# wallisc/TracerBoy

Hardware: AMD Instinct MI355X
Metric: Msamples/s (WxHxspp/s) (higher is better)
Workload: dtype f32; 1 GPU; cornell-box 1920x1080 64spp depth8; triangles=36, bvh_builder=sah, pipeline=lockstep, parallelism=tiles1, scene_in_lds=True, kernel_variant=matte

## Files before the change

### include/tracerboy_hip.h

```cpp
#ifndef TRACERBOY_HIP_H
#define TRACERBOY_HIP_H

#include <stdint.h>
#include "tb_abi.h"

#ifdef __cplusplus
extern "C" {
#endif

#define TB_OK 0
#define TB_E_INVALID -1
#define TB_E_NO_DEVICE -2
#define TB_E_IO -3
#define TB_E_PARSE -4
#define TB_E_DEVICE -5
#define TB_E_UNSUPPORTED -6
#define TB_E_NO_SCENE -7

typedef struct tb_context tb_context;

typedef struct tb_camera {
    float Position[3], LookAt[3], Right[3], Up[3];
    float LensHeight, FocalDistance;
} tb_camera;
// ... 220 lines not shown
void tb_default_visualize_settings(tb_visualize_settings* out);
int tb_record_paths(tb_context* ctx, uint32_t x, uint32_t y, uint32_t first_frame, uint32_t n_frames, TbPathFrame* frames_or_null, uint32_t* rays_total_or_null);
int tb_clear_paths(tb_context* ctx);
int tb_read_paths(tb_context* ctx, TbVisualizerRay* rays_or_null, uint32_t capacity, uint32_t* count);
int tb_visualize_rays(tb_context* ctx, const tb_visualize_settings* settings_or_null, float* rgba_f32_or_null, uint8_t* rgba8_or_null);
int tb_visualize_constants(const tb_camera* camera, uint32_t width, uint32_t height, const tb_visualize_settings* settings_or_null, TbVisualizeConstants* out);
int tb_run_visualize_rays(tb_context* ctx, const TbVisualizeConstants* constants, const TbVisualizerRay* rays, uint32_t n_rays, const float* scene_rgba,
                          const float* world_pos_or_null, float* out_rgba);

#define TB_RAYS_CLOSEST  0u
#define TB_RAYS_OCCLUDED 1u
#define TB_RAYS_DEVICE   0x100u
int tb_trace_rays(tb_context* ctx, uint32_t mode_and_flags, uint64_t n, const TbQueryRay* rays, void* out);

#define TB_RADIANCE_RAY        0u
#define TB_RADIANCE_HEMISPHERE 1u
#define TB_RADIANCE_DEVICE     0x100u
#define TB_RADIANCE_ACCUMULATE 0x200u
int tb_trace_radiance(tb_context* ctx, const tb_output_settings* settings_or_null, float time, const TbRadianceCall* call, uint64_t n,
                      const TbRadianceRay* rays, TbFloat4* out);
int tb_radiance_refusal(const TbRadianceCall* call, uint64_t n, const void* rays, const void* out, char* why_or_null, uint32_t why_bytes);
int tb_make_camera_rays(tb_context* ctx, const tb_output_settings* settings_or_null, float time, uint32_t width, uint32_t height,
                        uint32_t x0, uint32_t y0, uint32_t x1, uint32_t y1, uint32_t frame, uint32_t flags, TbRadianceRay* out, float* seed_advance_out);

#define TB_BAKE_DEVICE     0x100u
#define TB_BAKE_ACCUMULATE 0x200u
typedef struct tb_bake_call { uint32_t width, height, first_sample, num_samples, dilate_passes, flags; } tb_bake_call;
int tb_bake_lightmap(tb_context* ctx, const tb_output_settings* settings_or_null, float time, const tb_bake_call* call, const float* uv_or_null,
                     float* rgba_out);
int tb_bake_refusal(const tb_bake_call* call, const void* uv_or_null, const void* rgba_out, char* why_or_null, uint32_t why_bytes);
int tb_read_bake(tb_context* ctx, TbRadianceRay* rays_or_null, TbBakeTexel* texels_or_null, float* sums_or_null);
int tb_run_bake_raster(tb_context* ctx, uint32_t width, uint32_t height, uint32_t n_vertices, const float* positions, const float* normals,
                       const float* uvs, uint32_t n_triangles, const uint32_t* tri_vertex_index, TbRadianceRay* rays_out, TbBakeTexel* texels_out);
int tb_run_bake_dilate(tb_context* ctx, uint32_t width, uint32_t height, uint32_t passes, const float* rgba_in, float* rgba_out);

#define TB_PROBES_DEVICE     0x100u
#define TB_PROBES_ACCUMULATE 0x200u
#define TB_PROBES_KEEP_MAPS  0x400u
typedef struct tb_probe_call { uint32_t n, first_probe_number, resolution, first_sample, num_samples, flags; } tb_probe_call;
int tb_bake_probes(tb_context* ctx, const tb_output_settings* settings_or_null, float time, const tb_probe_call* call, const float* positions_xyz,
                   TbProbe* probes_out);
int tb_probes_refusal(const tb_probe_call* call, const void* positions_xyz, const void* probes_out, char* why_or_null, uint32_t why_bytes);
int tb_read_probe_maps(tb_context* ctx, float* sums_or_null, TbQueryHit* hits_or_null);
int tb_sample_probes(tb_context* ctx, uint32_t flags, const tb_probe_grid* grid, uint32_t resolution, float backface_limit, const TbProbe* probes,
                     uint64_t n, const float* points_xyz, const float* normals_xyz, float* rgba_out);
int tb_sh9_irradiance(const TbProbe* probe, const float* normal_xyz, float* rgb_out);
int tb_probe_directions(uint32_t resolution, float* dirs_out_or_null, float* weights_out_or_null);
int tb_run_probe_rays(tb_context* ctx, uint32_t n, uint32_t resolution, uint32_t first_probe_number, const float* positions_xyz,
                      TbRadianceRay* radiance_rays_out, TbQueryRay* query_rays_out);
int tb_run_probe_project(tb_context* ctx, uint32_t n, uint32_t resolution, const float* positions_xyz, const float* sums, const TbQueryHit* hits,
                         TbProbe* probes_out);

#define TB_NEAREST_SIGNED     0x1u
#define TB_NEAREST_DEVICE     0x100u
#define TB_NEAREST_HOST_BRUTE 0x1000u
#define TB_NEAREST_HOST_WALK  0x2000u
int tb_nearest_points(tb_context* ctx, uint32_t flags, uint64_t n, const TbQueryPoint* points, TbNearest* out);
int tb_bake_distance_field(tb_context* ctx, uint32_t flags, const tb_probe_grid* grid, float max_distance, float* out);
int tb_nearest_refusal(uint32_t flags, uint64_t n, const void* points, const void* out, const tb_probe_grid* grid_or_null, char* why_or_null,
                       uint32_t why_bytes);

#define TB_WINDING_DEVICE     0x100u
#define TB_WINDING_HOST_BRUTE 0x1000u
#define TB_WINDING_HOST_WALK  0x2000u
int tb_winding_numbers(tb_context* ctx, uint32_t flags, uint64_t n, const TbQueryPoint* points, float beta, float* out);
int tb_bake_winding_field(tb_context* ctx, uint32_t flags, const tb_probe_grid* grid, float beta, float* out);
int tb_nearest_points_winding(tb_context* ctx, uint32_t flags, uint64_t n, const TbQueryPoint* points, float beta, TbNearest* out);
int tb_bake_distance_field_winding(tb_context* ctx, uint32_t flags, const tb_probe_grid* grid, float max_distance, float beta, float* out);
int tb_winding_refusal(uint32_t flags, uint64_t n, const void* points, const void* out, const tb_probe_grid* grid_or_null, float beta, char* why_or_null,
                       uint32_t why_bytes);

#define TB_UPDATE_DEVICE    0x100u
#define TB_GEOMETRY_REBUILD 1u
int tb_update_positions(tb_context* ctx, uint32_t flags, uint32_t first_vertex, uint32_t n_vertices, const float* xyz);
int tb_update_normals(tb_context* ctx, uint32_t flags, uint32_t first_vertex, uint32_t n_vertices, const float* xyz);
int tb_set_instance_transforms(tb_context* ctx, uint32_t first_instance, uint32_t n_instances, const float* object_to_world_3x4);
int tb_commit_geometry(tb_context* ctx, uint32_t flags);
int tb_geometry_vertex_range(tb_context* ctx, uint32_t geometry, uint32_t* first_vertex, uint32_t* n_vertices);

int tb_load_meshes(tb_context* ctx, const tb_scene_desc* desc);
int tb_meshes_refusal(const tb_scene_desc* desc, char* why_or_null, uint32_t why_bytes);
int tb_host_smooth_normals(const float* positions, uint32_t n_vertices, const uint32_t* indices, uint32_t n_triangles, float* normals_out);
int tb_recompute_normals(tb_context* ctx, uint32_t first_vertex, uint32_t n_vertices);

typedef struct tb_nn_info { uint32_t in_channels; uint32_t out_channels[16]; uint32_t in_channels_of[16]; uint64_t weight_bytes; } tb_nn_info;
typedef struct tb_conv3x3_desc { uint32_t width, height;
                                 uint32_t c_a, c_b, c_out;
                                 uint32_t upsample_a;
                                 uint32_t pool, relu; } tb_conv3x3_desc;
int tb_nn_weights_info(const char* tza_path, tb_nn_info* out, char* err, uint32_t err_len);
int tb_neural_load(tb_context* ctx, const char* tza_path);
int tb_run_conv3x3(tb_context* ctx, const tb_conv3x3_desc* d, const uint16_t* in_a, const uint16_t* in_b_or_null,
                   const uint16_t* weight_oihw, const uint16_t* bias, uint16_t* out);
int tb_run_neural(tb_context* ctx, uint32_t width, uint32_t height, const float* color_rgba,
                  const float* albedo_rgba_or_null, const float* normal_rgba_or_null, float* out_rgba);
int tb_denoise_neural(tb_context* ctx, const tb_post_settings* post, float* rgba_f32_or_null, uint8_t* rgba8_or_null);
int tb_run_nn_pack(tb_context* ctx, uint32_t width, uint32_t height, uint32_t padded_w, uint32_t padded_h, uint32_t unorm_color, const float* color_rgba,
                   const float* albedo_rgba_or_null, const float* normal_rgba_or_null, uint16_t* out_tensor);
int tb_run_nn_unpack(tb_context* ctx, uint32_t width, uint32_t height, uint32_t padded_w, uint32_t padded_h, const uint16_t* tensor, float* out_rgba);
int tb_run_nn_resolve_aux(tb_context* ctx, uint32_t width, uint32_t height, const float* albedo_sum, const float* normal_sum, float* out_albedo,
                          float* out_normal);
int tb_run_nn_to_rgba8(tb_context* ctx, uint32_t width, uint32_t height, const float* rgba, uint8_t* out_rgba8);

typedef struct tb_sr_info { uint32_t in_channels[7], out_channels[7], kernel[7]; uint64_t weight_bytes; } tb_sr_info;
typedef struct tb_conv_desc { uint32_t width, height;
                              uint32_t c_a, c_b, c_out;
                              uint32_t kernel;
                              uint32_t upsample_a, relu;
                              uint32_t form;                 } tb_conv_desc;
int tb_sr_weights_info(const char* path, tb_sr_info* out, char* err, uint32_t err_len);
int tb_sr_read_layer(const char* path, uint32_t layer, uint16_t* weight_oihw, uint16_t* bias_or_null, char* err, uint32_t err_len);
int tb_sr_load(tb_context* ctx, const char* path);
int tb_run_conv(tb_context* ctx, const tb_conv_desc* d, const uint16_t* in_a, const uint16_t* in_b_or_null, const uint16_t* weight_oihw,
                const uint16_t* bias_or_null, uint16_t* out);
int tb_run_sr_finish(tb_context* ctx, uint32_t in_w, uint32_t in_h, const uint16_t* residual_2w2h3, const uint16_t* input_wh3, float* out_rgba);
int tb_run_sr(tb_context* ctx, uint32_t width, uint32_t height, const float* color_rgba, float* out_rgba);
int tb_upscale_neural(tb_context* ctx, const tb_post_settings* post, float* rgba_f32_or_null, uint8_t* rgba8_or_null);

#define TB_COMPARE_SSIM 1u
#define TB_COMPARE_SUMS 2u
#define TB_COMPARE_MEAN 0u
#define TB_COMPARE_DENOISED 1u
typedef struct tb_compare_settings { float peak; float rel_epsilon; uint32_t flags; } tb_compare_settings;
typedef struct tb_compare_result {
    uint64_t pixels, excluded, unsampled;
    uint64_t ssim_windows, ssim_windows_skipped;
    double mse, mae, rel_mse, max_abs, psnr, ssim;
    float gpu_us;
} tb_compare_result;
void tb_default_compare_settings(tb_compare_settings* out);
int tb_run_compare(tb_context* ctx, uint32_t w, uint32_t h, const float* test_rgba, const float* ref_rgba, const tb_compare_settings* settings_or_null,
                   tb_compare_result* out, float* sq_err_map_or_null, float* ssim_map_or_null);
int tb_set_reference(tb_context* ctx, uint32_t w, uint32_t h, const float* rgba_or_null);
int tb_compare(tb_context* ctx, uint32_t surface, const tb_compare_settings* settings_or_null, tb_compare_result* out, float* sq_err_map_or_null,
               float* ssim_map_or_null);

typedef struct tb_host_scene tb_host_scene;
int tb_host_scene_load(const char* pbrt_path, int bvh_builder, int load_flags, tb_host_scene** out, char* err, uint32_t err_len);
int tb_host_scene_procedural(int kind, uint32_t target_triangles, uint32_t seed, int bvh_builder, tb_host_scene** out, char* err, uint32_t err_len);
int tb_host_scene_from_meshes(const tb_scene_desc* desc, int bvh_builder, tb_host_scene** out, char* err, uint32_t err_len);
void tb_host_scene_free(tb_host_scene* s);
int tb_host_scene_view_get(tb_host_scene* s, TbSceneView* view);
int tb_host_scene_camera(tb_host_scene* s, tb_camera* cam);
int tb_host_scene_info(tb_host_scene* s, tb_scene_info* info);
int tb_host_scene_digest(tb_host_scene* s, uint64_t* out);
int tb_host_scene_frame_constants(tb_host_scene* s, const tb_output_settings* settings, uint32_t frame, float time_seed, TbPerFrameConstants* out);
int tb_host_scene_layout_b(tb_host_scene* s, const TbNodeB** nodes, uint32_t* num_nodes, const TbTriB** tris, uint32_t* num_tris, uint32_t* root_ref);
typedef struct tb_lds_image_info { uint32_t bytes, off_nodes, off_tris, num_nodes, num_tris, node_stride, tri_copies, root_ref, stack_depth; } tb_lds_image_info;
int tb_host_scene_lds_image(tb_host_scene* s, uint8_t* out, uint32_t capacity, tb_lds_image_info* info);
int tb_host_scene_tables_in_range(const TbTriB* tris, uint32_t num_tris, const uint32_t* hit_groups, uint32_t num_hit_groups, const uint32_t* indices,
    uint32_t num_indices, uint32_t num_vertex_floats, uint32_t num_materials);
typedef struct tb_wave_trips { uint64_t inner_trips, leaf_trips, idle_passes, inner_active, leaf_active; double cost; } tb_wave_trips;
typedef struct tb_wave_stage_info { uint32_t ran, rays, seed, park_min, depth_limit, moves, evaluations, inner_insts, leaf_insts, reserved;
    tb_wave_trips before, after; double milliseconds; } tb_wave_stage_info;
int tb_wave_replay(const char* const* steps, uint32_t lanes, uint32_t park_min, tb_wave_trips* out);
int tb_host_scene_wave_walk(tb_host_scene* s, uint32_t n, const float* origins, const float* dirs, const float* t_max, uint32_t* inner_steps,
    uint32_t* leaf_steps, char* steps, uint64_t steps_capacity);
int tb_host_scene_wave_rays(tb_host_scene* s, uint32_t seed, uint32_t waves, int feeler_percent, float* origins, float* dirs, float* t_max, uint32_t capacity);
int tb_host_scene_wave_cost(tb_host_scene* s, uint32_t seed, uint32_t waves, int feeler_percent, uint32_t park_min, tb_wave_trips* out);
int tb_host_scene_wave_stage(tb_host_scene* s, tb_wave_stage_info* out);
int tb_host_pbrt_dump(const char* pbrt_path, const char* out_path, char* err, uint32_t err_len);
int tb_host_scene_triangles(tb_host_scene* s, const float** positions, uint32_t* num_vertices, const uint32_t** tri_vertex_index,
                            const uint32_t** tri_geometry, const uint32_t** tri_primitive, const uint32_t** tri_flags, uint32_t* num_triangles);
int tb_host_scene_nearest(tb_host_scene* scene, uint32_t flags, uint64_t n, const TbQueryPoint* points, TbNearest* out);
int tb_host_scene_nearest_excess(tb_host_scene* scene, uint64_t n, const TbQueryPoint* points, float* worst_out);
int tb_host_scene_winding(tb_host_scene* scene, uint32_t flags, uint64_t n, const TbQueryPoint* points, float beta, float* out);

#ifdef __cplusplus
}
#endif
#endif
```

### tracerboy_amd/_ctypes_abi.py

```python
import ctypes as C

TB_GUIDE_ALBEDO, TB_GUIDE_NORMAL, TB_GUIDE_POSITION = 0, 1, 2


class TbFloat2(C.Structure):
    _fields_ = [("x", C.c_float), ("y", C.c_float)]


class TbFloat3(C.Structure):
    _fields_ = [("x", C.c_float), ("y", C.c_float), ("z", C.c_float)]


class TbFloat4(C.Structure):
    _fields_ = [("x", C.c_float), ("y", C.c_float), ("z", C.c_float), ("w", C.c_float)]


class TbPerFrameConstants(C.Structure):
    _fields_ = [
        ("CameraPosition", TbFloat3), ("Time", C.c_float),
        ("CameraLookAt", TbFloat3), ("InvalidateHistory", C.c_uint32),
        ("CameraUp", TbFloat3), ("OutputMode", C.c_uint32),
        ("CameraRight", TbFloat3), ("DOFFocusDistance", C.c_float),
        ("DOFApertureWidth", C.c_float), ("EnableNormalMaps", C.c_uint32), ("FocalDistance", C.c_float), ("FireflyClampValue", C.c_float),
        ("GlobalFrameCount", C.c_uint32), ("MinConvergence", C.c_float), ("LightCount", C.c_uint32), ("UseBlueNoise", C.c_uint32),
# ... 124 lines not shown


class TbFsrConstants(C.Structure):
    _fields_ = [("easu", C.c_uint32 * 16), ("rcas", C.c_uint32 * 4)]


TB_FSR_SURFACE_UNORM8 = 0
TB_FSR_SURFACE_F32 = 1


TB_MAX_VISUALIZER_RAYS = 1024
TB_PATH_JITTERED, TB_PATH_REJECTED, TB_PATH_TRUNCATED = 1, 2, 4


class TbVisualizerRay(C.Structure):
    _fields_ = [("Origin", C.c_float * 3), ("Direction", C.c_float * 3), ("HitT", C.c_float), ("BounceCount", C.c_float)]


class TbPathFrame(C.Structure):
    _fields_ = [("sum", C.c_float * 4), ("frame", C.c_uint32), ("first_ray", C.c_uint32), ("num_rays", C.c_uint32), ("flags", C.c_uint32)]


class TbVisualizeConstants(C.Structure):
    _fields_ = [("ResolutionX", C.c_uint32), ("ResolutionY", C.c_uint32), ("CylinderRadius", C.c_float), ("FocalLength", C.c_float),
                ("CameraPosition", C.c_float * 3), ("LensHeight", C.c_float), ("CameraLookAt", C.c_float * 3), ("RayDepth", C.c_float),
                ("CameraRight", C.c_float * 3), ("Padding2", C.c_float), ("CameraUp", C.c_float * 3), ("RayCount", C.c_int32)]


class tb_visualize_settings(C.Structure):
    _fields_ = [("RayWidth", C.c_float), ("RayDepth", C.c_float), ("RayCount", C.c_int32)]


class TbQueryRay(C.Structure):
    _fields_ = [("Origin", C.c_float * 3), ("TMax", C.c_float), ("Direction", C.c_float * 3), ("Flags", C.c_uint32)]


class TbQueryHit(C.Structure):
    _fields_ = [("T", C.c_float), ("U", C.c_float), ("V", C.c_float), ("Prim", C.c_uint32), ("Geom", C.c_uint32), ("Material", C.c_int32),
                ("UV", C.c_float * 2), ("Normal", C.c_float * 3), ("Pad", C.c_uint32)]


class TbRadianceRay(C.Structure):
    _fields_ = [("Origin", C.c_float * 3), ("SeedX", C.c_float), ("Direction", C.c_float * 3), ("SeedY", C.c_float)]


class TbRadianceCall(C.Structure):
    _fields_ = [("first_sample", C.c_uint32), ("num_samples", C.c_uint32), ("seed_advance", C.c_float), ("mode_and_flags", C.c_uint32)]


class TbBakeTexel(C.Structure):
    _fields_ = [("triangle", C.c_uint32), ("cls", C.c_uint32), ("w0", C.c_float), ("w1", C.c_float)]


class tb_bake_call(C.Structure):
    _fields_ = [("width", C.c_uint32), ("height", C.c_uint32), ("first_sample", C.c_uint32), ("num_samples", C.c_uint32),
                ("dilate_passes", C.c_uint32), ("flags", C.c_uint32)]


assert C.sizeof(TbBakeTexel) == 16 and C.sizeof(tb_bake_call) == 24


class TbProbe(C.Structure):
    _fields_ = [("SH", C.c_float * 27), ("Weight", C.c_float), ("Hits", C.c_float), ("Backfaces", C.c_float), ("MinDistance", C.c_float),
                ("MeanDistance", C.c_float)]


class tb_probe_grid(C.Structure):
    _fields_ = [("origin", C.c_float * 3), ("spacing", C.c_float * 3), ("count", C.c_uint32 * 3)]


class tb_probe_call(C.Structure):
    _fields_ = [("n", C.c_uint32), ("first_probe_number", C.c_uint32), ("resolution", C.c_uint32), ("first_sample", C.c_uint32),
                ("num_samples", C.c_uint32), ("flags", C.c_uint32)]


assert C.sizeof(TbProbe) == 128 and C.sizeof(tb_probe_grid) == 36 and C.sizeof(tb_probe_call) == 24


class TbQueryPoint(C.Structure):
    _fields_ = [("Position", C.c_float * 3), ("MaxDistance", C.c_float)]


class TbNearest(C.Structure):
    _fields_ = [("Point", C.c_float * 3), ("Distance", C.c_float), ("U", C.c_float), ("V", C.c_float), ("Prim", C.c_uint32), ("Geom", C.c_uint32)]


assert C.sizeof(TbQueryPoint) == 16 and C.sizeof(TbNearest) == 32


class tb_nn_info(C.Structure):
    _fields_ = [("in_channels", C.c_uint32), ("out_channels", C.c_uint32 * 16), ("in_channels_of", C.c_uint32 * 16), ("weight_bytes", C.c_uint64)]


class tb_conv3x3_desc(C.Structure):
    _fields_ = [(n, C.c_uint32) for n in ("width", "height", "c_a", "c_b", "c_out", "upsample_a", "pool", "relu")]


class tb_sr_info(C.Structure):
    _fields_ = [("in_channels", C.c_uint32 * 7), ("out_channels", C.c_uint32 * 7), ("kernel", C.c_uint32 * 7), ("weight_bytes", C.c_uint64)]


class tb_conv_desc(C.Structure):
    _fields_ = [(n, C.c_uint32) for n in ("width", "height", "c_a", "c_b", "c_out", "kernel", "upsample_a", "relu", "form")]


TB_UPDATE_DEVICE, TB_GEOMETRY_REBUILD = 0x100, 1
TB_MESH_NORMALS_FLAT, TB_MESH_NORMALS_SMOOTH, TB_MESH_DEVICE = 0, 1, 0x100


class tb_mesh_desc(C.Structure):
    _fields_ = [("positions", C.c_void_p), ("n_vertices", C.c_uint32), ("indices", C.c_void_p), ("n_triangles", C.c_uint32),
                ("normals_or_null", C.c_void_p), ("uvs_or_null", C.c_void_p), ("material", C.c_uint32), ("normals_mode", C.c_uint32)]


class tb_scene_desc(C.Structure):
    _fields_ = [("meshes", C.POINTER(tb_mesh_desc)), ("n_meshes", C.c_uint32), ("materials", C.POINTER(TbMaterial)), ("n_materials", C.c_uint32),
                ("camera_or_null", C.POINTER(tb_camera)), ("env_rgba_or_null", C.c_void_p), ("env_width", C.c_uint32), ("env_height", C.c_uint32),
                ("env_scale", C.c_float * 3), ("film_width", C.c_uint32), ("film_height", C.c_uint32), ("flags", C.c_uint32)]
TB_COMPARE_SSIM, TB_COMPARE_SUMS = 1, 2
TB_COMPARE_MEAN, TB_COMPARE_DENOISED = 0, 1


class tb_compare_settings(C.Structure):
    _fields_ = [("peak", C.c_float), ("rel_epsilon", C.c_float), ("flags", C.c_uint32)]


class tb_compare_result(C.Structure):
    _fields_ = [(n, C.c_uint64) for n in ("pixels", "excluded", "unsampled", "ssim_windows", "ssim_windows_skipped")] + \
               [(n, C.c_double) for n in ("mse", "mae", "rel_mse", "max_abs", "psnr", "ssim")] + [("gpu_us", C.c_float)]


class tb_readback_stats(C.Structure):
    _fields_ = [("ActiveWaves", C.c_uint32), ("ActivePixels", C.c_uint32), ("SelectedPixelDistance", C.c_float), ("SelectedMaterialID", C.c_int32),
                ("rays", TbRayStats)]


class tb_scene_info(C.Structure):
    _fields_ = [("numTriangles", C.c_uint32), ("numVertices", C.c_uint32), ("numMaterials", C.c_uint32), ("numLights", C.c_uint32),
                ("numGeometries", C.c_uint32), ("numTextures", C.c_uint32), ("bvhBytesA", C.c_uint32), ("bvhNodesB", C.c_uint32),
                ("bvhMaxDepth", C.c_uint32), ("filmWidth", C.c_uint32), ("filmHeight", C.c_uint32),
                ("sceneMin", C.c_float * 3), ("sceneMax", C.c_float * 3)]


class tb_lds_image_info(C.Structure):
    _fields_ = [(n, C.c_uint32) for n in ("bytes", "off_nodes", "off_tris", "num_nodes", "num_tris", "node_stride", "tri_copies", "root_ref", "stack_depth")]


class tb_wave_trips(C.Structure):
    _fields_ = [(n, C.c_uint64) for n in ("inner_trips", "leaf_trips", "idle_passes", "inner_active", "leaf_active")] + [("cost", C.c_double)]


class tb_wave_stage_info(C.Structure):
    _fields_ = [(n, C.c_uint32) for n in ("ran", "rays", "seed", "park_min", "depth_limit", "moves", "evaluations", "inner_insts", "leaf_insts",
                                          "reserved")] + [("before", tb_wave_trips), ("after", tb_wave_trips), ("milliseconds", C.c_double)]


class tb_state_info(C.Structure):
    _fields_ = [("version", C.c_uint32), ("width", C.c_uint32), ("height", C.c_uint32), ("first_frame", C.c_uint32), ("next_frame", C.c_uint32),
                ("time_seed", C.c_float), ("settings", tb_output_settings), ("camera", tb_camera),
                ("tile_rank", C.c_uint32), ("tile_world", C.c_uint32), ("tile_w", C.c_uint32), ("tile_h", C.c_uint32),
                ("alpha_test", C.c_uint32), ("adaptive", C.c_uint32), ("adaptive_test", C.c_uint32),
                ("adaptive_min_frames", C.c_int64), ("scene_digest", C.c_uint64), ("output_digest", C.c_uint64), ("jittered_digest", C.c_uint64)]


class tb_plan_input(C.Structure):
    _fields_ = [("variant_features", C.c_uint32), ("variant_waves_hi", C.c_uint32), ("variant_prepass_in_base", C.c_uint32),
                ("variant_has_wavefront", C.c_uint32), ("variant_has_pooled", C.c_uint32), ("variant_has_split", C.c_uint32), ("variant_stash_entries", C.c_uint32),
                ("scene_in_lds", C.c_uint32), ("lds_blob_bytes", C.c_uint32), ("stack_depth", C.c_uint32), ("two_level", C.c_uint32), ("has_lights", C.c_uint32),
                ("has_compact_nodes", C.c_uint32), ("interior_walk_triangle_share", C.c_float),
                ("width", C.c_uint32), ("height", C.c_uint32), ("frames", C.c_uint32), ("max_bounces", C.c_int32), ("owned_regions", C.c_uint64),
                ("count_rays", C.c_uint32), ("aov", C.c_uint32), ("realtime", C.c_uint32), ("selected_pixel", C.c_uint32),
                ("pipeline", C.c_int64), ("frame_group", C.c_int64), ("high_occupancy", C.c_int64), ("stack_lds_cap", C.c_int64), ("stack_overflow_max", C.c_int64),
                ("node_layout", C.c_int64), ("primary_prepass", C.c_int64), ("overlap_launches", C.c_int64), ("pooled_samples", C.c_int64),
                ("split_trav", C.c_int64), ("split_shade", C.c_int64), ("split_stack_cap", C.c_int64), ("guided_groups", C.c_int64), ("sync_call", C.c_uint32), ("costly_first", C.c_uint32),
                ("adaptive", C.c_uint32)]


class tb_launch_plan(C.Structure):
    _fields_ = [("pipeline", C.c_int32), ("groups", C.c_uint32), ("high_occupancy_copy", C.c_uint32), ("full_variant", C.c_uint32),
                ("stack_lds_entries", C.c_uint32), ("stack_overflow_entries", C.c_uint32), ("compact_nodes", C.c_uint32), ("prepass", C.c_uint32),
                ("overlap_launches", C.c_uint32), ("batch_frames", C.c_uint32), ("frame_group", C.c_uint32),
                ("rule_pipeline", C.c_uint32), ("rule_copy", C.c_uint32), ("rule_prepass", C.c_uint32), ("guided_groups", C.c_uint32), ("costly_first", C.c_uint32)]


assert C.sizeof(tb_state_info) == 208
assert C.sizeof(TbPostConstants) == 36
assert C.sizeof(TbTemporalConstants) == 144
assert C.sizeof(TbDenoiserConstants) == 28
assert C.sizeof(TbFsrConstants) == 80
assert C.sizeof(TbVisualizerRay) == 32 and C.sizeof(TbVisualizeConstants) == 80 and C.sizeof(TbPathFrame) == 32
assert C.sizeof(tb_visualize_settings) == 12
assert C.sizeof(TbQueryRay) == 32 and C.sizeof(TbQueryHit) == 48
assert C.sizeof(TbRadianceRay) == 32 and C.sizeof(TbRadianceCall) == 16
assert C.sizeof(tb_compare_settings) == 12 and C.sizeof(tb_compare_result) == 96
assert C.sizeof(TbPerFrameConstants) == 148
assert C.sizeof(TbConfigConstants) == 76
assert C.sizeof(TbLight) == 104
assert C.sizeof(TbMaterial) == 84
assert C.sizeof(TbTextureData) == 80
assert C.sizeof(TbHitGroupRecord) == 72
assert C.sizeof(TbNodeB) == 64
assert C.sizeof(TbTriB) == 48
```

### tracerboy_amd/api.py

```python
import ctypes as C
import os

import numpy as np

from . import _ctypes_abi as abi

_HERE = os.path.dirname(os.path.abspath(__file__))
LIB_PATH = os.environ.get("TB_LIB", os.path.join(_HERE, "libtracerboy_hip.so"))

_lib = None


class TracerBoyError(RuntimeError):
    def __init__(self, code, message):
        super().__init__("tracerboy_hip error %d: %s" % (code, message))
        self.code = code


def lib():
    global _lib
    if _lib is not None:
        return _lib
    if not os.path.exists(LIB_PATH):
        raise ImportError("libtracerboy_hip.so is not built: run `python -m tracerboy_amd.build` "
# ... 18 lines not shown
        "tb_get_camera": (C.c_int, [vp, P(abi.tb_camera)]),
        "tb_set_camera": (C.c_int, [vp, P(abi.tb_camera)]),
        "tb_get_material": (C.c_int, [vp, C.c_int, P(abi.TbMaterial)]),
        "tb_set_material": (C.c_int, [vp, C.c_int, P(abi.TbMaterial)]),
        "tb_material_count": (C.c_int, [vp]),
        "tb_render": (C.c_int, [vp, C.c_uint32, C.c_uint32, C.c_uint32, P(abi.tb_output_settings), C.c_float]),
        "tb_render_async": (C.c_int, [vp, C.c_uint32, C.c_uint32, C.c_uint32, P(abi.tb_output_settings), C.c_float]),
        "tb_sync": (C.c_int, [vp]),
        "tb_read_accum": (C.c_int, [vp, vp, vp]),
        "tb_default_post_settings": (None, [P(abi.tb_post_settings)]),
        "tb_default_denoiser_settings": (None, [P(abi.tb_denoiser_settings)]),
        "tb_render_realtime": (C.c_int, [vp, C.c_uint32, C.c_uint32, P(abi.tb_output_settings), P(abi.tb_denoiser_settings), C.c_float]),
        "tb_read_realtime": (C.c_int, [vp, C.c_int, vp]),
        "tb_denoise": (C.c_int, [vp, P(abi.tb_denoiser_settings), vp]),
        "tb_read_denoise_stage": (C.c_int, [vp, C.c_int, vp]),
        "tb_render_guides": (C.c_int, [vp, C.c_uint32, C.c_uint32]),
        "tb_read_guide": (C.c_int, [vp, C.c_int, vp]),
        "tb_set_sample_budget": (C.c_int, [vp, C.c_uint32, C.c_uint32, vp]),
        "tb_read_sample_budget": (C.c_int, [vp, vp]),
        "tb_budget_stop_converged": (C.c_int, [vp, C.c_float, C.c_uint32, P(C.c_uint64), P(C.c_uint64)]),
        "tb_run_budget_stop": (C.c_int, [vp, C.c_uint32, C.c_uint32, vp, vp, vp, C.c_float, C.c_uint32, C.c_uint32, P(C.c_uint64), P(C.c_uint64)]),
        "tb_post_process": (C.c_int, [vp, P(abi.tb_post_settings), C.c_uint32, vp, vp]),
        "tb_read_averaged_luminance": (C.c_int, [vp, P(C.c_float)]),
        "tb_write_image_rgba8": (C.c_int, [C.c_char_p, C.c_uint32, C.c_uint32, vp]),
        "tb_write_image_f32": (C.c_int, [C.c_char_p, C.c_uint32, C.c_uint32, vp]),
        "tb_decode_image": (C.c_int, [C.c_char_p, P(C.c_uint32), P(C.c_uint32), P(C.c_int), P(C.c_int), vp]),
        "tb_read_aov": (C.c_int, [vp, C.c_int, vp]),
        "tb_accum_device_ptr": (C.c_int, [vp, P(vp), P(vp)]),
        "tb_read_stats": (C.c_int, [vp, P(abi.tb_readback_stats)]),
        "tb_read_wave_profile": (C.c_int, [vp, P(C.c_uint64)]),
        "tb_read_split_profile": (C.c_int, [vp, P(C.c_uint64)]),
        "tb_plan_defaults": (None, [P(abi.tb_plan_input)]),
        "tb_plan_launch": (C.c_int, [P(abi.tb_plan_input), P(abi.tb_launch_plan)]),
        "tb_variant_waves_hi": (C.c_int, [C.c_char_p]),
        "tb_variant_waves_lds": (C.c_int, [C.c_char_p]),
        "tb_invalidate_history": (None, [vp]),
        "tb_samples_rendered": (C.c_uint32, [vp]),
        "tb_select_pixel": (C.c_int, [vp, C.c_uint32, C.c_uint32]),
        "tb_set_tile_assignment": (C.c_int, [vp, C.c_uint32, C.c_uint32, C.c_uint32, C.c_uint32]),
        "tb_owned_pixels": (C.c_uint64, [vp, C.c_uint32, C.c_uint32]),
        "tb_pack_owned_device": (C.c_int, [vp, vp]),
        "tb_pack_owned_device_async": (C.c_int, [vp, vp]),
        "tb_stream": (vp, [vp]),
        "tb_unpack_gathered_device": (C.c_int, [vp, vp, vp, C.c_uint64, C.c_uint32, C.c_uint32, C.c_uint32, C.c_uint32, C.c_uint32, vp]),
        "tb_unpack_gathered_host": (C.c_int, [C.c_uint32, C.c_uint32, C.c_uint32, C.c_uint32, C.c_uint32, P(vp), vp]),
        "tb_set_option": (C.c_int, [vp, C.c_char_p, C.c_int64]),
        "tb_get_option": (C.c_int64, [vp, C.c_char_p]),
        "tb_host_scene_view": (C.c_int, [vp, P(abi.TbSceneView)]),
        "tb_make_frame_constants": (C.c_int, [vp, C.c_uint32, C.c_uint32, C.c_uint32, P(abi.tb_output_settings), C.c_float, P(abi.TbPerFrameConstants)]),
        "tb_last_render_ms": (C.c_float, [vp]),
        "tb_trace_closest": (C.c_int, [vp, C.c_uint32] + [vp] * 11),
        "tb_device_math": (C.c_int, [vp, C.c_int, C.c_uint32, vp, vp, vp]),
        "tb_run_temporal": (C.c_int, [vp, P(abi.TbTemporalConstants)] + [vp] * 8),
        "tb_run_denoise_pass": (C.c_int, [vp, P(abi.TbDenoiserConstants)] + [vp] * 5),
        "tb_run_composite": (C.c_int, [vp, C.c_uint32, C.c_uint32] + [vp] * 4),
        "tb_fsr_constants": (C.c_int, [C.c_uint32] * 4 + [C.c_float, P(abi.TbFsrConstants)]),
        "tb_run_fsr_easu": (C.c_int, [vp, P(abi.TbFsrConstants)] + [C.c_uint32] * 5 + [vp, vp]),
        "tb_run_fsr_rcas": (C.c_int, [vp, P(abi.TbFsrConstants)] + [C.c_uint32] * 3 + [vp, vp]),
        "tb_upscale": (C.c_int, [vp, P(abi.tb_post_settings), C.c_uint32, C.c_uint32, C.c_uint32, C.c_float, vp, vp]),
        "tb_default_visualize_settings": (None, [P(abi.tb_visualize_settings)]),
        "tb_record_paths": (C.c_int, [vp] + [C.c_uint32] * 4 + [vp, P(C.c_uint32)]),
        "tb_clear_paths": (C.c_int, [vp]),
        "tb_read_paths": (C.c_int, [vp, vp, C.c_uint32, P(C.c_uint32)]),
        "tb_visualize_rays": (C.c_int, [vp, P(abi.tb_visualize_settings), vp, vp]),
        "tb_visualize_constants": (C.c_int, [P(abi.tb_camera), C.c_uint32, C.c_uint32, P(abi.tb_visualize_settings), P(abi.TbVisualizeConstants)]),
        "tb_run_visualize_rays": (C.c_int, [vp, P(abi.TbVisualizeConstants), vp, C.c_uint32, vp, vp, vp]),
        "tb_trace_rays": (C.c_int, [vp, C.c_uint32, C.c_uint64, vp, vp]),
        "tb_trace_radiance": (C.c_int, [vp, P(abi.tb_output_settings), C.c_float, P(abi.TbRadianceCall), C.c_uint64, vp, vp]),
        "tb_radiance_refusal": (C.c_int, [P(abi.TbRadianceCall), C.c_uint64, vp, vp, C.c_char_p, C.c_uint32]),
        "tb_make_camera_rays": (C.c_int, [vp, P(abi.tb_output_settings), C.c_float] + [C.c_uint32] * 8 + [vp, P(C.c_float)]),
        "tb_bake_lightmap": (C.c_int, [vp, P(abi.tb_output_settings), C.c_float, P(abi.tb_bake_call), vp, vp]),
        "tb_bake_refusal": (C.c_int, [P(abi.tb_bake_call), vp, vp, C.c_char_p, C.c_uint32]),
        "tb_read_bake": (C.c_int, [vp, vp, vp, vp]),
        "tb_run_bake_raster": (C.c_int, [vp, C.c_uint32, C.c_uint32, C.c_uint32, vp, vp, vp, C.c_uint32, vp, vp, vp]),
        "tb_run_bake_dilate": (C.c_int, [vp, C.c_uint32, C.c_uint32, C.c_uint32, vp, vp]),
        "tb_bake_probes": (C.c_int, [vp, P(abi.tb_output_settings), C.c_float, P(abi.tb_probe_call), vp, vp]),
        "tb_probes_refusal": (C.c_int, [P(abi.tb_probe_call), vp, vp, C.c_char_p, C.c_uint32]),
        "tb_read_probe_maps": (C.c_int, [vp, vp, vp]),
        "tb_sample_probes": (C.c_int, [vp, C.c_uint32, P(abi.tb_probe_grid), C.c_uint32, C.c_float, vp, C.c_uint64, vp, vp, vp]),
        "tb_sh9_irradiance": (C.c_int, [vp, vp, vp]),
        "tb_probe_directions": (C.c_int, [C.c_uint32, vp, vp]),
        "tb_run_probe_rays": (C.c_int, [vp, C.c_uint32, C.c_uint32, C.c_uint32, vp, vp, vp]),
        "tb_run_probe_project": (C.c_int, [vp, C.c_uint32, C.c_uint32, vp, vp, vp, vp]),
        "tb_nearest_points": (C.c_int, [vp, C.c_uint32, C.c_uint64, vp, vp]),
        "tb_bake_distance_field": (C.c_int, [vp, C.c_uint32, P(abi.tb_probe_grid), C.c_float, vp]),
        "tb_nearest_refusal": (C.c_int, [C.c_uint32, C.c_uint64, vp, vp, P(abi.tb_probe_grid), C.c_char_p, C.c_uint32]),
        "tb_host_scene_nearest": (C.c_int, [vp, C.c_uint32, C.c_uint64, vp, vp]),
        "tb_host_scene_nearest_excess": (C.c_int, [vp, C.c_uint64, vp, P(C.c_float)]),
        "tb_winding_numbers": (C.c_int, [vp, C.c_uint32, C.c_uint64, vp, C.c_float, vp]),
        "tb_bake_winding_field": (C.c_int, [vp, C.c_uint32, P(abi.tb_probe_grid), C.c_float, vp]),
        "tb_nearest_points_winding": (C.c_int, [vp, C.c_uint32, C.c_uint64, vp, C.c_float, vp]),
        "tb_bake_distance_field_winding": (C.c_int, [vp, C.c_uint32, P(abi.tb_probe_grid), C.c_float, C.c_float, vp]),
        "tb_winding_refusal": (C.c_int, [C.c_uint32, C.c_uint64, vp, vp, P(abi.tb_probe_grid), C.c_float, C.c_char_p, C.c_uint32]),
        "tb_host_scene_winding": (C.c_int, [vp, C.c_uint32, C.c_uint64, vp, C.c_float, vp]),
        "tb_update_positions": (C.c_int, [vp, C.c_uint32, C.c_uint32, C.c_uint32, vp]),
        "tb_update_normals": (C.c_int, [vp, C.c_uint32, C.c_uint32, C.c_uint32, vp]),
        "tb_set_instance_transforms": (C.c_int, [vp, C.c_uint32, C.c_uint32, vp]),
        "tb_commit_geometry": (C.c_int, [vp, C.c_uint32]),
        "tb_geometry_vertex_range": (C.c_int, [vp, C.c_uint32, P(C.c_uint32), P(C.c_uint32)]),
        "tb_load_meshes": (C.c_int, [vp, P(abi.tb_scene_desc)]),
        "tb_meshes_refusal": (C.c_int, [P(abi.tb_scene_desc), C.c_char_p, C.c_uint32]),
        "tb_host_scene_from_meshes": (C.c_int, [P(abi.tb_scene_desc), C.c_int, P(vp), C.c_char_p, C.c_uint32]),
        "tb_host_smooth_normals": (C.c_int, [vp, C.c_uint32, vp, C.c_uint32, vp]),
        "tb_recompute_normals": (C.c_int, [vp, C.c_uint32, C.c_uint32]),
        "tb_default_compare_settings": (None, [P(abi.tb_compare_settings)]),
        "tb_run_compare": (C.c_int, [vp, C.c_uint32, C.c_uint32, vp, vp, P(abi.tb_compare_settings), P(abi.tb_compare_result), vp, vp]),
        "tb_set_reference": (C.c_int, [vp, C.c_uint32, C.c_uint32, vp]),
        "tb_compare": (C.c_int, [vp, C.c_uint32, P(abi.tb_compare_settings), P(abi.tb_compare_result), vp, vp]),
        "tb_nn_weights_info": (C.c_int, [C.c_char_p, P(abi.tb_nn_info), C.c_char_p, C.c_uint32]),
        "tb_neural_load": (C.c_int, [vp, C.c_char_p]),
        "tb_run_conv3x3": (C.c_int, [vp, P(abi.tb_conv3x3_desc)] + [vp] * 5),
        "tb_run_neural": (C.c_int, [vp, C.c_uint32, C.c_uint32] + [vp] * 4),
        "tb_denoise_neural": (C.c_int, [vp, P(abi.tb_post_settings), vp, vp]),
        "tb_run_nn_pack": (C.c_int, [vp] + [C.c_uint32] * 5 + [vp] * 4),
        "tb_run_nn_unpack": (C.c_int, [vp] + [C.c_uint32] * 4 + [vp, vp]),
        "tb_run_nn_resolve_aux": (C.c_int, [vp, C.c_uint32, C.c_uint32] + [vp] * 4),
        "tb_run_nn_to_rgba8": (C.c_int, [vp, C.c_uint32, C.c_uint32, vp, vp]),
        "tb_sr_weights_info": (C.c_int, [C.c_char_p, P(abi.tb_sr_info), C.c_char_p, C.c_uint32]),
        "tb_sr_read_layer": (C.c_int, [C.c_char_p, C.c_uint32, vp, vp, C.c_char_p, C.c_uint32]),
        "tb_sr_load": (C.c_int, [vp, C.c_char_p]),
        "tb_run_conv": (C.c_int, [vp, P(abi.tb_conv_desc)] + [vp] * 5),
        "tb_run_sr_finish": (C.c_int, [vp, C.c_uint32, C.c_uint32, vp, vp, vp]),
        "tb_run_sr": (C.c_int, [vp, C.c_uint32, C.c_uint32, vp, vp]),
        "tb_upscale_neural": (C.c_int, [vp, P(abi.tb_post_settings), vp, vp]),
        "tb_variant_stash_entries": (C.c_int, [C.c_char_p]),
        "tb_frame_groups": (C.c_uint32, [C.c_uint32, C.c_uint32, C.c_uint32, C.c_uint32, P(C.c_uint32), P(C.c_uint32)]),
        "tb_state_begin": (C.c_int, [vp, C.c_uint32, C.c_uint32, P(abi.tb_output_settings), C.c_float, C.c_uint32]),
        "tb_state_save": (C.c_int, [vp, C.c_char_p]),
        "tb_state_load": (C.c_int, [vp, C.c_char_p, C.c_uint32]),
        "tb_accum_digest": (C.c_int, [vp, P(C.c_uint64)]),
        "tb_scene_digest": (C.c_int, [vp, P(C.c_uint64)]),
        "tb_state_info_read": (C.c_int, [C.c_char_p, P(abi.tb_state_info), C.c_char_p, C.c_uint32]),
        "tb_state_read_host": (C.c_int, [C.c_char_p, P(abi.tb_state_info), vp, vp, C.c_char_p, C.c_uint32]),
        "tb_state_write_host": (C.c_int, [C.c_char_p, P(abi.tb_state_info), vp, vp]),
        "tb_state_digest_host": (C.c_uint64, [vp, C.c_uint64]),
        "tb_host_scene_digest": (C.c_int, [vp, P(C.c_uint64)]),
        "tb_host_scene_load": (C.c_int, [C.c_char_p, C.c_int, C.c_int, P(vp), C.c_char_p, C.c_uint32]),
        "tb_host_scene_procedural": (C.c_int, [C.c_int, C.c_uint32, C.c_uint32, C.c_int, P(vp), C.c_char_p, C.c_uint32]),
        "tb_host_scene_free": (None, [vp]),
        "tb_host_pbrt_dump": (C.c_int, [C.c_char_p, C.c_char_p, C.c_char_p, C.c_uint32]),
        "tb_host_scene_view_get": (C.c_int, [vp, P(abi.TbSceneView)]),
        "tb_host_scene_camera": (C.c_int, [vp, P(abi.tb_camera)]),
        "tb_host_scene_info": (C.c_int, [vp, P(abi.tb_scene_info)]),
        "tb_host_scene_frame_constants": (C.c_int, [vp, P(abi.tb_output_settings), C.c_uint32, C.c_float, P(abi.TbPerFrameConstants)]),
        "tb_host_scene_layout_b": (C.c_int, [vp, P(P(abi.TbNodeB)), P(C.c_uint32), P(P(abi.TbTriB)), P(C.c_uint32), P(C.c_uint32)]),
        "tb_host_scene_lds_image": (C.c_int, [vp, P(C.c_uint8), C.c_uint32, P(abi.tb_lds_image_info)]),
        "tb_host_scene_tables_in_range": (C.c_int, [P(abi.TbTriB), C.c_uint32, P(C.c_uint32), C.c_uint32, P(C.c_uint32)] + [C.c_uint32] * 3),
        "tb_host_scene_triangles": (C.c_int, [vp, P(P(C.c_float)), P(C.c_uint32), P(P(C.c_uint32)), P(P(C.c_uint32)), P(P(C.c_uint32)), P(P(C.c_uint32)), P(C.c_uint32)]),
        "tb_wave_replay": (C.c_int, [P(C.c_char_p), C.c_uint32, C.c_uint32, P(abi.tb_wave_trips)]),
        "tb_host_scene_wave_walk": (C.c_int, [vp, C.c_uint32, P(C.c_float), P(C.c_float), P(C.c_float), P(C.c_uint32), P(C.c_uint32), C.c_char_p, C.c_uint64]),
        "tb_host_scene_wave_rays": (C.c_int, [vp, C.c_uint32, C.c_uint32, C.c_int, P(C.c_float), P(C.c_float), P(C.c_float), C.c_uint32]),
        "tb_host_scene_wave_cost": (C.c_int, [vp, C.c_uint32, C.c_uint32, C.c_int, C.c_uint32, P(abi.tb_wave_trips)]),
        "tb_host_scene_wave_stage": (C.c_int, [vp, P(abi.tb_wave_stage_info)]),
    }
    for name, (res, args) in sig.items():
        fn = getattr(L, name)
        fn.restype = res
        fn.argtypes = args
    L._tb_exports = sorted(sig)
    _lib = L
    return L


def GetDefaultOutputSettings():
    s = abi.tb_output_settings()
    lib().tb_default_output_settings(C.byref(s))
    return s


def GetDefaultDenoiserSettings():
    s = abi.tb_denoiser_settings()
    lib().tb_default_denoiser_settings(C.byref(s))
    return s


def GetDefaultPostProcessSettings():
    s = abi.tb_post_settings()
    lib().tb_default_post_settings(C.byref(s))
    return s


def GetDefaultCompareSettings():
    s = abi.tb_compare_settings()
    lib().tb_default_compare_settings(C.byref(s))
    return s


COMPARE_FIELDS = tuple(n for n, _ in abi.tb_compare_result._fields_)


def FsrConstants(in_width, in_height, out_width, out_height, sharpness=0.2):
    k = abi.TbFsrConstants()
    rc = lib().tb_fsr_constants(in_width, in_height, out_width, out_height, sharpness, C.byref(k))
    if rc != 0:
        raise TracerBoyError(rc, "tb_fsr_constants: a size is 0 or the sharpness is not finite")
    return k


def GetDefaultVisualizeSettings():
    s = abi.tb_visualize_settings()
    lib().tb_default_visualize_settings(C.byref(s))
    return s


def VisualizeConstants(camera, width, height, settings=None):
    k = abi.TbVisualizeConstants()
    rc = lib().tb_visualize_constants(C.byref(camera), width, height, C.byref(settings) if settings is not None else None, C.byref(k))
    if rc != 0:
        raise TracerBoyError(rc, "tb_visualize_constants: a size is 0")
    return k


RAYS_CLOSEST, RAYS_OCCLUDED, RAYS_DEVICE = 0, 1, 0x100
QUERY_RAY_DISABLED = 1
QUERY_RAY_DTYPE = np.dtype([("Origin", np.float32, 3), ("TMax", np.float32), ("Direction", np.float32, 3), ("Flags", np.uint32)])
QUERY_HIT_DTYPE = np.dtype([("T", np.float32), ("U", np.float32), ("V", np.float32), ("Prim", np.uint32), ("Geom", np.uint32), ("Material", np.int32),
                            ("UV", np.float32, 2), ("Normal", np.float32, 3), ("Pad", np.uint32)])


def make_query_rays(origins, dirs, tmax=np.inf, disabled=None):
    o = np.asarray(origins, np.float32); d = np.asarray(dirs, np.float32)
    if o.ndim != 2 or o.shape[1] != 3 or d.shape != o.shape:
        raise ValueError("make_query_rays: origins and dirs are (n, 3) arrays of one length")
    rays = np.zeros(o.shape[0], QUERY_RAY_DTYPE)
    rays["Origin"] = o; rays["Direction"] = d
    rays["TMax"] = np.broadcast_to(np.asarray(tmax, np.float32), (o.shape[0],))
    if disabled is not None:
        rays["Flags"] = np.where(np.broadcast_to(np.asarray(disabled, bool), (o.shape[0],)), QUERY_RAY_DISABLED, 0)
    return rays


def _is_torch_tensor(a):
    return type(a).__module__.split(".")[0] == "torch" and hasattr(a, "data_ptr")


def _check_query_rays(rays, mode, device):
    if mode not in (RAYS_CLOSEST, RAYS_OCCLUDED):
        raise ValueError("TraceRays: mode is RAYS_CLOSEST or RAYS_OCCLUDED, not %r" % (mode,))
    if _is_torch_tensor(rays):
        import torch
        if rays.dtype != torch.float32 or rays.dim() != 2 or rays.shape[1] != 8:
            raise ValueError("TraceRays: a tensor of rays is float32 of shape (n, 8), not %s %s" % (rays.dtype, tuple(rays.shape)))
        if not rays.is_contiguous():
            raise ValueError("TraceRays: the tensor of rays is not contiguous")
        if rays.device.type != "cuda" or rays.device.index != device:
            raise ValueError("TraceRays: the tensor of rays is on %s, the context on cuda:%d" % (rays.device, device))
        if rays.data_ptr() % 16:
            raise ValueError("TraceRays: the tensor of rays is not 16-B aligned")
        return True
    if not isinstance(rays, np.ndarray):
        raise ValueError("TraceRays: rays are a numpy array or a torch tensor, not %s" % type(rays).__name__)
    if rays.dtype == QUERY_RAY_DTYPE:
        if rays.ndim != 1:
            raise ValueError("TraceRays: an array of QUERY_RAY_DTYPE has one dimension, not %d" % rays.ndim)
    elif rays.dtype != np.float32 or rays.ndim != 2 or rays.shape[1] != 8:
        raise ValueError("TraceRays: rays are QUERY_RAY_DTYPE or float32 of shape (n, 8), not %s %s" % (rays.dtype, rays.shape))
    if not rays.flags["C_CONTIGUOUS"]:
        raise ValueError("TraceRays: the array of rays is not contiguous")
    return False


RADIANCE_RAY, RADIANCE_HEMISPHERE, RADIANCE_DEVICE, RADIANCE_ACCUMULATE = 0, 1, 0x100, 0x200
RADIANCE_RAY_DTYPE = np.dtype([("Origin", np.float32, 3), ("SeedX", np.float32), ("Direction", np.float32, 3), ("SeedY", np.float32)])
assert RADIANCE_RAY_DTYPE.itemsize == 32


def make_radiance_rays(origins, dirs_or_normals, seed_xy=None):
    o = np.asarray(origins, np.float32); d = np.asarray(dirs_or_normals, np.float32)
    if o.ndim != 2 or o.shape[1] != 3 or d.shape != o.shape:
        raise ValueError("make_radiance_rays: origins and directions are (n, 3) arrays of one length")
    n = o.shape[0]
    if seed_xy is None:
        i = np.arange(n, dtype=np.int64)
        seed = np.stack([i % 4096, i // 4096], axis=1).astype(np.float32)
    else:
        seed = np.asarray(seed_xy, np.float32)
        if seed.shape != (n, 2):
            raise ValueError("make_radiance_rays: seed_xy is an (n, 2) array")
    rays = np.zeros(n, RADIANCE_RAY_DTYPE)
    rays["Origin"] = o; rays["Direction"] = d; rays["SeedX"] = seed[:, 0]; rays["SeedY"] = seed[:, 1]
    return rays


def _check_count(what, name, v, lo, hi):
    if isinstance(v, bool) or not isinstance(v, (int, np.integer)) or v < lo or v > hi:
        raise ValueError("%s: %s is a whole number in [%d, %d], not %r" % (what, name, lo, hi, v))
    return int(v)


def _check_radiance_call(rays, samples, first_sample, seed_advance, mode, out, device):
    if isinstance(mode, bool) or mode not in (RADIANCE_RAY, RADIANCE_HEMISPHERE):
        raise ValueError("TraceRadiance: mode is RADIANCE_RAY or RADIANCE_HEMISPHERE, not %r" % (mode,))
    _check_count("TraceRadiance", "samples", samples, 1, 1 << 24)
    _check_count("TraceRadiance", "first_sample", first_sample, 0, (1 << 32) - samples)
    if isinstance(seed_advance, bool) or not isinstance(seed_advance, (int, float, np.integer, np.floating)) or not np.isfinite(seed_advance):
        raise ValueError("TraceRadiance: seed_advance is a finite number, not %r" % (seed_advance,))
    if _is_torch_tensor(rays):
        import torch
        if rays.dtype != torch.float32 or rays.dim() != 2 or rays.shape[1] != 8:
            raise ValueError("TraceRadiance: a tensor of rays is float32 of shape (n, 8), not %s %s" % (rays.dtype, tuple(rays.shape)))
        if not rays.is_contiguous():
            raise ValueError("TraceRadiance: the tensor of rays is not contiguous")
        if rays.device.type != "cuda" or rays.device.index != device:
            raise ValueError("TraceRadiance: the tensor of rays is on %s, the context on cuda:%d" % (rays.device, device))
        if rays.data_ptr() % 16:
            raise ValueError("TraceRadiance: the tensor of rays is not 16-B aligned")
# ... 518 lines not shown
    rc = lib().tb_state_read_host(os.fsencode(path), C.byref(info), _np_ptr(out), _np_ptr(jit), err, 512)
    if rc != 0:
        raise TracerBoyError(rc, err.value.decode(errors="replace"))
    return info, out, jit


def WriteStateFile(path, info, output, jittered):
    out = np.ascontiguousarray(output, np.float32); jit = np.ascontiguousarray(jittered, np.float32)
    assert out.ndim == 3 and out.shape[2] == 4 and jit.shape == out.shape
    h = abi.tb_state_info.from_buffer_copy(info)
    h.height, h.width = out.shape[:2]
    rc = lib().tb_state_write_host(os.fsencode(path), C.byref(h), _np_ptr(out), _np_ptr(jit))
    if rc != 0:
        raise TracerBoyError(rc, "could not write state file %s" % path)


class HostScene:

    def __init__(self, path=None, procedural=None, bvh_builder=0, flatten_instances=True, flip_texture_uvs=True, reinsertion_passes=None,
                 reinsertion_share=None, presplit=None, wave_tree=None):
        self._h = C.c_void_p()
        err = C.create_string_buffer(512)
        if wave_tree is not None:
            bvh_builder |= (1 + (1 if wave_tree else 0)) << 6
        if reinsertion_passes is not None:
            bvh_builder |= (int(reinsertion_passes) + 1) << 8
        if reinsertion_share is not None:
            bvh_builder |= int(reinsertion_share) << 16
        if presplit is not None:
            bvh_builder |= min(int(presplit), 127) << 24
        if path is not None:
            rc = lib().tb_host_scene_load(os.fsencode(path), bvh_builder, (1 if flatten_instances else 0) | (0 if flip_texture_uvs else 2), C.byref(self._h), err, 512)
        else:
            kind, tris, seed = procedural
            rc = lib().tb_host_scene_procedural(kind, tris, seed, bvh_builder, C.byref(self._h), err, 512)
        if rc != 0:
            raise TracerBoyError(rc, err.value.decode(errors="replace"))

    @classmethod
    def from_meshes(cls, meshes, materials, camera=None, environment=None, env_scale=(1, 1, 1), film=(0, 0), bvh_builder=0):
        d, keep, _ = _scene_desc("HostScene.from_meshes", meshes, materials, camera, environment, env_scale, film, None)
        self = cls.__new__(cls)
        self._h = C.c_void_p()
        err = C.create_string_buffer(512)
        rc = lib().tb_host_scene_from_meshes(C.byref(d), bvh_builder, C.byref(self._h), err, 512)
        if rc != 0:
            raise TracerBoyError(rc, err.value.decode(errors="replace"))
        return self

    def close(self):
        if self._h:
            lib().tb_host_scene_free(self._h)
            self._h = C.c_void_p()

    def __del__(self):
        try:
            self.close()
        except Exception:
            pass

    def view(self):
        v = abi.TbSceneView()
        lib().tb_host_scene_view_get(self._h, C.byref(v))
        return v

    def camera(self):
        c = abi.tb_camera()
        lib().tb_host_scene_camera(self._h, C.byref(c))
        return c

    def info(self):
        i = abi.tb_scene_info()
        lib().tb_host_scene_info(self._h, C.byref(i))
        return i

    def frame_constants(self, settings=None, frame=0, time_seed=0.0):
        pf = abi.TbPerFrameConstants()
        lib().tb_host_scene_frame_constants(self._h, C.byref(settings) if settings is not None else None, frame, time_seed, C.byref(pf))
        return pf

    def digest(self):
        d = C.c_uint64()
        rc = lib().tb_host_scene_digest(self._h, C.byref(d))
        if rc != 0:
            raise TracerBoyError(rc, "tb_host_scene_digest")
        return d.value

    def bvh_bytes(self):
        v = self.view()
        return np.ctypeslib.as_array(C.cast(v.bvh, C.POINTER(C.c_uint8)), shape=(v.bvhBytes,)).copy()

    def triangles(self):
        pos = C.POINTER(C.c_float)(); nv = C.c_uint32(); tvi = C.POINTER(C.c_uint32)(); tg = C.POINTER(C.c_uint32)()
        tp = C.POINTER(C.c_uint32)(); tf = C.POINTER(C.c_uint32)(); nt = C.c_uint32()
        lib().tb_host_scene_triangles(self._h, C.byref(pos), C.byref(nv), C.byref(tvi), C.byref(tg), C.byref(tp), C.byref(tf), C.byref(nt))
        n, m = nt.value, nv.value
        return dict(positions=np.ctypeslib.as_array(pos, shape=(m, 3)).copy(), tri_vertex_index=np.ctypeslib.as_array(tvi, shape=(n, 3)).copy(),
                    tri_geometry=np.ctypeslib.as_array(tg, shape=(n,)).copy(), tri_primitive=np.ctypeslib.as_array(tp, shape=(n,)).copy(),
                    tri_flags=np.ctypeslib.as_array(tf, shape=(n,)).copy())

    def layout_b(self):
        nodes = C.POINTER(abi.TbNodeB)(); nn = C.c_uint32(); tris = C.POINTER(abi.TbTriB)(); nt = C.c_uint32(); root = C.c_uint32()
        lib().tb_host_scene_layout_b(self._h, C.byref(nodes), C.byref(nn), C.byref(tris), C.byref(nt), C.byref(root))
        nb = np.frombuffer(C.string_at(nodes, nn.value * 64), dtype=np.uint32).reshape(nn.value, 16).copy()
        tb = np.frombuffer(C.string_at(tris, nt.value * 48), dtype=np.uint32).reshape(nt.value, 12).copy()
        return nb, tb, root.value

    def nearest(self, points, signed=False, walk=False):
        _check_query_points("HostScene.nearest", points, 0, allow_tensor=False)
        flags = (NEAREST_SIGNED if _check_flag("HostScene.nearest", "signed", signed) else 0) | \
            (NEAREST_HOST_WALK if _check_flag("HostScene.nearest", "walk", walk) else NEAREST_HOST_BRUTE)
        out = np.empty(points.shape[0], NEAREST_DTYPE)
        rc = lib().tb_host_scene_nearest(self._h, flags, points.shape[0], _np_ptr(points), _np_ptr(out))
        if rc != 0:
            raise TracerBoyError(rc, "tb_host_scene_nearest")
        return out

    def winding(self, points, beta=WINDING_BETA, walk=False):
        _check_query_points("HostScene.winding", points, 0, allow_tensor=False)
        beta = _check_beta("HostScene.winding", beta)
        flags = WINDING_HOST_WALK if _check_flag("HostScene.winding", "walk", walk) else WINDING_HOST_BRUTE
        out = np.empty(points.shape[0], np.float32)
        rc = lib().tb_host_scene_winding(self._h, flags, points.shape[0], _np_ptr(points), beta, _np_ptr(out))
        if rc != 0:
            raise TracerBoyError(rc, "tb_host_scene_winding")
        return out

    def nearest_excess(self, points):
        _check_query_points("HostScene.nearest_excess", points, 0, allow_tensor=False)
        worst = C.c_float()
        rc = lib().tb_host_scene_nearest_excess(self._h, points.shape[0], _np_ptr(points), C.byref(worst))
        if rc != 0:
            raise TracerBoyError(rc, "tb_host_scene_nearest_excess")
        return worst.value

    def lds_image(self):
        info = abi.tb_lds_image_info()
        rc = lib().tb_host_scene_lds_image(self._h, None, 0, C.byref(info))
        if rc != 0:
            raise TracerBoyError(rc, "tb_host_scene_lds_image")
        buf = np.zeros(info.bytes, dtype=np.uint8)
        rc = lib().tb_host_scene_lds_image(self._h, buf.ctypes.data_as(C.POINTER(C.c_uint8)), info.bytes, C.byref(info))
        if rc != 0:
            raise TracerBoyError(rc, "tb_host_scene_lds_image")
        return buf, info

    def wave_stage(self):
        info = abi.tb_wave_stage_info()
        rc = lib().tb_host_scene_wave_stage(self._h, C.byref(info))
        if rc != 0:
            raise TracerBoyError(rc, "tb_host_scene_wave_stage")
        return info

    def wave_rays(self, seed=0, waves=0, feeler_percent=-1):
        fp = C.POINTER(C.c_float)
        n = lib().tb_host_scene_wave_rays(self._h, seed, waves, feeler_percent, None, None, None, 0)
        if n < 0:
            raise TracerBoyError(n, "tb_host_scene_wave_rays")
        o = np.zeros((n, 3), dtype=np.float32); d = np.zeros((n, 3), dtype=np.float32); t = np.zeros(n, dtype=np.float32)
        lib().tb_host_scene_wave_rays(self._h, seed, waves, feeler_percent, o.ctypes.data_as(fp), d.ctypes.data_as(fp), t.ctypes.data_as(fp), n)
        return o, d, t

    def wave_walk(self, origins, dirs, t_max=None, want_steps=False):
        fp = C.POINTER(C.c_float); up = C.POINTER(C.c_uint32)
        o = np.ascontiguousarray(origins, dtype=np.float32).reshape(-1, 3); d = np.ascontiguousarray(dirs, dtype=np.float32).reshape(-1, 3)
        t = None if t_max is None else np.ascontiguousarray(t_max, dtype=np.float32)
        n = len(o); inner = np.zeros(n, dtype=np.uint32); leaf = np.zeros(n, dtype=np.uint32)
        rc = lib().tb_host_scene_wave_walk(self._h, n, o.ctypes.data_as(fp), d.ctypes.data_as(fp), None if t is None else t.ctypes.data_as(fp),
                                           inner.ctypes.data_as(up), leaf.ctypes.data_as(up), None, 0)
        if rc != 0:
            raise TracerBoyError(rc, "tb_host_scene_wave_walk")
        if not want_steps:
            return inner, leaf
        cap = int(inner.sum()) + int(leaf.sum()) + n
        buf = C.create_string_buffer(cap)
        rc = lib().tb_host_scene_wave_walk(self._h, n, o.ctypes.data_as(fp), d.ctypes.data_as(fp), None if t is None else t.ctypes.data_as(fp), None, None, buf, cap)
        if rc != 0:
            raise TracerBoyError(rc, "tb_host_scene_wave_walk")
        return inner, leaf, [w.decode() for w in buf.raw[:cap].split(b"\0")[:n]]

    def wave_cost(self, seed=0, waves=0, feeler_percent=-1, park_min=0):
        out = abi.tb_wave_trips()
        rc = lib().tb_host_scene_wave_cost(self._h, seed, waves, feeler_percent, park_min, C.byref(out))
        if rc != 0:
            raise TracerBoyError(rc, "tb_host_scene_wave_cost")
        return out


def wave_replay(steps, park_min=2):
    arr = (C.c_char_p * max(len(steps), 1))(*[s.encode() for s in steps])
    out = abi.tb_wave_trips()
    rc = lib().tb_wave_replay(arr, len(steps), park_min, C.byref(out))
    if rc != 0:
        raise TracerBoyError(rc, "tb_wave_replay")
    return out


class TracerBoy:

    def __init__(self, device_id=0, devices=None):
        self._L = lib()
        self._ctx = C.c_void_p()
        if devices is not None:
            ids = (C.c_int * len(devices))(*[int(d) for d in devices])
            rc = self._L.tb_create_multi(C.byref(self._ctx), ids, len(devices))
        else:
            rc = self._L.tb_create(C.byref(self._ctx), int(device_id))
        if rc != 0:
            raise TracerBoyError(rc, (self._L.tb_last_error(None) or b"").decode(errors="replace"))
        self.width = self.height = 0
        self._budget_shape = None
        self._device = int(devices[0]) if devices is not None else int(device_id)

    def close(self):
        if getattr(self, "_ctx", None):
            self._L.tb_destroy(self._ctx)
            self._ctx = C.c_void_p()

    def __del__(self):
        try:
            self.close()
        except Exception:
            pass

    def __enter__(self):
        return self

    def __exit__(self, *a):
        self.close()

    def _check(self, rc):
        if rc != 0:
            raise TracerBoyError(rc, (self._L.tb_last_error(self._ctx) or b"").decode(errors="replace"))

    def LoadScene(self, sceneFileName):
        self._num_vertices = None
        self._check(self._L.tb_load_scene(self._ctx, os.fsencode(sceneFileName)))

    def LoadProcedural(self, kind, target_triangles, seed=1234):
        self._num_vertices = None
        self._check(self._L.tb_load_procedural(self._ctx, kind, target_triangles, seed))

    def LoadMeshes(self, meshes, materials, camera=None, environment=None, env_scale=(1, 1, 1), film=(0, 0)):
        meshes = list(meshes)
        d, keep, on_device = _scene_desc("LoadMeshes", meshes, materials, camera, environment, env_scale, film, getattr(self, "_device", 0))
        if on_device:
            import torch
            torch.cuda.current_stream(meshes[0].positions.device).synchronize()
        self._num_vertices = None
        self._check(self._L.tb_load_meshes(self._ctx, C.byref(d)))

    def Render(self, width, height, n_frames=1, outputSettings=None, time_seed=0.0, sync=True):
        fn = self._L.tb_render if sync else self._L.tb_render_async
        self._check(fn(self._ctx, width, height, n_frames, C.byref(outputSettings) if outputSettings is not None else None, time_seed))
        self.width, self.height = width, height

    def Sync(self):
        self._check(self._L.tb_sync(self._ctx))

    def GetNumberOfSamplesSinceLastInvalidate(self):
        return int(self._L.tb_samples_rendered(self._ctx))

    def InvalidateHistory(self):
        self._L.tb_invalidate_history(self._ctx)

    def GetCamera(self):
        c = abi.tb_camera()
        self._check(self._L.tb_get_camera(self._ctx, C.byref(c)))
        return c

    def SetCamera(self, cam):
        self._check(self._L.tb_set_camera(self._ctx, C.byref(cam)))

    def IsMaterialIDValid(self, i):
        return 0 <= i < self._L.tb_material_count(self._ctx)

    def GetMaterial(self, i):
        m = abi.TbMaterial()
        self._check(self._L.tb_get_material(self._ctx, i, C.byref(m)))
        return m

    def SetMaterial(self, i, m):
        self._check(self._L.tb_set_material(self._ctx, i, C.byref(m)))

    def SelectPixel(self, x, y):
        self._check(self._L.tb_select_pixel(self._ctx, x, y))

    def ReadbackStats(self):
        s = abi.tb_readback_stats()
        self._check(self._L.tb_read_stats(self._ctx, C.byref(s)))
        return s

    def WaveProfile(self):
        raw = (C.c_uint64 * 14)()
        self._check(self._L.tb_read_wave_profile(self._ctx, raw))
        names = ["bvh_inner", "bvh_leaf", "closest_shade", "shadow_slot", "scatter", "regenerate", "iteration"]
        return {n: (int(raw[2 * i]), int(raw[2 * i + 1]), (raw[2 * i] / (64.0 * raw[2 * i + 1])) if raw[2 * i + 1] else 0.0) for i, n in enumerate(names)}

    def SplitProfile(self):
        raw = (C.c_uint64 * 16)()
        self._check(self._L.tb_read_split_profile(self._ctx, raw))
        v = [int(x) for x in raw]
        d = dict(t_inner_steps=v[0], t_inner_lanes=v[1], t_leaf_steps=v[2], t_leaf_lanes=v[3], t_ticket_draws=v[4], t_rays=v[5], t_sleeps=v[6], t_cycles=v[7],
                 s_rounds=v[8], s_lanes=v[9], s_sleeps=v[10], s_cycles=v[11], s_rays=v[12], s_samples=v[13], t_waves=v[14], s_waves=v[15])
        d["inner_occupancy"] = v[1] / (64.0 * v[0]) if v[0] else 0.0
        d["leaf_occupancy"] = v[3] / (64.0 * v[2]) if v[2] else 0.0
# ... 708 lines not shown
```

### tracerboy_amd/csrc/host/bvh_build.cpp

```cpp
#include "host_scene.h"
#include "launch_plan.h"
#include "lds_image.h"
#include "wave_cost.h"
#include "../../../include/tb_vec.h"

#include <algorithm>
#include <atomic>
#include <chrono>
#include <cmath>
#include <cstring>
#include <cstdlib>
#include <exception>
#include <stdexcept>
#include <thread>
#include <mutex>

namespace tbhost {

namespace {

struct Bounds { tb3 mn, mx; };

struct Tree {
    uint32_t N = 0;
    std::vector<uint32_t> order;
    std::vector<uint32_t> left, right;
    std::vector<uint32_t> refTri; std::vector<Bounds> refBox;
};

inline tb3 P(const HostScene& s, uint32_t tri, int k) { const float* p = &s.positions[3ull * s.triVertexIndex[3ull * tri + k]];
    return tb3_make(p[0], p[1], p[2]); }
inline uint32_t triOfRef(const Tree& t, uint32_t r) { return t.refTri.empty() ? r : t.refTri[r]; }
inline Bounds boundsOfRef(const HostScene& s, const Tree& t, uint32_t r)
{
    if (!t.refBox.empty()) return t.refBox[r];
    Bounds b; b.mn = tb3_splat(3.402823466e+38f); b.mx = tb3_splat(-3.402823466e+38f);
    for (int k = 0; k < 3; k++) { const tb3 v = P(s, r, k); b.mn = tb3_min(b.mn, v); b.mx = tb3_max(b.mx, v); }
    return b;
}

template <class F> void parallelFor(size_t n, F f)
{
    unsigned hw = std::thread::hardware_concurrency(); if (hw == 0) hw = 1;
    size_t nt = n < 65536 ? 1 : std::min<size_t>(hw, 16);
    if (nt == 1) { f((size_t)0, n); return; }
    std::vector<std::thread> th; size_t chunk = (n + nt - 1) / nt;
    std::exception_ptr failed; std::mutex fm;
    for (size_t t = 0; t < nt; t++) { size_t a = t * chunk, b = std::min(n, a + chunk);
        if (a < b) th.emplace_back([=, &failed, &fm]() { try { f(a, b); } catch (...) { std::lock_guard<std::mutex> g(fm); if (!failed) failed = std::current_exception(); } }); }
    for (auto& t : th) t.join();
    if (failed) std::rethrow_exception(failed);
}

inline uint32_t expand10(uint32_t v) { v &= 0x3ff; v = (v | (v << 16)) & 0x030000FF; v = (v | (v << 8)) & 0x0300F00F; v = (v | (v << 4)) & 0x030C30C3;
    v = (v | (v << 2)) & 0x09249249; return v; }

inline uint32_t mortonCode(tb3 c, tb3 smin, tb3 dim)
{
    tb3 u = (c - smin) / dim;
    float ax = tb_min(tb_max(u.x * 1024.0f, 0.0f), 1023.0f), ay = tb_min(tb_max(u.y * 1024.0f, 0.0f), 1023.0f), az = tb_min(tb_max(u.z * 1024.0f, 0.0f),
        1023.0f);
    return expand10((uint32_t)ay) | (expand10((uint32_t)ax) << 1) | (expand10((uint32_t)az) << 2);
}

void sortAndSplit(std::vector<uint64_t>& keys, Tree& t)
{
    const uint32_t N = t.N;
    std::sort(keys.begin(), keys.end());
    t.order.resize(N);
    std::vector<uint32_t> codes(N);
    for (uint32_t i = 0; i < N; i++) { t.order[i] = (uint32_t)keys[i]; codes[i] = (uint32_t)(keys[i] >> 32); }
    if (N < 2) return;
    t.left.resize(N - 1); t.right.resize(N - 1);
    auto delta = [&](int64_t a, int64_t b) -> int {
        if (b < 0 || b >= (int64_t)N) return -1;
        uint32_t x = codes[(size_t)a] ^ codes[(size_t)b];
        if (x) return __builtin_clz(x);
        uint32_t y = (uint32_t)a ^ (uint32_t)b;
        return (y ? __builtin_clz(y) : 32) + 31;
    };
    parallelFor(N - 1, [&](size_t a, size_t b) {
        for (int64_t i = (int64_t)a; i < (int64_t)b; i++) {
            int d = delta(i, i + 1) - delta(i, i - 1); d = (d > 0) - (d < 0);
            int dmin = delta(i, i - d);
            int64_t lmax = 2; while (delta(i, i + lmax * d) > dmin) lmax *= 4;
            int64_t l = 0; for (int64_t st = lmax / 2; st > 0; st /= 2) if (delta(i, i + (l + st) * d) > dmin) l += st;
            int64_t j = i + l * d, first = std::min(i, j), last = std::max(i, j);
            int dn = delta(first, last);
            int64_t split = first, step = last - first;
            do { step = (step + 1) >> 1; int64_t ns = split + step; if (ns < last && delta(first, ns) > dn) split = ns; } while (step > 1);
            t.left[(size_t)i] = (split == first) ? (N - 1) + (uint32_t)split : (uint32_t)split;
            t.right[(size_t)i] = (split + 1 == last) ? (N - 1) + (uint32_t)split + 1 : (uint32_t)split + 1;
        }
    });
}

void buildLbvh(const HostScene& s, Tree& t)
{
    const uint32_t N = t.N;
    tb3 smin = tb3_splat(3.402823466e+38f), smax = tb3_splat(-3.402823466e+38f);
    for (uint32_t i = 0; i < N; i++) for (int k = 0; k < 3; k++) { tb3 v = P(s, i, k); smin = tb3_min(v, smin); smax = tb3_max(v, smax); }
    tb3 dim = tb3_max(smax - smin, tb3_splat(0.00001f));
    std::vector<uint64_t> keys(N);
    parallelFor(N, [&](size_t a, size_t b) {
        for (size_t i = a; i < b; i++) {
            tb3 c = (P(s, (uint32_t)i, 0) + P(s, (uint32_t)i, 1) + P(s, (uint32_t)i, 2)) / 3.0f;
            keys[i] = ((uint64_t)mortonCode(c, smin, dim) << 32) | (uint64_t)i;
        }
    });
    sortAndSplit(keys, t);
}

inline Bounds emptyB() { Bounds b; b.mn = tb3_splat(3.402823466e+38f); b.mx = tb3_splat(-3.402823466e+38f); return b; }
inline void grow(Bounds& b, tb3 p) { b.mn = tb3_min(b.mn, p); b.mx = tb3_max(b.mx, p); }
inline void grow(Bounds& b, const Bounds& o) { b.mn = tb3_min(b.mn, o.mn); b.mx = tb3_max(b.mx, o.mx); }
inline float area(const Bounds& b) { tb3 d = b.mx - b.mn; if (d.x < 0 || d.y < 0 || d.z < 0) return 0.0f; return 2.0f * (d.x * d.y + d.y * d.z + d.z * d.x); }

void buildSah(const HostScene& s, Tree& t)
{
    const uint32_t N = t.N;
    std::vector<Bounds> tb(N); std::vector<tb3> cen(N);
    parallelFor(N, [&](size_t a, size_t z) { for (size_t i = a; i < z; i++) { const Bounds b = boundsOfRef(s, t, (uint32_t)i);
        tb[i] = b; cen[i] = (b.mn + b.mx) * 0.5f; } });
    std::vector<uint32_t> ids(N); for (uint32_t i = 0; i < N; i++) ids[i] = i;
    if (N >= 2) { t.left.assign(N - 1, 0); t.right.assign(N - 1, 0); }
    constexpr int B = 32;
    struct Bins { Bounds bb[3][B]; uint32_t bc[3][B]; Bounds cb; };
    constexpr uint32_t WIDE = 1u << 17;
    bool topPhase = true;
    auto split = [&](uint32_t begin, uint32_t end) -> uint32_t {
        const uint32_t count = end - begin;
        const bool wide = topPhase && count >= WIDE;
        Bounds cb = emptyB();
        if (wide) {
            std::mutex m;
            parallelFor(count, [&](size_t a, size_t z) { Bounds l = emptyB(); for (size_t i = a; i < z; i++) grow(l, cen[ids[begin + i]]);
                std::lock_guard<std::mutex> g(m); grow(cb, l); });
        } else for (uint32_t i = begin; i < end; i++) grow(cb, cen[ids[i]]);
        const tb3 ext = cb.mx - cb.mn;
        const int axis = (ext.x >= ext.y && ext.x >= ext.z) ? 0 : (ext.y >= ext.z ? 1 : 2);
        uint32_t mid = begin + count / 2;
        const float e = tb3_get(ext, axis);
        bool cut = false;
        if (e > 0.0f && count > 2) {
            float k0[3], k1[3]; bool use[3];
            for (int ax = 0; ax < 3; ax++) { const float ea = tb3_get(ext, ax); use[ax] = ea > 0.0f; k0[ax] = tb3_get(cb.mn, ax);
                k1[ax] = use[ax] ? (float)B * (1.0f - 1e-6f) / ea : 0.0f; }
            auto binOf = [&](uint32_t id, int ax) { int b = (int)((tb3_get(cen[id], ax) - k0[ax]) * k1[ax]); return b < 0 ? 0 : (b >= B ? B - 1 : b); };
            Bounds bb[3][B]; uint32_t bc[3][B];
            for (int ax = 0; ax < 3; ax++) for (int i = 0; i < B; i++) { bb[ax][i] = emptyB(); bc[ax][i] = 0; }
            auto scan = [&](size_t a, size_t z, Bounds (*lb)[B], uint32_t (*lc)[B]) {
                for (size_t i = a; i < z; i++) { const uint32_t id = ids[begin + i];
                    for (int ax = 0; ax < 3; ax++) if (use[ax]) { const int b = binOf(id, ax); grow(lb[ax][b], tb[id]); lc[ax][b]++; } } };
            if (wide) {
                std::mutex m;
                parallelFor(count, [&](size_t a, size_t z) {
                    std::vector<Bounds> lbv(3 * B, emptyB()); std::vector<uint32_t> lcv(3 * B, 0);
                    scan(a, z, (Bounds(*)[B])lbv.data(), (uint32_t(*)[B])lcv.data());
                    std::lock_guard<std::mutex> g(m);
                    for (int ax = 0; ax < 3; ax++) for (int i = 0; i < B; i++) { grow(bb[ax][i], lbv[ax * B + i]); bc[ax][i] += lcv[ax * B + i]; } });
            } else scan(0, count, bb, bc);
            float bestCost = 3.402823466e+38f; int bestAxis = -1, bestBin = -1;
            for (int ax = 0; ax < 3; ax++) {
                if (!use[ax]) continue;
                float ra[B]; Bounds acc = emptyB(); uint32_t rc[B]; uint32_t c = 0;
                for (int i = B - 1; i > 0; i--) { grow(acc, bb[ax][i]); c += bc[ax][i]; ra[i] = area(acc); rc[i] = c; }
                acc = emptyB(); c = 0;
                for (int i = 0; i < B - 1; i++) { grow(acc, bb[ax][i]); c += bc[ax][i]; if (c == 0 || rc[i + 1] == 0) continue;
// ... 68 lines not shown
    Poly p; p.n = 3;
    for (int k = 0; k < 3; k++) { const tb3 v = P(s, tri, k); p.v[k][0] = v.x; p.v[k][1] = v.y; p.v[k][2] = v.z; }
    for (int a = 0; a < 3 && p.n >= 3; a++) { clipPoly(p, a, tb3_get(b.mn, a), false); if (p.n >= 3) clipPoly(p, a, tb3_get(b.mx, a), true); }
    return p;
}
inline Bounds boundsOfPoly(const Poly& p, const Bounds& within)
{
    double mn[3] = {1e300, 1e300, 1e300}, mx[3] = {-1e300, -1e300, -1e300};
    for (int i = 0; i < p.n; i++) for (int k = 0; k < 3; k++) { mn[k] = std::min(mn[k], p.v[i][k]); mx[k] = std::max(mx[k], p.v[i][k]); }
    Bounds b;
    float lo[3], hi[3];
    for (int k = 0; k < 3; k++) {
        const double pad = 4.0 * 1.1920929e-7 * std::max(std::fabs(mn[k]), std::fabs(mx[k]));
        lo[k] = std::nextafterf((float)(mn[k] - pad), -3.402823466e+38f); hi[k] = std::nextafterf((float)(mx[k] + pad), 3.402823466e+38f);
    }
    b.mn = tb3_max(tb3_make(lo[0], lo[1], lo[2]), within.mn); b.mx = tb3_min(tb3_make(hi[0], hi[1], hi[2]), within.mx);
    return b;
}
inline double idealArea(const Poly& p)
{
    double ax = 0, ay = 0, az = 0;
    for (int i = 1; i + 1 < p.n; i++) {
        const double e1[3] = {p.v[i][0] - p.v[0][0], p.v[i][1] - p.v[0][1], p.v[i][2] - p.v[0][2]}, e2[3] = {p.v[i + 1][0] - p.v[0][0], p.v[i + 1][1] - p.v[0][1],
            p.v[i + 1][2] - p.v[0][2]};
        ax += e1[1] * e2[2] - e1[2] * e2[1]; ay += e1[2] * e2[0] - e1[0] * e2[2]; az += e1[0] * e2[1] - e1[1] * e2[0];
    }
    return std::fabs(ax) + std::fabs(ay) + std::fabs(az);
}

void presplitReferences(const HostScene& s, Tree& t, int percent)
{
    const uint32_t N = t.N;
    const uint64_t budget = (uint64_t)N * (uint64_t)std::max(percent, 0) / 100u;
    if (!budget || N < 2) return;
    t.refTri.resize(N); t.refBox.resize(N);
    Bounds scene = emptyB();
    for (uint32_t i = 0; i < N; i++) { t.refTri[i] = i; Bounds b = emptyB(); for (int k = 0; k < 3; k++) grow(b, P(s, i, k)); t.refBox[i] = b; grow(scene, b); }
    const tb3 sext = tb3_max(scene.mx - scene.mn, tb3_splat(1e-30f));
    auto areaD = [](const Bounds& b) { const double x = (double)b.mx.x - b.mn.x, y = (double)b.mx.y - b.mn.y, z = (double)b.mx.z - b.mn.z; return 2.0 * (x * y + y * z + z * x); };
    auto priority = [&](uint32_t r) { const Poly p = polyOfRef(s, t.refTri[r], t.refBox[r]); return p.n < 3 ? 0.0 : areaD(t.refBox[r]) - idealArea(p); };
    struct Item { double pri; uint32_t ref; bool operator<(const Item& o) const { return pri < o.pri || (pri == o.pri && ref > o.ref); } };
    std::vector<Item> heap; heap.reserve(N + (size_t)budget * 2);
    double totalArea = 0;
    for (uint32_t i = 0; i < N; i++) { totalArea += areaD(t.refBox[i]); heap.push_back(Item{priority(i), i}); }
    std::make_heap(heap.begin(), heap.end());
    constexpr double kBig = 16.0, kEmpty = 0.3;
    const double bigArea = kBig * totalArea / (double)N;
    uint64_t made = 0;
    while (made < budget && !heap.empty()) {
        std::pop_heap(heap.begin(), heap.end()); const Item it = heap.back(); heap.pop_back();
        if (!(it.pri > 0.0)) break;
        if (!(areaD(t.refBox[it.ref]) > bigArea && it.pri > kEmpty * areaD(t.refBox[it.ref]))) continue;
        const Bounds b = t.refBox[it.ref];
        const tb3 ext = b.mx - b.mn;
        int axis = (ext.x >= ext.y && ext.x >= ext.z) ? 0 : (ext.y >= ext.z ? 1 : 2);
        const double lo = tb3_get(b.mn, axis), hi = tb3_get(b.mx, axis), s0 = tb3_get(scene.mn, axis), se = tb3_get(sext, axis);
        double plane = 0.5 * (lo + hi);
        for (int level = 1; level <= 30; level++) {
            const double cell = se / (double)(1u << level);
            const double k = std::floor((lo - s0) / cell) + 1.0, cand = s0 + k * cell;
            if (cand > lo && cand < hi) { plane = cand; break; }
        }
        const float pf = (float)plane;
        if (!(pf > tb3_get(b.mn, axis) && pf < tb3_get(b.mx, axis))) continue;
        Poly whole = polyOfRef(s, t.refTri[it.ref], b);
        if (whole.n < 3) continue;
        Poly L = whole, R = whole; clipPoly(L, axis, (double)pf, true); clipPoly(R, axis, (double)pf, false);
        if (L.n < 3 || R.n < 3) continue;
        Bounds wl = b, wr = b;
        if (axis == 0) { wl.mx.x = pf; wr.mn.x = pf; } else if (axis == 1) { wl.mx.y = pf; wr.mn.y = pf; } else { wl.mx.z = pf; wr.mn.z = pf; }
        const Bounds bl = boundsOfPoly(L, wl), br = boundsOfPoly(R, wr);
        const uint32_t nr = (uint32_t)t.refTri.size();
        t.refBox[it.ref] = bl; t.refTri.push_back(t.refTri[it.ref]); t.refBox.push_back(br); made++;
        heap.push_back(Item{areaD(bl) - idealArea(L), it.ref}); std::push_heap(heap.begin(), heap.end());
        heap.push_back(Item{areaD(br) - idealArea(R), nr}); std::push_heap(heap.begin(), heap.end());
    }
    if (!made) { t.refTri.clear(); t.refBox.clear(); return; }
    t.N = (uint32_t)t.refTri.size();
}

void optimizeByReinsertion(const HostScene& s, Tree& t, int maxPasses, double minGain)
{
    const uint32_t N = t.N; if (N < 4) return;
    const uint32_t M = 2 * N - 1, NONE = 0xffffffffu;
    std::vector<Bounds> box(M); std::vector<float> sa(M); std::vector<uint32_t> parent(M, NONE); std::vector<uint16_t> height(M, 0);
    auto isLeaf = [&](uint32_t x) { return x >= N - 1; };
    auto unite = [&](const Bounds& a, const Bounds& b) { Bounds u = a; grow(u, b); return u; };
    for (uint32_t k = 0; k < N; k++) { Bounds b = boundsOfRef(s, t, t.order[k]);
        b.mn = tb3_min(b.mn, b.mx - tb3_splat(0.001f)); box[N - 1 + k] = b; sa[N - 1 + k] = area(b); }
    for (uint32_t i = 0; i + 1 < N; i++) { parent[t.left[i]] = i; parent[t.right[i]] = i; }
    auto pull = [&](uint32_t x) { const uint32_t l = t.left[x], r = t.right[x]; box[x] = unite(box[l], box[r]); sa[x] = area(box[x]);
        height[x] = (uint16_t)(1 + std::max(height[l], height[r])); };
    std::vector<uint32_t> st;
    {
        std::vector<uint32_t> pre; pre.reserve(M); st.push_back(0);
        while (!st.empty()) { uint32_t x = st.back(); st.pop_back(); pre.push_back(x); if (!isLeaf(x)) { st.push_back(t.left[x]); st.push_back(t.right[x]); } }
        for (size_t w = pre.size(); w-- > 0;) if (!isLeaf(pre[w])) pull(pre[w]);
    }
    const uint32_t h0 = height[0] + 1u;
    const uint32_t depthLimit = (h0 <= 31u ? 31u : (h0 <= 39u ? 39u : h0)) - 1u;
    auto refit = [&](uint32_t x) { for (; x != NONE; x = parent[x]) pull(x); };
    auto totalCost = [&]() { double c = 0; for (uint32_t i = 0; i + 1 < N; i++) c += sa[i]; return c; };
    auto replaceChild = [&](uint32_t p, uint32_t from, uint32_t to) { if (t.left[p] == from) t.left[p] = to; else t.right[p] = to; parent[to] = p; };
    double cost = totalCost();
    std::vector<uint32_t> cand(M - 1);
    struct Item { uint32_t node, depth; float induced; };
    std::vector<Item> todo;
    for (int pass = 0; pass < maxPasses; pass++) {
        for (uint32_t x = 1; x < M; x++) cand[x - 1] = x;
        std::stable_sort(cand.begin(), cand.end(), [&](uint32_t a, uint32_t b) { return sa[a] > sa[b]; });
        size_t tried = 0;
        const double share = (double)s.reinsertionShare;
        const size_t limit = share >= 100.0 ? cand.size() : (size_t)((double)cand.size() * std::max(share, 0.0) / 100.0);
        for (uint32_t x : cand) {
            if (tried++ >= limit) break;
            const uint32_t p = parent[x]; if (p == NONE || p == 0) continue;
            const uint32_t g = parent[p], sib = t.left[p] == x ? t.right[p] : t.left[p];
            replaceChild(g, p, sib); parent[p] = NONE; refit(g);
            const Bounds bx = box[x]; const float ax = sa[x]; const uint32_t hx = height[x];
            uint32_t best = sib; float bestInc = area(unite(box[sib], bx));
            for (uint32_t a = parent[sib]; a != NONE; a = parent[a]) bestInc += area(unite(box[a], bx)) - sa[a];
            todo.clear(); todo.push_back(Item{0, 0, 0.0f});
            while (!todo.empty()) {
                const Item it = todo.back(); todo.pop_back();
                if (it.induced + ax >= bestInc) continue;
                const uint32_t y = it.node;
                const float direct = area(unite(box[y], bx));
                if (y != 0 && it.induced + direct < bestInc && it.depth + 1u + std::max<uint32_t>(hx,
                    height[y]) <= depthLimit) { bestInc = it.induced + direct; best = y; }
                if (!isLeaf(y)) {
                    const float below = it.induced + direct - sa[y];
                    if (below + ax < bestInc) {
                        const uint32_t l = t.left[y], r = t.right[y];
                        const float gl = area(unite(box[l], bx)) - sa[l], gr = area(unite(box[r], bx)) - sa[r];
                        if (gl <= gr) { todo.push_back(Item{r, it.depth + 1u, below}); todo.push_back(Item{l, it.depth + 1u, below}); }
                        else { todo.push_back(Item{l, it.depth + 1u, below}); todo.push_back(Item{r, it.depth + 1u, below}); }
                    }
                }
            }
            const uint32_t q = parent[best];
            replaceChild(q, best, p); t.left[p] = best; t.right[p] = x; parent[best] = p; parent[x] = p;
            refit(p);
        }
        const double now = totalCost();
        static const bool verbose = getenv("TB_REINSERT_VERBOSE") != nullptr;
        if (verbose) fprintf(stderr, "reinsertion pass %d: SAH cost %.6g -> %.6g\n", pass, cost, now);
        const bool goOn = now < cost * (1.0 - minGain);
        cost = now;
        if (!goOn) break;
    }
}

constexpr bool kWaveTreeByDefault = true;
constexpr uint32_t kWaveStageWaves = 24, kWaveStageFeelerPercent = 42, kWaveStageSeed = 0x7b01u, kWaveStagePasses = 4, kWaveStagePlaces = 3;

bool willBeLdsResident(const HostScene& s, uint32_t N, uint32_t depthNodes)
{
    if (!s.instances.empty() || !s.ldsSceneBudget) return false;
    return LdsSceneBytes(N > 1 ? N - 1 : 1, N, s.hitGroups.size(), s.indexBuffer.size(), s.vertexBuffer.size(), s.materials.size(), s.lights.size(),
        WalkStackDepth(depthNodes)) <= s.ldsSceneBudget;
}

void optimizeForWaves(const HostScene& s, Tree& t, HostScene::WaveStageReport& rep)
{
    const uint32_t N = t.N; if (N < 4) return;
    const auto started = std::chrono::steady_clock::now();
    const uint32_t M = 2 * N - 1, NONE = 0xffffffffu;
    auto isLeaf = [&](uint32_t x) { return x >= N - 1; };
    std::vector<tb3> lmn(N), lmx(N);
    WaveTree wt; wt.v0.resize(N); wt.v1.resize(N); wt.v2.resize(N);
    for (uint32_t k = 0; k < N; k++) { const Bounds b = boundsOfRef(s, t, t.order[k]); lmn[k] = b.mn; lmx[k] = b.mx;
        const uint32_t tri = triOfRef(t, t.order[k]); wt.v0[k] = P(s, tri, 0); wt.v1[k] = P(s, tri, 1); wt.v2[k] = P(s, tri, 2); }
    WaveSurfaces surf; WaveSurfacesOf(s, surf);
    std::vector<WaveRay> rays;
    WaveModelRays(surf, kWaveStageSeed, kWaveStageWaves, kWaveStageFeelerPercent, rays);
    if (rays.empty()) return;
    std::vector<char> arena;
    uint32_t depthNow = 0;
    auto price = [&]() { depthNow = WaveTreeFit(wt, N, t.left.data(), t.right.data(), lmn.data(), lmx.data()); rep.evaluations++;
        return WaveCostOfTree(wt, rays, kLdsSceneParkMin, arena); };
    WaveTrips cur = price();
    const uint32_t d0 = depthNow, image = (uint32_t)LdsImageBytes(N - 1, N);
    const bool sixFit = LdsCopyFits(6, WalkStackDepth(d0), image);
    auto depthOk = [&](uint32_t d) { return d <= (d0 <= 31u ? 31u : (d0 <= 39u ? 39u : d0)) && willBeLdsResident(s, N, d) &&
        (!sixFit || LdsCopyFits(6, WalkStackDepth(d), image)); };
    uint32_t depthLimit = d0; while (depthOk(depthLimit + 1)) depthLimit++;
    rep.ran = 1; rep.rays = (uint32_t)rays.size(); rep.seed = kWaveStageSeed; rep.parkMin = kLdsSceneParkMin; rep.depthLimit = depthLimit;
    rep.innerBefore = cur.inner; rep.leafBefore = cur.leaf; rep.costBefore = cur.cost();

    std::vector<uint32_t> parent(M, NONE);
    for (uint32_t i = 0; i + 1 < N; i++) { parent[t.left[i]] = i; parent[t.right[i]] = i; }
    std::vector<Bounds> box(M); std::vector<float> sa(M);
    std::vector<uint32_t> pre, st;
    auto refitBelow = [&](uint32_t root) {
        pre.clear(); st.clear(); st.push_back(root);
        while (!st.empty()) { const uint32_t x = st.back(); st.pop_back(); pre.push_back(x); if (!isLeaf(x)) { st.push_back(t.left[x]); st.push_back(t.right[x]); } }
        for (size_t w = pre.size(); w-- > 0;) { const uint32_t x = pre[w];
            if (isLeaf(x)) { Bounds b; b.mx = lmx[x - (N - 1)]; b.mn = tb3_min(lmn[x - (N - 1)], b.mx - tb3_splat(0.001f)); box[x] = b; }
            else { box[x] = box[t.left[x]]; grow(box[x], box[t.right[x]]); }
            sa[x] = area(box[x]); } };
    auto replaceChild = [&](uint32_t p, uint32_t from, uint32_t to) { if (t.left[p] == from) t.left[p] = to; else t.right[p] = to; parent[to] = p; };
    struct Place { float induced; uint32_t node; };
    std::vector<Place> places; std::vector<uint32_t> cand(M - 1), inTree;
    for (uint32_t pass = 0; pass < kWaveStagePasses; pass++) {
        bool moved = false;
        refitBelow(0);
        for (uint32_t x = 1; x < M; x++) cand[x - 1] = x;
        std::stable_sort(cand.begin(), cand.end(), [&](uint32_t a, uint32_t b) { return sa[a] > sa[b]; });
        for (uint32_t x : cand) {
            const uint32_t p = parent[x]; if (p == NONE || p == 0) continue;
            const uint32_t g = parent[p], oldLeft = t.left[p], oldRight = t.right[p], sib = oldLeft == x ? oldRight : oldLeft;
            const bool pWasLeft = t.left[g] == p;
            replaceChild(g, p, sib); parent[p] = NONE;
            refitBelow(x); const Bounds bx = box[x];
            refitBelow(0); inTree = pre;
            places.clear();
            for (uint32_t y : inTree) { if (y == 0 || y == sib) continue;
                Bounds u = box[y]; grow(u, bx); float induced = area(u);
                for (uint32_t a = parent[y]; a != NONE; a = parent[a]) { Bounds w = box[a]; grow(w, bx); induced += area(w) - sa[a]; }
                places.push_back(Place{induced, y}); }
            std::stable_sort(places.begin(), places.end(), [](const Place& a, const Place& b) { return a.induced < b.induced; });
            uint32_t best = NONE; WaveTrips bestTrips = cur;
            for (size_t k = 0; k < places.size() && k < kWaveStagePlaces; k++) {
                const uint32_t y = places[k].node, q = parent[y];
                replaceChild(q, y, p); t.left[p] = y; t.right[p] = x; parent[y] = p; parent[x] = p;
                const WaveTrips tr = price();
                if (depthNow <= depthLimit && tr.cost() < bestTrips.cost()) { best = y; bestTrips = tr; }
                replaceChild(q, p, y); parent[p] = NONE;
            }
            if (best != NONE) {
                const uint32_t q = parent[best];
                replaceChild(q, best, p); t.left[p] = best; t.right[p] = x; parent[best] = p; parent[x] = p;
                cur = bestTrips; moved = true; rep.moves++;
            } else {
                if (pWasLeft) t.left[g] = p; else t.right[g] = p;
                parent[p] = g; t.left[p] = oldLeft; t.right[p] = oldRight; parent[sib] = p; parent[x] = p;
            }
        }
        if (!moved) break;
    }
    rep.innerAfter = cur.inner; rep.leafAfter = cur.leaf; rep.costAfter = cur.cost();
    rep.milliseconds = std::chrono::duration<double, std::milli>(std::chrono::steady_clock::now() - started).count();
}

struct TreeletPass {
    const uint32_t N; std::vector<uint32_t>&left, &right;
    std::vector<Bounds> box;
    static float sarea(const Bounds& b) { const tb3 d = b.mx - b.mn; return 2.0f * (d.x * d.y + d.x * d.z + d.y * d.z); }
    bool leaf(uint32_t x) const { return x >= N - 1; }

    void rebuild(uint32_t root)
    {
        uint32_t leafNode[7], inner[6]; Bounds sub[128]; float cost[128]; uint8_t cut[128];
        inner[0] = root; leafNode[0] = left[root]; leafNode[1] = right[root];
        for (uint32_t n = 2; n < 7; n++) {
            float best = 0.0f; uint32_t at = 0, node = 0;
            for (uint32_t i = 0; i < n; i++) if (!leaf(leafNode[i])) { const float a = sarea(box[leafNode[i]]); if (a > best) { best = a; at = i;
                node = leafNode[i]; } }
            inner[n - 1] = node; leafNode[at] = left[node]; leafNode[n] = right[node];
        }
        const float rootArea = sarea(box[root]);
        for (uint32_t m = 1; m < 128; m++) {
            const uint32_t low = (uint32_t)__builtin_ctz(m), rest = m & (m - 1);
            sub[m] = box[leafNode[low]]; if (rest) grow(sub[m], sub[rest]);
            cost[m] = rest ? sarea(sub[m]) : sarea(sub[m]) / rootArea;
        }
        static uint8_t bySize[8][35]; static uint8_t sizeCount[8]; static bool tables = false;
        if (!tables) { for (uint32_t m = 1; m < 128; m++) { const int k = __builtin_popcount(m); bySize[k][sizeCount[k]++] = (uint8_t)m; } tables = true; }
        for (int k = 2; k <= 7; k++) for (uint32_t q = 0; q < sizeCount[k]; q++) {
            const uint32_t m = bySize[k][q], d = (m - 1) & m;
            float least = 3.402823466e+38f; uint32_t arg = 0;
            uint32_t p = (0u - d) & m;
            do { const float c = cost[p] + cost[m ^ p]; if (c < least) { least = c; arg = p; } p = (p - d) & m; } while (p);
            cost[m] += least; cut[m] = (uint8_t)arg;
        }
        uint32_t used = 1; struct Todo { uint32_t mask, node; } todo[7]; uint32_t n = 0; todo[n++] = {127u, root};
        while (n) {
            const Todo t = todo[--n];
            const uint32_t lm = cut[t.mask], rm = t.mask ^ lm; uint32_t ln, rn;
            if (lm & (lm - 1)) { ln = inner[used++]; todo[n++] = {lm, ln}; } else ln = leafNode[__builtin_ctz(lm)];
            if (rm & (rm - 1)) { rn = inner[used++]; todo[n++] = {rm, rn}; } else rn = leafNode[__builtin_ctz(rm)];
            left[t.node] = ln; right[t.node] = rn;
        }
        for (int j = 5; j >= 0; j--) { const uint32_t x = inner[j]; box[x] = box[left[x]]; grow(box[x], box[right[x]]); }
    }

    void run(uint32_t minTris, const std::vector<Bounds>& leafBox)
    {
        const uint32_t M = 2 * N - 1;
        std::vector<uint32_t> pre; pre.reserve(M); { std::vector<uint32_t> st(1, 0u); while (!st.empty()) { const uint32_t x = st.back(); st.pop_back();
            pre.push_back(x); if (!leaf(x)) { st.push_back(left[x]); st.push_back(right[x]); } } }
        std::vector<uint32_t> tris(M, 0); std::vector<uint8_t> done(M, 0);
        for (size_t w = pre.size(); w-- > 0;) {
            const uint32_t x = pre[w];
            if (leaf(x)) { box[x] = leafBox[x - (N - 1)]; tris[x] = 1; continue; }
            const uint32_t l = left[x], r = right[x];
            box[x] = box[l]; grow(box[x], box[r]); tris[x] = tris[l] + tris[r];
            if (tris[x] < minTris) continue;
            uint32_t fewest = 0xffu; bool everyGroupCame = true, anyBig = false;
            for (uint32_t c : {l, r}) if (tris[c] >= minTris) { anyBig = true; if (!done[c]) everyGroupCame = false;
                else fewest = std::min<uint32_t>(fewest, done[c]); }
            if (!anyBig) done[x] = 1; else if (everyGroupCame && fewest < 33) done[x] = (uint8_t)(fewest + 1);
            if (done[x]) rebuild(x);
        }
    }
};

void treeletPasses(const HostScene& s, Tree& t, uint32_t passes)
{
    const uint32_t N = t.N; if (N < 7) return;
    std::vector<Bounds> leafBox(N);
    for (uint32_t k = 0; k < N; k++) {
        Bounds b = emptyB(); for (int v = 0; v < 3; v++) grow(b, P(s, t.order[k], v));
        b.mn = tb3_min(b.mn, b.mx - tb3_splat(0.001f));
        const tb3 c = (b.mn + b.mx) * 0.5f, h = b.mx - c;
        leafBox[k].mn = c - h; leafBox[k].mx = c + h;
    }
    TreeletPass tp{N, t.left, t.right, std::vector<Bounds>(2 * (size_t)N - 1)};
    uint32_t minTris = 7;
    for (uint32_t i = 0; i < passes && minTris <= N; i++, minTris *= 2) tp.run(minTris, leafBox);
}

void BuildBvhSingle(HostScene& s, int builder)
{
    const uint64_t N64 = s.triGeometry.size();
    if (N64 == 0) throw std::runtime_error("BuildBvh: no triangles");
    if (N64 > 0x00ffffffull) throw std::runtime_error("BuildBvh: more than 2^24-1 triangles does not fit the 24-bit node indices of the reference layout");
    Tree t; t.N = (uint32_t)N64;
    if (builder == 1 && s.presplitPercent > 0) presplitReferences(s, t, s.presplitPercent);
    if (t.N > 0x00ffffffu) throw std::runtime_error("BuildBvh: more than 2^24-1 references after pre-splitting (lower option presplit)");
    const uint32_t N = t.N;
    if (builder == 1) {
        buildSah(s, t);
        const int passes = s.reinsertionPasses >= 0 ? s.reinsertionPasses : (N <= 4096 ? 16 : 3);
        if (passes > 0) optimizeByReinsertion(s, t, passes, N <= 4096 ? 1e-6 : 5e-3);
        s.waveStage = HostScene::WaveStageReport{};
        const bool waveStage = s.waveTree >= 0 ? s.waveTree != 0 : (kWaveTreeByDefault && passes > 0);
        if (waveStage && N >= 4) {
            std::vector<tb3> mn(N, tb3_splat(0.0f)); WaveTree probe;
            const uint32_t depth = WaveTreeFit(probe, N, t.left.data(), t.right.data(), mn.data(), mn.data());
            if (willBeLdsResident(s, N, depth)) optimizeForWaves(s, t, s.waveStage);
        }
    } else {
        buildLbvh(s, t);
        if (builder == 3) treeletPasses(s, t, 3);
    }

    const uint64_t numNodes = 2ull * N - 1;
    const uint64_t offBoxes = 16, offPrims = offBoxes + 32 * numNodes, offMeta = offPrims + 40ull * N, total = offMeta + 12ull * N;
    if (total > 0xffffffffull) throw std::runtime_error("BuildBvh: BVH image exceeds 4 GiB");
    s.bvhA.assign((size_t)total, 0);
    TbBvhHeader hdr = {(uint32_t)offBoxes, (uint32_t)offPrims, (uint32_t)offMeta, (uint32_t)total};
    memcpy(s.bvhA.data(), &hdr, 16);
    TbAabbNode* nodes = (TbAabbNode*)(s.bvhA.data() + offBoxes);
    uint8_t* prims = s.bvhA.data() + offPrims;
    TbPrimitiveMeta* meta = (TbPrimitiveMeta*)(s.bvhA.data() + offMeta);
    s.trisB.resize(N);
    for (uint32_t k = 0; k < N; k++) {
        uint32_t tri = triOfRef(t, t.order[k]);
        TbPrimitive p; p.PrimitiveType = 1;
        TbTriB tbv;
        for (int v = 0; v < 3; v++) {
            tb3 q = P(s, tri, v);
            float* d = v == 0 ? p.v0 : (v == 1 ? p.v1 : p.v2); d[0] = q.x; d[1] = q.y; d[2] = q.z;
            float* e = v == 0 ? tbv.v0 : (v == 1 ? tbv.v1 : tbv.v2); e[0] = q.x; e[1] = q.y; e[2] = q.z;
        }
        memcpy(prims + 40ull * k, &p, 40);
        meta[k].GeometryContributionToHitGroupIndex = s.triGeometry[tri];
        meta[k].PrimitiveIndex = s.triPrimitive[tri];
        meta[k].GeometryFlags = s.triFlags[tri];
        tbv.geometryIndex = s.triGeometry[tri]; tbv.primitiveIndex = s.triPrimitive[tri]; tbv.geometryFlags = s.triFlags[tri];
        s.trisB[k] = tbv;
    }
    std::vector<uint32_t> walk; walk.reserve((size_t)numNodes);
    std::vector<uint32_t> depth((size_t)numNodes, 0);
    { std::vector<uint32_t> st; st.push_back(0); depth[0] = 1; uint32_t maxD = 1;
      while (!st.empty()) { uint32_t x = st.back(); st.pop_back(); walk.push_back(x);
          if (N > 1 && x < N - 1) { uint32_t l = t.left[x], r = t.right[x]; depth[l] = depth[r] = depth[x] + 1; if (depth[l] > maxD) maxD = depth[l];
              st.push_back(l); st.push_back(r); } }
      s.bvhMaxDepth = maxD; }
    std::vector<uint32_t> count((size_t)numNodes, 0);
    auto center = [&](uint32_t i) { return tb3_make(nodes[i].center[0], nodes[i].center[1], nodes[i].center[2]); };
    auto half = [&](uint32_t i) { return tb3_make(nodes[i].halfDim[0], nodes[i].halfDim[1], nodes[i].halfDim[2]); };
    auto put = [&](uint32_t i, tb3 mn, tb3 mx, uint32_t fx, uint32_t fy) {
        tb3 c = (mn + mx) * 0.5f, h = mx - c;
        nodes[i].center[0] = c.x; nodes[i].center[1] = c.y; nodes[i].center[2] = c.z; nodes[i].flags = fx;
        nodes[i].halfDim[0] = h.x; nodes[i].halfDim[1] = h.y; nodes[i].halfDim[2] = h.z; nodes[i].rightNodeIndex = fy;
    };
    for (size_t w = walk.size(); w-- > 0;) {
        uint32_t x = walk[w];
        if (x >= N - 1) {
            uint32_t k = x - (N - 1);
            const Bounds rb = boundsOfRef(s, t, t.order[k]);
            tb3 mn = rb.mn, mx = rb.mx;
// ... 223 lines not shown
```

### tracerboy_amd/csrc/host/context_scene.cpp

```cpp
#include "context_internal.h"
#include "lds_image.h"

namespace tbctx {

void releaseScene(tb_context* c)
{
    c->sceneBufs.clear();
    c->dyn.reset();
    c->bake.reset();
    c->probes.reset();
    c->wn.reset();
    memset(&c->ds, 0, sizeof c->ds);
}

uint32_t sceneFeatureMask(const HostScene& s)
{
    uint32_t f = 0;
    if (!s.envMap.empty()) f |= PT_FEAT_ENV;
    for (const TbMaterial& m : s.materials) {
        if ((m.Flags & TB_MAT_NO_SPECULAR) == 0 && (m.Flags & TB_MAT_MIX) == 0) f |= PT_FEAT_SPECULAR;
        if (m.albedoIndex != TB_INVALID_TEXTURE || m.emissiveIndex != TB_INVALID_TEXTURE || m.specularMapIndex != TB_INVALID_TEXTURE ||
            m.normalMapIndex != TB_INVALID_TEXTURE) f |= PT_FEAT_TEXTURES | PT_FEAT_SPECULAR;
        if (m.Flags & TB_MAT_SUBSURFACE_SCATTER) f |= PT_FEAT_SSS;
        if (m.Flags & TB_MAT_MIX) f |= PT_FEAT_MIX;
// ... 70 lines not shown
        else for (uint32_t x : level) dfs(x);
    }
    for (uint32_t i = 0; i < (uint32_t)order.size(); i++) if (order[i] != PAD) newIndex[order[i]] = i;
    std::vector<TbNodeB> out(order.size());
    for (uint32_t i = 0; i < (uint32_t)order.size(); i++) {
        if (order[i] == PAD) { memset(&out[i], 0, sizeof(TbNodeB)); out[i].left = out[i].right = TB_BVH_LEAF_FLAG; continue; }
        TbNodeB nd = s.nodesB[order[i]];
        if (inner(nd.left)) nd.left = newIndex[nd.left];
        if (inner(nd.right)) nd.right = newIndex[nd.right];
        out[i] = nd;
    }
    s.nodesB.swap(out);
    s.rootRefB = 0;
}

void BuildBvhGpu(tb_context* c, HostScene& s, uint32_t treeletPasses)
{
    const uint64_t N64 = s.triGeometry.size();
    if (N64 == 0) throw std::runtime_error("BuildBvh: no triangles");
    if (N64 > 0x00ffffffull) throw std::runtime_error("BuildBvh: more than 2^24-1 triangles does not fit the 24-bit node indices of the reference layout");
    if (s.blueNoise0.empty()) LoadBlueNoiseTiles(s);
    const uint32_t N = (uint32_t)N64;
    const uint64_t nodes = 2ull * N - 1, total = 16 + 32 * nodes + 52ull * N;
    if (total > 0xffffffffull) throw std::runtime_error("BuildBvh: BVH image exceeds 4 GiB");
    DevBuf dPos, dIdx, dGeo, dPrim, dFlag, dA, dNodes, dTris, dScratch, dHeight;
    auto up = [&](DevBuf& b, const void* p, size_t bytes) { ensure(b, bytes); HIP_TRY(hipMemcpyAsync(b.p, p, bytes, hipMemcpyHostToDevice, c->stream)); };
    up(dPos, s.positions.data(), s.positions.size() * 4); up(dIdx, s.triVertexIndex.data(), s.triVertexIndex.size() * 4);
    up(dGeo, s.triGeometry.data(), 4ull * N); up(dPrim, s.triPrimitive.data(), 4ull * N); up(dFlag, s.triFlags.data(), 4ull * N);
    const size_t nB = N > 1 ? N - 1 : 1, scratchBytes = bvh_gpu_scratch_bytes(N);
    ensure(dA, total); ensure(dNodes, nB * sizeof(TbNodeB)); ensure(dTris, (size_t)N * sizeof(TbTriB)); ensure(dScratch, scratchBytes); ensure(dHeight, 4);
    HIP_TRY(hipMemsetAsync(dNodes.p, 0, nB * sizeof(TbNodeB), c->stream));
    HIP_TRY(bvh_gpu_build(c->stream, (const float*)dPos.p, (const uint32_t*)dIdx.p, (const uint32_t*)dGeo.p, (const uint32_t*)dPrim.p,
        (const uint32_t*)dFlag.p, N,
                          treeletPasses, (uint8_t*)dScratch.p, scratchBytes, (uint8_t*)dA.p, (TbNodeB*)dNodes.p, (TbTriB*)dTris.p, (uint32_t*)dHeight.p));
    s.bvhA.resize((size_t)total); s.nodesB.resize(nB); s.trisB.resize(N);
    HIP_TRY(hipMemcpy(s.bvhA.data(), dA.p, total, hipMemcpyDeviceToHost));
    HIP_TRY(hipMemcpy(s.nodesB.data(), dNodes.p, nB * sizeof(TbNodeB), hipMemcpyDeviceToHost));
    HIP_TRY(hipMemcpy(s.trisB.data(), dTris.p, (size_t)N * sizeof(TbTriB), hipMemcpyDeviceToHost));
    HIP_TRY(hipMemcpy(&s.bvhMaxDepth, dHeight.p, 4, hipMemcpyDeviceToHost));
    s.rootRefB = N == 1 ? TB_BVH_LEAF_FLAG : 0u;
}

void buildCompactNodes(const HostScene& s, std::vector<TbNodeC>& out, TbQuantFrame& q, uint32_t nodeUnits)
{
    double lo[3] = {1e300, 1e300, 1e300}, hi[3] = {-1e300, -1e300, -1e300};
    auto grow = [&](const float* cc, const float* hh, int k) { for (int a = 0; a < 3; a++) { lo[a] = std::min(lo[a], (double)cc[a * 2 + k] - hh[a * 2 + k]);
        hi[a] = std::max(hi[a], (double)cc[a * 2 + k] + hh[a * 2 + k]); } };
    auto boxOf = [](const TbNodeB& n, float* cc, float* hh) {
        cc[0] = n.cx[0]; cc[1] = n.cx[1]; cc[2] = n.cy[0]; cc[3] = n.cy[1]; cc[4] = n.cz[0]; cc[5] = n.cz[1];
        hh[0] = n.hx[0]; hh[1] = n.hx[1]; hh[2] = n.hy[0]; hh[3] = n.hy[1]; hh[4] = n.hz[0]; hh[5] = n.hz[1];
    };
    auto isPad = [](const TbNodeB& n) { return n.left == TB_BVH_LEAF_FLAG && n.right == TB_BVH_LEAF_FLAG && n.hx[0] == 0.0f && n.hx[1] == 0.0f && n.cx[0] ==
        0.0f && n.cx[1] == 0.0f; };
    for (const TbNodeB& n : s.nodesB) { if (isPad(n)) continue; float cc[6], hh[6]; boxOf(n, cc, hh); grow(cc, hh, 0); grow(cc, hh, 1); }
    double ext = 0; for (int a = 0; a < 3; a++) ext = std::max(ext, hi[a] - lo[a]);
    if (!(ext > 0)) ext = 1.0;
    for (int a = 0; a < 3; a++) {
        const double e = std::max(hi[a] - lo[a], ext * 1e-6);
        q.cell[a] = (float)(e * 1.004 / 65535.0);
        q.origin[a] = (float)(lo[a] - 0.002 * e);
        for (int guard = 0; guard < 64 && !((double)q.origin[a] + 2.0 * (double)q.cell[a] <= lo[a]); guard++) q.origin[a] = std::nextafter(q.origin[a],
            -std::numeric_limits<float>::infinity());
    }
    out.assign(s.nodesB.size(), TbNodeC{});
    auto ref = [nodeUnits](uint32_t r) { return (r & TB_BVH_LEAF_FLAG) ? (TB_BVH_LEAF_FLAG | ((r & ~TB_BVH_LEAF_FLAG) * 3u)) : r * nodeUnits; };
    for (size_t i = 0; i < s.nodesB.size(); i++) {
        const TbNodeB& n = s.nodesB[i]; TbNodeC& o = out[i];
        o.left = ref(n.left); o.right = ref(n.right);
        if (isPad(n)) continue;
        float cc[6], hh[6]; boxOf(n, cc, hh);
        for (int a = 0; a < 3; a++) for (int k = 0; k < 2; k++) {
            const double bl = ((double)cc[a * 2 + k] - hh[a * 2 + k] - q.origin[a]) / q.cell[a],
                bh = ((double)cc[a * 2 + k] + hh[a * 2 + k] - q.origin[a]) / q.cell[a];
            long ql = (long)std::floor(bl - 0.125), qh = (long)std::ceil(bh + 0.125);
            if (ql < 0 || qh > 65535 || !(bl == bl) || !(bh == bh)) throw std::runtime_error("compact nodes: a box lies outside the quantisation grid");
            const long cq = (ql + qh) >> 1, hq = qh - cq;
            o.c[a][k] = (uint16_t)cq; o.h[a][k] = (uint16_t)hq;
        }
    }
}

void ensureCompactNodes(tb_context* c)
{
    if (c->compactTried || c->ds.nodesC) return;
    c->compactTried = true;
    refreshHostScene(c);
    const HostScene& s = c->scene;
    if (!s.instances.empty() || (s.rootRefB & TB_BVH_LEAF_FLAG)) return;
    try {
        std::vector<TbNodeC> compact;
        buildCompactNodes(s, compact, c->ds.quant, 2u);
        c->ds.nodesC = upload(c, compact);
    } catch (const std::exception&) { c->ds.nodesC = nullptr; }
}

void BuildTlasGpu(tb_context* c, HostScene& s, const std::vector<float>& blasBoxes, std::vector<TbNodeB>& top, uint32_t& rootRef, uint32_t& depth)
{
    const uint32_t M = (uint32_t)s.instances.size();
    std::vector<float> o2w(12ull * M), w2o(12ull * M); std::vector<uint32_t> blas(M), base(M);
    for (uint32_t i = 0; i < M; i++) { memcpy(&o2w[12ull * i], s.instances[i].objectToWorld, 48); memcpy(&w2o[12ull * i], s.instances[i].worldToObject, 48);
        blas[i] = s.instances[i].blas; base[i] = s.instances[i].hitGroupBase; }
    const size_t total = 16 + 32 * (2ull * M - 1) + 116ull * M, scratchBytes = bvh_gpu_tlas_scratch_bytes(M);
    DevBuf dO, dW, dB, dH, dBox, dScratch, dA, dTop, dWords;
    auto up = [&](DevBuf& b, const void* p, size_t bytes) { ensure(b, bytes); HIP_TRY(hipMemcpyAsync(b.p, p, bytes, hipMemcpyHostToDevice, c->stream)); };
    up(dO, o2w.data(), o2w.size() * 4); up(dW, w2o.data(), w2o.size() * 4); up(dB, blas.data(), 4ull * M); up(dH, base.data(), 4ull * M);
        up(dBox, blasBoxes.data(), blasBoxes.size() * 4);
    ensure(dScratch, scratchBytes); ensure(dA, total); ensure(dTop, std::max<size_t>(1, M - 1) * sizeof(TbNodeB)); ensure(dWords, 8);
    HIP_TRY(hipMemsetAsync(dA.p, 0, total, c->stream));
    HIP_TRY(bvh_gpu_build_tlas(c->stream, M, (const float*)dO.p, (const float*)dW.p, (const uint32_t*)dB.p, (const uint32_t*)dH.p, (const float*)dBox.p,
        (uint8_t*)dScratch.p, scratchBytes,
                               (uint8_t*)dA.p, (TbNodeB*)dTop.p, (uint32_t*)dWords.p, (uint32_t*)dWords.p + 1));
    s.tlasA.resize(total); top.assign(M > 1 ? M - 1 : 0, TbNodeB{});
    uint32_t words[2];
    HIP_TRY(hipMemcpy(s.tlasA.data(), dA.p, total, hipMemcpyDeviceToHost));
    if (M > 1) HIP_TRY(hipMemcpy(top.data(), dTop.p, (size_t)(M - 1) * sizeof(TbNodeB), hipMemcpyDeviceToHost));
    HIP_TRY(hipMemcpy(words, dWords.p, 8, hipMemcpyDeviceToHost));
    rootRef = words[0]; depth = words[1];
}

uint32_t sceneTextureUse(const tb_context* c)
{
    const int64_t* hint = c->options.ifSet<OPT_texture_use_hint>();
    if (hint && *hint == 0) return 3u;
    uint32_t use = 0;
    for (const TbMaterial& m : c->scene.materials) {
        if (m.albedoIndex != TB_INVALID_TEXTURE || m.emissiveIndex != TB_INVALID_TEXTURE || m.specularMapIndex != TB_INVALID_TEXTURE ||
            m.alphaIndex != TB_INVALID_TEXTURE) use |= 1u;
        if (m.normalMapIndex != TB_INVALID_TEXTURE) use |= 2u;
    }
    return use;
}

void finalizeScene(tb_context* c, bool build)
{
    HostScene& s = c->scene;
    c->sceneGeneration++;
    {
        uint64_t walks = 0;
        if (s.instances.empty())
            for (uint32_t g : s.triGeometry) { if (g < s.hitGroups.size()) { const uint32_t m = s.hitGroups[g].MaterialIndex;
                if (m < s.materials.size() && (s.materials[m].Flags & TB_MAT_SUBSURFACE_SCATTER)) walks++; } }
        c->interiorWalkTriangleShare = s.triGeometry.empty() ? 0.0f : (float)((double)walks / (double)s.triGeometry.size());
    }
    {
        uint32_t maxPrim = 0;
        for (uint32_t q : s.triPrimitive) maxPrim = std::max(maxPrim, q);
        auto bitsFor = [](uint64_t maxValue) { uint32_t b = 1; while (b < 32 && (maxValue >> b)) b++; return b; };
        c->hitPrimBits = bitsFor(maxPrim); c->hitGeomBits = bitsFor(s.hitGroups.empty() ? 0 : s.hitGroups.size() - 1);
    }
    const int64_t builder = opt<OPT_bvh_builder>(c);
    const bool twoLevel = !s.instances.empty();
    s.reinsertionPasses = (int)opt<OPT_reinsertion_passes>(c); s.reinsertionShare = (int)opt<OPT_reinsertion_share>(c);
    s.presplitPercent = (int)std::max<int64_t>(0, std::min<int64_t>(400, opt<OPT_presplit>(c)));
    s.waveTree = (int)opt<OPT_wave_tree>(c);
    s.ldsSceneBudget = opt<OPT_scene_in_lds>(c) != 0 ? (uint32_t)std::max<int64_t>(0, std::min<int64_t>(0x7fffffff, opt<OPT_lds_scene_budget>(c))) : 0u;
    if (build) {
    if (twoLevel && (builder == 2 || builder == 4))
        BuildBvhWith(s, [&](HostScene& one) { BuildBvhGpu(c, one, builder == 4 ? 3u : 0u); },
                     [&](HostScene& all, const std::vector<float>& boxes, std::vector<TbNodeB>& top, uint32_t& rootRef, uint32_t& depth) { BuildTlasGpu(c, all,
                         boxes, top, rootRef, depth); });
    else if (twoLevel) BuildBvh(s, (int)builder);
    else if (builder == 2 || builder == 4) BuildBvhGpu(c, s, builder == 4 ? 3u : 0u);
    else BuildBvh(s, (int)builder);
    if (!twoLevel) reorderNodes(s, (int)opt<OPT_node_order>(c), (uint32_t)opt<OPT_node_order_top_levels>(c));
    }
    c->camera = s.camera;
    releaseScene(c);
    TbDeviceScene& d = c->ds;
    if (s.nodesB.size() > 0x7fffffffull / 5 || s.trisB.size() > 0x7fffffffull / 3) throw std::runtime_error("scene too large for 31-bit device child refs");
    auto deviceRef = [](uint32_t ref,
        uint32_t nodeUnits) { return (ref & TB_BVH_LEAF_FLAG) ? (TB_BVH_LEAF_FLAG | ((ref & ~TB_BVH_LEAF_FLAG) * 3u)) : ref * nodeUnits; };
    {
        std::vector<TbNodeB> dev(s.nodesB);
        const size_t topNodes = s.instances.size() > 1 ? s.instances.size() - 1 : 0;
        auto topRef = [](uint32_t ref) { return (ref & TB_BVH_LEAF_FLAG) ? (TB_BVH_LEAF_FLAG | ((ref & ~TB_BVH_LEAF_FLAG) * 4u)) : ref * 4u; };
        for (size_t i = 0; i < dev.size(); i++) {
            TbNodeB& nd = dev[i];
            if (i < topNodes) { nd.left = topRef(nd.left); nd.right = topRef(nd.right); } else { nd.left = deviceRef(nd.left, 4);
                nd.right = deviceRef(nd.right, 4); }
        }
        d.nodes = upload(c, dev);
    }
    d.tris = upload(c, s.trisB);
    d.nodesC = nullptr; c->compactTried = false;
    d.rootRef = twoLevel ? ((s.rootRefB & TB_BVH_LEAF_FLAG) ? (TB_BVH_LEAF_FLAG | ((s.rootRefB & ~TB_BVH_LEAF_FLAG) * 4u)) : s.rootRefB * 4u) :
        deviceRef(s.rootRefB, 4);  d.numNodes = (uint32_t)s.nodesB.size(); d.numTris = (uint32_t)s.trisB.size();
    { const TbAabbNode* root = (const TbAabbNode*)((twoLevel ? s.tlasA.data() : s.bvhA.data()) + 16); memcpy(d.rootCenter, root->center, 12);
        memcpy(d.rootHalf, root->halfDim, 12); }
    {
        std::vector<TbInstanceB> devInst(s.instancesB);
        for (TbInstanceB& ib : devInst) ib.blasRootRef = deviceRef(ib.blasRootRef, 4);
        d.instances = upload(c, devInst); d.numInstances = (uint32_t)devInst.size();
    }
    std::vector<TbDevHitGroup> devHit(s.hitGroups.size());
    for (size_t i = 0; i < devHit.size(); i++) {
        if (s.hitGroups[i].VertexBufferOffset % 32 || s.hitGroups[i].IndexBufferOffset % 4)
            throw std::runtime_error("hit group buffer offsets must be vertex-/index-aligned");
        devHit[i] = TbDevHitGroup{s.hitGroups[i].MaterialIndex, s.hitGroups[i].VertexBufferOffset / 4, s.hitGroups[i].IndexBufferOffset / 4, 0};
    }
    std::vector<TbDevMaterial> devMat(s.materials.size());
    for (size_t i = 0; i < devMat.size(); i++) { memset(&devMat[i], 0, sizeof(TbDevMaterial)); devMat[i].m = s.materials[i]; }
    std::vector<TbDevLight> devLight(s.lights.size());
    for (size_t i = 0; i < devLight.size(); i++) { memset(&devLight[i], 0, sizeof(TbDevLight)); devLight[i].l = s.lights[i]; }
    d.hitGroups = upload(c, devHit); d.numHitGroups = (uint32_t)s.hitGroups.size();
    d.indexBuffer = upload(c, s.indexBuffer); d.numIndices = (uint32_t)s.indexBuffer.size();
    d.vertexBuffer = upload(c, s.vertexBuffer); d.numVertexFloats = (uint32_t)s.vertexBuffer.size();
    d.materials = upload(c, devMat); d.numMaterials = (uint32_t)s.materials.size();
    d.textureData = upload(c, s.textureData); d.numTextureData = (uint32_t)s.textureData.size();
    d.lights = upload(c, devLight); d.numLights = (uint32_t)s.lights.size();
    c->tablesInRange = SceneTablesInRange(s.trisB.data(), s.trisB.size(), devHit.data(), devHit.size(), s.indexBuffer.data(), s.indexBuffer.size(),
        s.vertexBuffer.size(), s.materials.size());
    d.images = upload(c, s.images); d.numImages = (uint32_t)s.images.size();
    d.texelPool = upload(c, s.texelPool);
    d.envMap = upload(c, s.envMap); d.envWidth = s.envWidth; d.envHeight = s.envHeight;
    d.blueNoise0 = upload(c, s.blueNoise0); d.blueNoise1 = upload(c, s.blueNoise1);
    d.config = s.config;
    d.stackDepth = WalkStackDepth(s.bvhMaxDepth);
    d.alphaTest = opt<OPT_alpha_test>(c) ? 1u : 0u;
    d.textureUse = sceneTextureUse(c);
    {
        size_t budget = (size_t)opt<OPT_lds_scene_budget>(c);
        c->sceneInLds = LdsSceneBytes(s.nodesB.size(), s.trisB.size(), devHit.size(), s.indexBuffer.size(), s.vertexBuffer.size(), devMat.size(),
            devLight.size(), d.stackDepth) <= budget && opt<OPT_scene_in_lds>(c) != 0 && !twoLevel;
        d.ldsBlob = nullptr; d.ldsBlobBytes = 0; d.offNodes = d.offTris = 0;
        if (c->sceneInLds) {
            const LdsImage image = BuildLdsImage(s.nodesB.data(), s.nodesB.size(), s.trisB.data(), s.trisB.size());
            d.ldsBlob = upload(c, image.bytes); d.ldsBlobBytes = (uint32_t)image.bytes.size(); d.offNodes = image.offNodes; d.offTris = image.offTris;
        }
        const int64_t* parkMin = c->options.ifSet<OPT_park_min>();
        d.parkMin = (uint32_t)std::max<int64_t>(1, parkMin ? *parkMin : (c->sceneInLds ? (int64_t)kLdsSceneParkMin : 24));
    }
    HIP_TRY(hipStreamSynchronize(c->stream));
    c->sceneFeatures = sceneFeatureMask(s);
    c->hasScene = true;
    resetHistory(c);
}

}
```

### tracerboy_amd/csrc/host/host_api.cpp

```cpp
#include "host_shared.h"
#include "launch_plan.h"
#include "lds_image.h"
#include "options.h"
#include "tb_state.h"
#include "wave_cost.h"
#include "../kernels/probe_launch.h"
#include "tb_nearest.h"
#include "winding_host.h"

#include <cmath>
#include <cstring>
#include <functional>
#include <memory>
#include <stdexcept>
#include <thread>

using namespace tbhost;
using namespace tbctx;

void tbctx::fillSceneInfo(const HostScene& s, tb_scene_info* o)
{
    memset(o, 0, sizeof *o);
    o->numTriangles = (uint32_t)s.triGeometry.size(); o->numVertices = (uint32_t)(s.positions.size() / 3); o->numMaterials = (uint32_t)s.materials.size();
    o->numLights = (uint32_t)s.lights.size(); o->numGeometries = (uint32_t)s.hitGroups.size(); o->numTextures = (uint32_t)s.textureData.size();
// ... 289 lines not shown
        std::unique_ptr<tb_host_scene> h(new tb_host_scene());
        std::string why;
        const int rc = MeshesToScene(*desc, h->scene, why);
        if (rc != TB_OK) return hostFail(err, errLen, rc, "tb_host_scene_from_meshes: " + why);
        applyBuilderWord(h->scene, builder); BuildBvh(h->scene, builderOfWord(builder));
        *out = h.release(); return TB_OK;
    } catch (const std::exception& e) { return hostFail(err, errLen, TB_E_INVALID, e.what()); }
}

int tb_host_smooth_normals(const float* positions, uint32_t nv, const uint32_t* indices, uint32_t nt, float* normalsOut)
{
    if ((nv && (!positions || !normalsOut)) || (nt && !indices)) return TB_E_INVALID;
    for (uint64_t i = 0; i < 3ull * nt; i++) if (indices[i] >= nv) return TB_E_INVALID;
    try { SmoothNormals(positions, nv, indices, nt, normalsOut); } catch (const std::exception&) { return TB_E_INVALID; }
    return TB_OK;
}

void tb_host_scene_free(tb_host_scene* s) { delete s; }

int tb_host_scene_view_get(tb_host_scene* s, TbSceneView* v) { if (!s || !v) return TB_E_INVALID; fillView(s->scene, v); return TB_OK; }
int tb_host_scene_digest(tb_host_scene* s, uint64_t* out) { if (!s || !out) return TB_E_INVALID; *out = sceneDigestOf(s->scene); return TB_OK; }
int tb_host_scene_camera(tb_host_scene* s, tb_camera* cam) { if (!s || !cam) return TB_E_INVALID; *cam = s->scene.camera; return TB_OK; }
int tb_host_scene_info(tb_host_scene* h, tb_scene_info* o)
{
    if (!h || !o) return TB_E_INVALID;
    fillSceneInfo(h->scene, o);
    return TB_OK;
}
int tb_host_scene_frame_constants(tb_host_scene* h, const tb_output_settings* settings, uint32_t frame, float t, TbPerFrameConstants* out)
{
    if (!h || !out) return TB_E_INVALID;
    tb_output_settings s; if (settings) s = *settings; else DefaultOutputSettings(s);
    MakeFrameConstants(h->scene, h->scene.camera, s, frame, t, 0xffffffffu, 0xffffffffu, *out);
    return TB_OK;
}
int tb_host_scene_layout_b(tb_host_scene* h, const TbNodeB** nodes, uint32_t* nn, const TbTriB** tris, uint32_t* nt, uint32_t* root)
{
    if (!h) return TB_E_INVALID;
    if (nodes) *nodes = h->scene.nodesB.data(); if (nn) *nn = (uint32_t)h->scene.nodesB.size();
    if (tris) *tris = h->scene.trisB.data(); if (nt) *nt = (uint32_t)h->scene.trisB.size();
    if (root) *root = h->scene.rootRefB;
    return TB_OK;
}
int tb_host_scene_lds_image(tb_host_scene* h, uint8_t* out, uint32_t capacity, tb_lds_image_info* info)
{
    if (!h || !info) return TB_E_INVALID;
    const HostScene& s = h->scene;
    memset(info, 0, sizeof *info);
    const size_t bytes = LdsImageBytes(s.nodesB.size(), s.trisB.size());
    if (bytes > 0x7fffffffull) return TB_E_UNSUPPORTED;
    info->bytes = (uint32_t)bytes; info->num_nodes = (uint32_t)s.nodesB.size(); info->num_tris = (uint32_t)s.trisB.size();
    info->node_stride = TB_LDS_NODE_STRIDE; info->tri_copies = TB_LDS_TRI_COPIES; info->root_ref = s.rootRefB;
    info->stack_depth = WalkStackDepth(s.bvhMaxDepth);
    if (!out) return TB_OK;
    if (capacity < bytes) return TB_E_INVALID;
    const LdsImage im = BuildLdsImage(s.nodesB.data(), s.nodesB.size(), s.trisB.data(), s.trisB.size());
    info->off_nodes = im.offNodes; info->off_tris = im.offTris;
    memcpy(out, im.bytes.data(), im.bytes.size());
    return TB_OK;
}
int tb_host_scene_tables_in_range(const TbTriB* tris, uint32_t numTris, const uint32_t* hitGroups, uint32_t numHitGroups, const uint32_t* indices,
    uint32_t numIndices, uint32_t numVertexFloats, uint32_t numMaterials)
{
    if ((numTris && !tris) || (numHitGroups && !hitGroups) || (numIndices && !indices)) return TB_E_INVALID;
    std::vector<TbDevHitGroup> hg(numHitGroups);
    for (uint32_t i = 0; i < numHitGroups; i++) hg[i] = TbDevHitGroup{hitGroups[4 * i], hitGroups[4 * i + 1], hitGroups[4 * i + 2], 0};
    return SceneTablesInRange(tris, numTris, hg.data(), hg.size(), indices, numIndices, numVertexFloats, numMaterials) ? 1 : 0;
}
int tb_host_scene_triangles(tb_host_scene* h, const float** pos, uint32_t* nv, const uint32_t** tvi, const uint32_t** tg, const uint32_t** tp,
    const uint32_t** tf, uint32_t* nt)
{
    if (!h) return TB_E_INVALID;
    const HostScene& s = h->scene;
    if (pos) *pos = s.positions.data(); if (nv) *nv = (uint32_t)(s.positions.size() / 3);
    if (tvi) *tvi = s.triVertexIndex.data(); if (tg) *tg = s.triGeometry.data(); if (tp) *tp = s.triPrimitive.data(); if (tf) *tf = s.triFlags.data();
    if (nt) *nt = (uint32_t)s.triGeometry.size();
    return TB_OK;
}

static void tripsOut(const WaveTrips& w, tb_wave_trips* o)
{
    o->inner_trips = w.inner; o->leaf_trips = w.leaf; o->idle_passes = w.idle; o->inner_active = w.innerActive; o->leaf_active = w.leafActive;
    o->cost = w.cost();
}
int tb_wave_replay(const char* const* steps, uint32_t lanes, uint32_t parkMin, tb_wave_trips* out)
{
    if (!out || lanes > kWaveLanes || (lanes && !steps)) return TB_E_INVALID;
    uint32_t len[kWaveLanes] = {};
    for (uint32_t l = 0; l < lanes; l++) { if (!steps[l]) return TB_E_INVALID; len[l] = (uint32_t)strlen(steps[l]);
        for (uint32_t k = 0; k < len[l]; k++) if (steps[l][k] != 'I' && steps[l][k] != 'L') return TB_E_INVALID; }
    tripsOut(WaveReplay(steps, len, lanes, parkMin), out);
    return TB_OK;
}
int tb_host_scene_wave_walk(tb_host_scene* h, uint32_t n, const float* origins, const float* dirs, const float* tMax, uint32_t* innerSteps,
    uint32_t* leafSteps, char* steps, uint64_t stepsCapacity)
{
    if (!h || (n && (!origins || !dirs))) return TB_E_INVALID;
    WaveTree w; if (!waveTreeOfScene(h->scene, w)) return TB_E_UNSUPPORTED;
    std::vector<char> one; uint64_t used = 0;
    for (uint32_t i = 0; i < n; i++) {
        WaveRay r; r.o = tb3_make(origins[3 * i], origins[3 * i + 1], origins[3 * i + 2]); r.d = tb3_make(dirs[3 * i], dirs[3 * i + 1], dirs[3 * i + 2]);
        r.tMax = tMax ? tMax[i] : kWaveMaxT; WaveRayPrepare(r);
        one.clear(); WaveWalk(w, r, one);
        uint32_t in = 0; for (char c : one) in += c == 'I' ? 1u : 0u;
        if (innerSteps) innerSteps[i] = in; if (leafSteps) leafSteps[i] = (uint32_t)one.size() - in;
        if (steps) {
            if (used + one.size() + 1 > stepsCapacity) return TB_E_INVALID;
            if (!one.empty()) memcpy(steps + used, one.data(), one.size());
            used += one.size(); steps[used++] = 0;
        }
    }
    return TB_OK;
}
static bool modelRaysOf(const HostScene& s, uint32_t seed, uint32_t waves, int feelerPercent, std::vector<WaveRay>& rays)
{
    uint32_t dSeed, dWaves, dFeelers, places; WaveStageSize(dSeed, dWaves, dFeelers, places);
    WaveSurfaces surf; WaveSurfacesOf(s, surf);
    WaveModelRays(surf, seed ? seed : dSeed, waves ? waves : dWaves, feelerPercent < 0 ? dFeelers : (uint32_t)std::min(feelerPercent, 100), rays);
    return !rays.empty();
}
int tb_host_scene_wave_rays(tb_host_scene* h, uint32_t seed, uint32_t waves, int feelerPercent, float* origins, float* dirs, float* tMax, uint32_t capacity)
{
    if (!h || waves > (1u << 16)) return TB_E_INVALID;
    std::vector<WaveRay> rays; modelRaysOf(h->scene, seed, waves, feelerPercent, rays);
    if (origins || dirs || tMax) {
        if (capacity < rays.size()) return TB_E_INVALID;
        for (size_t i = 0; i < rays.size(); i++) {
            if (origins) { origins[3 * i] = rays[i].o.x; origins[3 * i + 1] = rays[i].o.y; origins[3 * i + 2] = rays[i].o.z; }
            if (dirs) { dirs[3 * i] = rays[i].d.x; dirs[3 * i + 1] = rays[i].d.y; dirs[3 * i + 2] = rays[i].d.z; }
            if (tMax) tMax[i] = rays[i].tMax;
        }
    }
    return (int)rays.size();
}
int tb_host_scene_wave_cost(tb_host_scene* h, uint32_t seed, uint32_t waves, int feelerPercent, uint32_t parkMin, tb_wave_trips* out)
{
    if (!h || !out || waves > (1u << 16)) return TB_E_INVALID;
    WaveTree w; if (!waveTreeOfScene(h->scene, w)) return TB_E_UNSUPPORTED;
    std::vector<WaveRay> rays; if (!modelRaysOf(h->scene, seed, waves, feelerPercent, rays)) return TB_E_UNSUPPORTED;
    std::vector<char> arena;
    tripsOut(WaveCostOfTree(w, rays, parkMin ? parkMin : kLdsSceneParkMin, arena), out);
    return TB_OK;
}
int tb_host_scene_wave_stage(tb_host_scene* h, tb_wave_stage_info* o)
{
    if (!h || !o) return TB_E_INVALID;
    const HostScene::WaveStageReport& r = h->scene.waveStage;
    memset(o, 0, sizeof *o);
    o->ran = r.ran; o->rays = r.rays; o->seed = r.seed; o->park_min = r.parkMin; o->depth_limit = r.depthLimit; o->moves = r.moves;
    o->evaluations = r.evaluations; o->inner_insts = kWaveInnerInsts; o->leaf_insts = kWaveLeafInsts;
    o->before.inner_trips = r.innerBefore; o->before.leaf_trips = r.leafBefore; o->before.cost = r.costBefore;
    o->after.inner_trips = r.innerAfter; o->after.leaf_trips = r.leafAfter; o->after.cost = r.costAfter;
    o->milliseconds = r.milliseconds;
    return TB_OK;
}

static const char* nearestRefusal(uint32_t flags, uint64_t n, const void* points, const void* out, const tb_probe_grid* grid, bool isGrid)
{
    if (flags & ~(TB_NEAREST_SIGNED | TB_NEAREST_DEVICE)) return "unknown flag bits";
    if (!isGrid) {
        if (n > (1ull << 31)) return "more than 2^31 points";
        if (n && (!points || !out)) return "null pointer";
        if (n && (flags & TB_NEAREST_DEVICE)) {
            if ((uintptr_t)points & 15u) return "device points are not 16-B aligned";
            if ((uintptr_t)out & 15u) return "device records are not 16-B aligned";
        }
        return nullptr;
    }
    if (!grid) return "null grid";
    if (!grid->count[0] || !grid->count[1] || !grid->count[2]) return "a count of the grid is 0";
    if ((uint64_t)grid->count[0] * grid->count[1] > (1ull << 31) || (uint64_t)grid->count[0] * grid->count[1] * grid->count[2] > (1ull << 31))
        return "more than 2^31 cells";
    for (int k = 0; k < 3; k++) if (!(tb_abs(grid->origin[k]) < tb_u2f(0x7f800000u)) || !(tb_abs(grid->spacing[k]) < tb_u2f(0x7f800000u)))
        return "the grid's origin or spacing is not finite";
    if (!out) return "null pointer";
    if ((flags & TB_NEAREST_DEVICE) && ((uintptr_t)out & 3u)) return "the device distances are not 4-B aligned";
    return nullptr;
}

int tb_nearest_refusal(uint32_t flags, uint64_t n, const void* points, const void* out, const tb_probe_grid* grid, char* why, uint32_t whyBytes)
{
    const char* no = nearestRefusal(flags, n, points, out, grid, grid != nullptr);
    if (why && whyBytes) { strncpy(why, no ? no : "", whyBytes - 1); why[whyBytes - 1] = 0; }
    return no ? TB_E_INVALID : TB_OK;
}

namespace {

struct NearestBest { float d2 = tb_u2f(0x7f800000u); uint32_t geom = TB_NEAREST_NONE, prim = TB_NEAREST_NONE; float u = 0.0f, v = 0.0f; tb3 point{0.0f, 0.0f, 0.0f};
    bool behind = false; };

tb3 cornerOf(const float* v) { return tb3_make(v[0], v[1], v[2]); }

bool nearestOffer(NearestBest& best, tb3 p, float limit, const TbTriB& t)
{
    const tb3 v0 = cornerOf(t.v0), v1 = cornerOf(t.v1), v2 = cornerOf(t.v2);
    const TbNearestOnTriangle r = tb_nearest_on_triangle(p, v0, v1, v2);
    if (!(r.D2 <= limit) || !tb_nearest_better(r.D2, t.geometryIndex, t.primitiveIndex, best.d2, best.geom, best.prim)) return false;
    best.d2 = r.D2; best.geom = t.geometryIndex; best.prim = t.primitiveIndex; best.u = r.U; best.v = r.V; best.point = r.Point;
    best.behind = tb_nearest_behind(p, r.Point, v0, v1, v2);
    return true;
}

TbNearest nearestRecord(const NearestBest& best, bool isSigned)
{
    TbNearest o; memset(&o, 0, sizeof o);
    o.Distance = tb_u2f(0x7f800000u); o.Prim = o.Geom = TB_NEAREST_NONE;
    if (best.geom == TB_NEAREST_NONE && best.prim == TB_NEAREST_NONE) return o;
    const float d = tb_sqrt(best.d2);
    o.Point[0] = best.point.x; o.Point[1] = best.point.y; o.Point[2] = best.point.z;
    o.Distance = isSigned && best.behind ? -d : d; o.U = best.u; o.V = best.v; o.Prim = best.prim; o.Geom = best.geom;
    return o;
}

void rootBoxOf(const HostScene& s, tb3& c, tb3& h)
{
    const TbAabbNode* root = (const TbAabbNode*)(s.bvhA.data() + 16);
    c = cornerOf(root->center); h = cornerOf(root->halfDim);
}
tb3 childCentre(const TbNodeB& n, int k) { return tb3_make(n.cx[k], n.cy[k], n.cz[k]); }
tb3 childHalf(const TbNodeB& n, int k) { return tb3_make(n.hx[k], n.hy[k], n.hz[k]); }

NearestBest nearestWalk(const HostScene& s, tb3 p, float limit, std::vector<uint32_t>& stack)
{
    NearestBest best;
    tb3 rc, rh; rootBoxOf(s, rc, rh);
    const float slack = tb_nearest_slack(tb_nearest_scale(p, rc, rh));
    float cull = tb_nearest_cull(limit, slack);
    if (tb_box_d2(p, rc, rh) > cull) return best;
    stack.clear();
    uint32_t ref = s.rootRefB;
    for (;;) {
        if (!(ref & TB_BVH_LEAF_FLAG)) {
            const TbNodeB& n = s.nodesB[ref];
            const float dl = tb_box_d2(p, childCentre(n, 0), childHalf(n, 0)), dr = tb_box_d2(p, childCentre(n, 1), childHalf(n, 1));
            const bool lh = !(dl > cull), rh2 = !(dr > cull);
            if (lh && rh2) { const bool rightFirst = dr < dl; stack.push_back(rightFirst ? n.left : n.right); ref = rightFirst ? n.right : n.left; continue; }
            if (lh || rh2) { ref = rh2 ? n.right : n.left; continue; }
        } else if (nearestOffer(best, p, limit, s.trisB[ref & ~TB_BVH_LEAF_FLAG])) cull = tb_nearest_cull(best.d2, slack);
        if (stack.empty()) return best;
        ref = stack.back(); stack.pop_back();
    }
}

bool nearestSceneOk(const tb_host_scene* h) { return h && h->scene.instances.empty() && !h->scene.trisB.empty() && h->scene.bvhA.size() >= 48; }

}

int tb_host_scene_nearest(tb_host_scene* h, uint32_t flags, uint64_t n, const TbQueryPoint* points, TbNearest* out)
{
    const uint32_t form = flags & (TB_NEAREST_HOST_BRUTE | TB_NEAREST_HOST_WALK);
    if (!h || (flags & ~(TB_NEAREST_SIGNED | TB_NEAREST_HOST_BRUTE | TB_NEAREST_HOST_WALK)) || (form != TB_NEAREST_HOST_BRUTE && form != TB_NEAREST_HOST_WALK) ||
        (n && (!points || !out))) return TB_E_INVALID;
    if (!h->scene.instances.empty()) return TB_E_UNSUPPORTED;
    if (!nearestSceneOk(h)) return TB_E_INVALID;
    const HostScene& s = h->scene;
    auto range = [&](uint64_t first, uint64_t end) {
        std::vector<uint32_t> stack;
        for (uint64_t i = first; i < end; i++) {
            const tb3 p = cornerOf(points[i].Position);
            const float limit = tb_nearest_limit(points[i].MaxDistance);
            NearestBest best;
            if (tb_nearest_finite3(p) && limit >= 0.0f) {
                if (form == TB_NEAREST_HOST_WALK) best = nearestWalk(s, p, limit, stack);
                else for (const TbTriB& t : s.trisB) nearestOffer(best, p, limit, t);
            }
            out[i] = nearestRecord(best, (flags & TB_NEAREST_SIGNED) != 0);
        }
    };
    const uint64_t work = form == TB_NEAREST_HOST_BRUTE ? n * (uint64_t)s.trisB.size() : n * 64u;
    const uint64_t threads = work < (1ull << 22) ? 1u : std::min<uint64_t>(std::min<uint64_t>(8u, std::max(1u, std::thread::hardware_concurrency())), n);
    std::vector<std::thread> pool;
    uint64_t t = 0;
    try { for (; t + 1 < threads; t++) pool.emplace_back(range, n * t / threads, n * (t + 1) / threads); } catch (const std::exception&) {}
    range(n * t / threads, n);
    for (std::thread& th : pool) th.join();
    return TB_OK;
}

int tb_host_scene_nearest_excess(tb_host_scene* h, uint64_t n, const TbQueryPoint* points, float* worstOut)
{
    if (!h || !worstOut || (n && !points)) return TB_E_INVALID;
    if (!h->scene.instances.empty()) return TB_E_UNSUPPORTED;
    if (!nearestSceneOk(h)) return TB_E_INVALID;
    const HostScene& s = h->scene;
    std::vector<std::vector<std::pair<tb3, tb3>>> above(s.trisB.size());
    {
        tb3 rc, rh; rootBoxOf(s, rc, rh);
        std::vector<std::pair<tb3, tb3>> path(1, std::make_pair(rc, rh));
        std::function<void(uint32_t)> down = [&](uint32_t ref) {
            if (ref & TB_BVH_LEAF_FLAG) { above[ref & ~TB_BVH_LEAF_FLAG] = path; return; }
            const TbNodeB& nd = s.nodesB[ref];
            for (int k = 0; k < 2; k++) { path.push_back(std::make_pair(childCentre(nd, k), childHalf(nd, k))); down(k ? nd.right : nd.left); path.pop_back(); }
        };
        down(s.rootRefB);
    }
    double worst = 0.0;
    for (uint64_t i = 0; i < n; i++) {
        const tb3 p = cornerOf(points[i].Position);
        const float limit = tb_nearest_limit(points[i].MaxDistance);
        if (!tb_nearest_finite3(p) || !(limit >= 0.0f)) continue;
        NearestBest best; size_t winner = 0;
        for (size_t t = 0; t < s.trisB.size(); t++) if (nearestOffer(best, p, limit, s.trisB[t])) winner = t;
        if (best.geom == TB_NEAREST_NONE && best.prim == TB_NEAREST_NONE) continue;
        const double unit = (double)tb_nearest_scale(p, above[winner][0].first, above[winner][0].second) * 1.1920928955078125e-7;
        for (const auto& box : above[winner]) {
            const double excess = sqrt((double)tb_box_d2(p, box.first, box.second)) - sqrt((double)best.d2);
// ... 37 lines not shown
```

### tracerboy_amd/csrc/host/host_scene.h

```cpp
#pragma once
#include "../../../include/tb_abi.h"
#include "../../../include/tracerboy_hip.h"
#include "pbrt_scene.h"

#include <string>
#include <functional>
#include <vector>

namespace tbhost {

struct HostScene {
    tb_camera camera{};
    std::vector<TbMaterial> materials;
    std::vector<TbTextureData> textureData;
    std::vector<TbLight> lights;
    std::vector<TbHitGroupRecord> hitGroups;
    std::vector<float> vertexBuffer;
    std::vector<float> positions;
    std::vector<uint32_t> indexBuffer;
    std::vector<uint32_t> triVertexIndex , triGeometry, triPrimitive, triFlags;
    std::vector<TbImageDesc> images;
    std::vector<TbFloat4> texelPool;
    std::vector<TbFloat4> envMap; uint32_t envWidth = 0, envHeight = 0;
    std::vector<TbFloat4> blueNoise0, blueNoise1;
    TbConfigConstants config{};
    int filmWidth = 0, filmHeight = 0;
    float sceneMin[3] = {0, 0, 0}, sceneMax[3] = {0, 0, 0};
    struct Blas { uint32_t firstTri = 0, numTris = 0, offsetA = 0, rootRefB = 0, depth = 0; };
    struct Instance { uint32_t blas = 0; float objectToWorld[12]; float worldToObject[12]; uint32_t hitGroupBase = 0; };
    std::vector<Blas> blas;
    std::vector<Instance> instances;
    std::vector<uint8_t> tlasA;
    std::vector<uint32_t> blasOffsets;
    std::vector<TbInstanceB> instancesB;
    std::vector<uint8_t> bvhA;
    std::vector<TbNodeB> nodesB;
    std::vector<TbTriB> trisB;
    uint32_t rootRefB = 0;
    uint32_t bvhMaxDepth = 0;
    int reinsertionPasses = -1;
    int reinsertionShare = 100;
    int presplitPercent = 0;
    int waveTree = -1;
    uint32_t ldsSceneBudget = 40u * 1024u;
    struct WaveStageReport { uint32_t ran = 0, rays = 0, seed = 0, parkMin = 0, depthLimit = 0, moves = 0, evaluations = 0;
        uint64_t innerBefore = 0, leafBefore = 0, innerAfter = 0, leafAfter = 0; double costBefore = 0, costAfter = 0, milliseconds = 0; } waveStage;
};

struct ConvertOptions {
    bool flattenInstances = true;
    bool flipTextureUVs = true;
};

void ConvertScene(const PbrtScene& in, HostScene& out, const ConvertOptions& opt);

void BuildBvh(HostScene& scene, int builder);
typedef std::function<void(HostScene&, const std::vector<float>& blasRootBoxes, std::vector<TbNodeB>& topNodes, uint32_t& rootRef,
    uint32_t& depth)> TlasBuilder;
void BuildBvhWith(HostScene& scene, const std::function<void(HostScene&)>& single, const TlasBuilder& tlas);
void RebuildTopLevel(HostScene& scene, const TlasBuilder& tlas);
void InvertInstanceTransform(const float objectToWorld[12], float worldToObject[12]);
float InstanceTransformDeterminant(const float objectToWorld[12]);
struct WaveSurfaces;
void WaveSurfacesOf(const HostScene& scene, WaveSurfaces& out);
void WaveStageSize(uint32_t& seed, uint32_t& waves, uint32_t& feelerPercent, uint32_t& places);

void MakeProceduralScene(HostScene& out, int kind, uint32_t targetTriangles, uint32_t seed);
void SetLookAtCamera(HostScene& s, const float eye[3], const float target[3], float fovDeg);

std::string MeshesRefusal(const tb_scene_desc* desc);
std::string MeshesUnsupported(const tb_scene_desc& desc);
int MeshesToScene(const tb_scene_desc& desc, HostScene& out, std::string& why);
void SmoothNormals(const float* positions, uint32_t numVertices, const uint32_t* indices, uint32_t numTriangles, float* normalsOut);

bool WritePngRGBA8(const std::string& file, uint32_t W, uint32_t H, const uint8_t* rgba, std::string& err);
bool WritePfmRGB(const std::string& file, uint32_t W, uint32_t H, const float* rgba, std::string& err);
bool WriteExrRGBA(const std::string& file, uint32_t W, uint32_t H, const float* rgba, std::string& err);
bool LoadImageRGBA32F(const std::string& file, std::vector<TbFloat4>& texels, uint32_t& w, uint32_t& h, bool& normalizedFormat, std::string& err,
    bool* hasAlpha = nullptr);
inline bool ImageDimensionsOk(uint32_t w, uint32_t h) { return w >= 1 && h >= 1 && w <= 16384 && h <= 16384; }
struct DecodedImage { std::vector<TbFloat4> texels; uint32_t width = 0, height = 0; bool normalized = false, hasAlpha = false; };
bool DecodeImageFile(const std::string& file, DecodedImage& img, std::string& err);

bool LoadBlueNoiseTiles(HostScene& scene);

void DefaultOutputSettings(tb_output_settings& s);
void MakeFrameConstants(const HostScene& scene, const tb_camera& cam, const tb_output_settings& s, uint32_t frame, float timeSeed,
                        uint32_t selX, uint32_t selY, TbPerFrameConstants& out);

}
```

### tracerboy_amd/csrc/host/options.h

```cpp
#pragma once
#include <stdint.h>
#include <string.h>

namespace tbhost {

enum : uint32_t {
    OPT_NO_DEFAULT = 1u,
    OPT_RESETS_HISTORY = 2u,
    OPT_NOT_NEGATIVE = 4u, OPT_ZERO_OR_ONE = 8u,
};

#define TB_OPTIONS(X) \
    X(pipeline, 0, 0) X(frame_group, 0, 0) X(high_occupancy, 1, 0) X(stack_lds_cap, 0, 0) X(stack_overflow_max, 24, 0) X(node_layout, 0, 0) \
    X(primary_prepass, 1, 0) X(first_bounce, 0, 0) X(compact_hits, 1, 0) X(compact_stamp_bits, 32, 0) X(overlap_launches, 1, 0) \
    X(guided_groups, 1, 0) X(costly_first, 1, 0) X(costly_late_samples, 1ll << 40, 0) X(banded_items, 0, 0) X(camera_constants, 1, 0) \
    X(count_rays, 0, OPT_RESETS_HISTORY) X(aov, 0, OPT_RESETS_HISTORY) X(force_full_variant, 0, 0) X(debug_profile_groups, 0, 0) X(alpha_test, 0, 0) \
    X(debug_light_count, 0, OPT_RESETS_HISTORY | OPT_NOT_NEGATIVE)  \
    X(post_denoised, 0, 0)  \
    X(denoise_guides, 0, 0)  \
    X(sr_conv_form, 1, OPT_ZERO_OR_ONE)  \
    X(adaptive, 0, 0) X(adaptive_min_frames, 1024 , OPT_NOT_NEGATIVE) X(adaptive_test, 0, OPT_ZERO_OR_ONE) \
    X(wavefront_paths, 16ll << 20, 0) X(wavefront_grid, 256 * 8, 0) X(wavefront_segment, 4096, 0) X(wavefront_sort, 0, 0) X(wavefront_refill, 0, 0) \
    X(pooled_paths, 2, 0) X(pooled_samples, 256ll << 20, 0) X(pooled_profile, 0, 0) \
    X(split_trav, 4, 0) X(split_shade, 0, 0) X(split_ready, 32, 0) X(split_refill, 16, 0) X(split_wi, 85, 0) X(split_wl, 160, 0) \
    X(split_frame_group, 8, 0) X(split_stack_cap, 0, 0) X(split_spin_limit, 1 << 21, 0) X(split_profile, 0, 0) X(split_trav_last, 0, 0) \
    X(split_shade_prio, 0, 0) \
    X(bvh_builder, 0, 0) X(reinsertion_passes, -1, 0) X(reinsertion_share, 100, 0) X(presplit, 0, 0) X(wave_tree, -1, 0) X(node_order, 2, 0) \
    X(node_order_top_levels, 10, 0) X(scene_in_lds, 1, 0) X(lds_scene_budget, 40 * 1024, 0) \
    X(park_min, 0, OPT_NO_DEFAULT) X(flatten_instances, 0, OPT_NO_DEFAULT) X(flip_texture_uvs, 0, OPT_NO_DEFAULT) X(texture_use_hint, 0, OPT_NO_DEFAULT)

enum Opt {
#define X(name, def, flags) OPT_##name,
    TB_OPTIONS(X)
#undef X
    OPT_COUNT
};
struct OptionRow { const char* name; int64_t def; uint32_t flags; };
constexpr OptionRow kOptions[OPT_COUNT] = {
#define X(name, def, flags) {#name, def, flags},
    TB_OPTIONS(X)
#undef X
};
constexpr int64_t OptionDefault(Opt k) { return kOptions[k].def; }
inline int FindOption(const char* name) { for (int k = 0; k < OPT_COUNT; k++) if (!strcmp(kOptions[k].name, name)) return k; return -1; }

struct Options {
    int64_t value[OPT_COUNT] = {}; bool isSet[OPT_COUNT] = {};
    template <Opt K> int64_t get() const
    {
        static_assert(!(kOptions[K].flags & OPT_NO_DEFAULT), "this option has no constant default: ifSet<>() and the call site's fallback");
        return isSet[K] ? value[K] : kOptions[K].def;
    }
    template <Opt K> const int64_t* ifSet() const
    {
        static_assert((kOptions[K].flags & OPT_NO_DEFAULT) != 0, "this option has a default: get<>()");
        return isSet[K] ? &value[K] : nullptr;
    }
};

}
```

### tracerboy_amd/csrc/host/wave_cost.h

```cpp
#pragma once
#include <stdint.h>
#include <algorithm>
#include <cmath>
#include <vector>
#include "../../../include/tb_vec.h"

namespace tbhost {

constexpr uint32_t kWaveInnerInsts = 63, kWaveLeafInsts = 88;
constexpr float kWaveMinT = 0.001f, kWaveMaxT = 999999.0f;
constexpr uint32_t kWaveLanes = 64;

struct WaveTree {
    uint32_t N = 0;
    std::vector<tb3> center, half;
    std::vector<uint32_t> left, right;
    std::vector<tb3> v0, v1, v2;
};

inline uint32_t WaveTreeFit(WaveTree& w, uint32_t N, const uint32_t* left, const uint32_t* right, const tb3* leafMin, const tb3* leafMax)
{
    w.N = N;
    if (!N) return 0;
    const uint32_t M = 2 * N - 1;
    w.center.resize(M); w.half.resize(M); w.left.resize(N - 1); w.right.resize(N - 1);
    auto put = [&](uint32_t i, tb3 mn, tb3 mx) { const tb3 c = (mn + mx) * 0.5f; w.center[i] = c; w.half[i] = mx - c; };
    std::vector<uint32_t> walk, depth(M, 0), count(M, 0), st; walk.reserve(M);
    st.push_back(0); depth[0] = 1; uint32_t maxD = 1;
    while (!st.empty()) { const uint32_t x = st.back(); st.pop_back(); walk.push_back(x);
        if (x < N - 1) { const uint32_t l = left[x], r = right[x]; depth[l] = depth[r] = depth[x] + 1; maxD = std::max(maxD, depth[l]); st.push_back(l);
            st.push_back(r); } }
    for (size_t k = walk.size(); k-- > 0;) {
        const uint32_t x = walk[k];
        if (x >= N - 1) { const tb3 mx = leafMax[x - (N - 1)], mn = tb3_min(leafMin[x - (N - 1)], mx - tb3_splat(0.001f)); put(x, mn, mx); count[x] = 1; }
        else {
            uint32_t l = left[x], r = right[x];
            if (count[l] > count[r]) std::swap(l, r);
            put(x, tb3_min(w.center[l] - w.half[l], w.center[r] - w.half[r]), tb3_max(w.center[l] + w.half[l], w.center[r] + w.half[r]));
            w.left[x] = l; w.right[x] = r; count[x] = count[l] + count[r];
        }
    }
    return maxD;
}

struct WaveRay {
    tb3 o, d; float tMax;
    tb3 inv, oinv, ainv, shear; int kx, ky, kz; bool cannotHit;
};

inline void WaveRayPrepare(WaveRay& r)
{
    const tb3 o = r.o, d = r.d;
    r.cannotHit = tb_isnan(o.x) || tb_isnan(o.y) || tb_isnan(o.z) || tb_isnan(d.x) || tb_isnan(d.y) || tb_isnan(d.z);
    const float DEGEN_INV = 1.2089258196146292e24f, DEGEN_AINV = 1.2101064112353466e24f;
    r.inv = tb3_make(1.0f / d.x, 1.0f / d.y, 1.0f / d.z);
    r.oinv = o * r.inv;
    const tb3 a = tb3_abs(d);
    const int z = (a.x > a.y && a.x > a.z) ? 0 : (a.y > a.z ? 1 : 2);
    r.kx = (z + 1) % 3; r.ky = (z + 2) % 3; r.kz = z;
    r.ainv = tb3_abs(r.inv);
    if (d.x == 0.0f) { r.inv.x = DEGEN_INV; r.ainv.x = DEGEN_AINV; r.oinv.x = o.x * DEGEN_INV; }
    if (d.y == 0.0f) { r.inv.y = DEGEN_INV; r.ainv.y = DEGEN_AINV; r.oinv.y = o.y * DEGEN_INV; }
    if (d.z == 0.0f) { r.inv.z = DEGEN_INV; r.ainv.z = DEGEN_AINV; r.oinv.z = o.z * DEGEN_INV; }
    if (tb3_get(d, r.kz) < 0.0f) std::swap(r.kx, r.ky);
    r.shear = tb3_make(tb3_get(d, r.kx) / tb3_get(d, r.kz), tb3_get(d, r.ky) / tb3_get(d, r.kz), 1.0f / tb3_get(d, r.kz));
}

inline bool WaveBoxTest(float& resultT, float closest, const WaveRay& r, tb3 c, tb3 h)
{
    const tb3 mid = tb3_make(tb_fma(c.x, r.inv.x, -r.oinv.x), tb_fma(c.y, r.inv.y, -r.oinv.y), tb_fma(c.z, r.inv.z, -r.oinv.z));
    const tb3 maxL = tb3_make(tb_fma(h.x, r.ainv.x, mid.x), tb_fma(h.y, r.ainv.y, mid.y), tb_fma(h.z, r.ainv.z, mid.z));
    const tb3 minL = tb3_make(tb_fma(-h.x, r.ainv.x, mid.x), tb_fma(-h.y, r.ainv.y, mid.y), tb_fma(-h.z, r.ainv.z, mid.z));
    const float minT = tb_max(tb_max(minL.x, minL.y), minL.z), maxT = tb_min(tb_min(maxL.x, maxL.y), maxL.z);
    resultT = tb_max(minT, 0.0f);
    return resultT < tb_min(maxT, closest);
}

inline void WaveTriTest(float& hitT, const WaveRay& r, tb3 v0, tb3 v1, tb3 v2)
{
    const tb3 a0 = v0 - r.o, b0 = v1 - r.o, c0 = v2 - r.o;
    float Ax = tb3_get(a0, r.kx), Ay = tb3_get(a0, r.ky), Az = tb3_get(a0, r.kz);
    float Bx = tb3_get(b0, r.kx), By = tb3_get(b0, r.ky), Bz = tb3_get(b0, r.kz);
    float Cx = tb3_get(c0, r.kx), Cy = tb3_get(c0, r.ky), Cz = tb3_get(c0, r.kz);
    Ax = tb_fma(-r.shear.x, Az, Ax); Ay = tb_fma(-r.shear.y, Az, Ay);
    Bx = tb_fma(-r.shear.x, Bz, Bx); By = tb_fma(-r.shear.y, Bz, By);
    Cx = tb_fma(-r.shear.x, Cz, Cx); Cy = tb_fma(-r.shear.y, Cz, Cy);
    const float U = Cx * By - Cy * Bx, V = Ax * Cy - Ay * Cx, W = Bx * Ay - By * Ax;
    const float det = U + V + W;
    if ((U < 0.0f || V < 0.0f || W < 0.0f) && (U > 0.0f || V > 0.0f || W > 0.0f)) return;
    if (det == 0.0f) return;
    Az = r.shear.z * Az; Bz = r.shear.z * Bz; Cz = r.shear.z * Cz;
    const float T = tb_fma(W, Cz, tb_fma(V, Bz, U * Az));
    float sT = tb_abs(T);
    if ((T > 0.0f) != (det > 0.0f)) sT = -sT;
    if (sT < 0.0f || sT > hitT * tb_abs(det)) return;
    hitT = T * (1.0f / det);
}

constexpr int kWaveWalkStack = 256;

inline float WaveWalk(const WaveTree& t, const WaveRay& r, std::vector<char>& steps)
{
    float closest = r.tMax;
    if (!t.N || r.cannotHit) return closest;
    float unusedT;
    if (!WaveBoxTest(unusedT, closest, r, t.center[0], t.half[0])) return closest;
    uint32_t stack[kWaveWalkStack]; int top = 0; stack[top++] = 0;
    while (top) {
        const uint32_t node = stack[--top];
        if (node >= t.N - 1) {
            steps.push_back('L');
            const uint32_t k = node - (t.N - 1);
            float t0 = closest;
            WaveTriTest(t0, r, t.v0[k], t.v1[k], t.v2[k]);
            if (t0 < closest && t0 > kWaveMinT) closest = t0;
        } else {
            const uint32_t l = t.left[node], rr = t.right[node];
            float lt, rt;
            const bool lh = WaveBoxTest(lt, closest, r, t.center[l], t.half[l]), rh = WaveBoxTest(rt, closest, r, t.center[rr], t.half[rr]);
            steps.push_back('I');
            if (top + 2 > kWaveWalkStack) return closest;
            if (lh && rh) { const bool rightFirst = rt < lt; stack[top++] = rightFirst ? l : rr; stack[top++] = rightFirst ? rr : l; }
            else if (lh || rh) stack[top++] = rh ? rr : l;
        }
    }
    return closest;
}

struct WaveTrips {
    uint64_t inner = 0, leaf = 0, idle = 0;
    uint64_t innerActive = 0, leafActive = 0;
    double cost() const { return (double)inner * kWaveInnerInsts + (double)leaf * kWaveLeafInsts; }
    void add(const WaveTrips& o) { inner += o.inner; leaf += o.leaf; idle += o.idle; innerActive += o.innerActive; leafActive += o.leafActive; }
};

inline WaveTrips WaveReplay(const char* const* steps, const uint32_t* len, uint32_t lanes, uint32_t parkMin)
{
    WaveTrips w;
    if (lanes > kWaveLanes) lanes = kWaveLanes;
    if (parkMin < 1) parkMin = 1;
    uint32_t p[kWaveLanes] = {};
    auto at = [&](uint32_t l, char c) { return p[l] < len[l] && steps[l][p[l]] == c; };
    auto count = [&](char c) { uint32_t n = 0; for (uint32_t l = 0; l < lanes; l++) n += at(l, c) ? 1u : 0u; return n; };
    uint32_t inner = count('I');
    bool busy;
    do {
        if (inner) do {
            w.inner++; w.innerActive += inner;
            for (uint32_t l = 0; l < lanes; l++) if (at(l, 'I')) p[l]++;
            inner = count('I');
        } while (inner >= parkMin);
        const uint32_t leaf = count('L');
        busy = inner != 0 || leaf != 0;
        if (leaf) { w.leaf++; w.leafActive += leaf; for (uint32_t l = 0; l < lanes; l++) if (at(l, 'L')) p[l]++; }
        else w.idle++;
        inner = count('I');
    } while (busy);
    return w;
}

struct WaveSurfaces {
    std::vector<tb3> v;
    std::vector<uint8_t> emits;
    std::vector<tb3> light;
};

inline uint32_t WaveHash(uint32_t a, uint32_t b, uint32_t c)
{
    uint32_t h = a * 0x9e3779b1u ^ (b + 0x7f4a7c15u) * 0x85ebca6bu ^ (c + 0x165667b1u) * 0xc2b2ae35u;
    h ^= h >> 16; h *= 0x7feb352du; h ^= h >> 15; h *= 0x846ca68bu; h ^= h >> 16;
    return h;
}
inline float WaveUnit(uint32_t seed, uint32_t index, uint32_t dim) { return (float)(WaveHash(seed, index, dim) >> 8) * (1.0f / 16777216.0f); }

inline void WaveModelRays(const WaveSurfaces& s, uint32_t seed, uint32_t waves, uint32_t feelerPercent, std::vector<WaveRay>& rays)
{
    rays.clear();
    const size_t T = s.v.size() / 3, L = s.light.size() / 3;
    std::vector<double> cdf; std::vector<uint32_t> tri;
    double sum = 0;
    for (size_t i = 0; i < T; i++) {
        if (i < s.emits.size() && s.emits[i]) continue;
        const tb3 n = tb3_cross(s.v[3 * i + 1] - s.v[3 * i], s.v[3 * i + 2] - s.v[3 * i]);
        const double a = 0.5 * std::sqrt((double)n.x * n.x + (double)n.y * n.y + (double)n.z * n.z);
        if (!(a > 0.0)) continue;
        sum += a; cdf.push_back(sum); tri.push_back((uint32_t)i);
    }
    if (tri.empty()) return;
    const uint32_t feelerWaves = L ? (uint32_t)(((uint64_t)waves * feelerPercent + 50u) / 100u) : 0u;
    rays.reserve((size_t)waves * kWaveLanes);
    for (uint32_t wv = 0; wv < waves; wv++) {
        const bool feeler = (uint64_t)(wv + 1) * feelerWaves / waves != (uint64_t)wv * feelerWaves / waves;
        for (uint32_t lane = 0; lane < kWaveLanes; lane++) {
            const uint32_t i = wv * kWaveLanes + lane;
            const double pick = (double)WaveUnit(seed, i, 0) * sum;
            const size_t at = std::min<size_t>((size_t)(std::lower_bound(cdf.begin(), cdf.end(), pick) - cdf.begin()), tri.size() - 1);
            const tb3 a = s.v[3 * tri[at]], b = s.v[3 * tri[at] + 1], c = s.v[3 * tri[at] + 2];
            const float su = tb_sqrt(WaveUnit(seed, i, 1)), u2 = WaveUnit(seed, i, 2);
            const tb3 p = a * (1.0f - su) + b * (su * (1.0f - u2)) + c * (su * u2);
            tb3 n = tb3_normalize(tb3_cross(b - a, c - a));
            if (WaveHash(seed, i, 3) & 1u) n = -n;
            WaveRay r; r.o = p + n * 0.001f; r.tMax = kWaveMaxT;
            if (feeler) {
                const size_t li = (size_t)(WaveHash(seed, i, 4) % (uint32_t)L);
                const float sv = tb_sqrt(WaveUnit(seed, i, 5)), v2 = WaveUnit(seed, i, 6);
                const tb3 q = s.light[3 * li] * (1.0f - sv) + s.light[3 * li + 1] * (sv * (1.0f - v2)) + s.light[3 * li + 2] * (sv * v2);
                const tb3 to = q - r.o; const float dist = tb3_length(to);
                r.d = dist > 0.0f ? to * (1.0f / dist) : n;
            } else {
                const float e1 = WaveUnit(seed, i, 4), e2 = WaveUnit(seed, i, 5);
                const float rad = tb_sqrt(e1), phi = 6.2831853f * e2;
                const tb3 helper = tb_abs(n.x) < 0.5f ? tb3_make(1, 0, 0) : tb3_make(0, 1, 0);
                const tb3 t1 = tb3_normalize(tb3_cross(helper, n)), t2 = tb3_cross(n, t1);
                r.d = tb3_normalize(t1 * (rad * tb_cos(phi)) + t2 * (rad * tb_sin(phi)) + n * tb_sqrt(tb_max(0.0f, 1.0f - e1)));
            }
            WaveRayPrepare(r);
            rays.push_back(r);
        }
    }
}

inline WaveTrips WaveCostOfTree(const WaveTree& t, const std::vector<WaveRay>& rays, uint32_t parkMin, std::vector<char>& arena)
{
    WaveTrips total;
    const char* ptr[kWaveLanes]; uint32_t len[kWaveLanes]; size_t off[kWaveLanes + 1];
    for (size_t first = 0; first < rays.size(); first += kWaveLanes) {
        const uint32_t lanes = (uint32_t)std::min<size_t>(kWaveLanes, rays.size() - first);
        arena.clear();
        for (uint32_t l = 0; l < lanes; l++) { off[l] = arena.size(); WaveWalk(t, rays[first + l], arena); }
        off[lanes] = arena.size();
        const char* base = arena.empty() ? "" : arena.data();
        for (uint32_t l = 0; l < lanes; l++) { ptr[l] = base + off[l]; len[l] = (uint32_t)(off[l + 1] - off[l]); }
        total.add(WaveReplay(ptr, len, lanes, parkMin));
    }
    return total;
}

}
```

Measured before the change: 8645 Msamples/s.

## Expand host BVH wave-cost search with incremental repricing, threading and validation

Reworks the host-side BVH optimisation for the wave-traversal cost model. Candidate trees are now repriced incrementally by reusing recorded traversal visits and cached slab intervals, and only rays whose walks change are re-walked. A cost bound allows early abandonment, and the search can run on multiple threads. The search gets more passes and checks candidates against a separate validation ray set, and the lane replay uses bitmasks. The intent is a search that explores more candidates and finds a BVH with cheaper lockstep traversal on the GPU, at the cost of more host build complexity.

```diff
diff --git a/include/tracerboy_hip.h b/include/tracerboy_hip.h
--- a/include/tracerboy_hip.h
+++ b/include/tracerboy_hip.h
@@ -396,13 +396,19 @@
     uint32_t num_indices, uint32_t num_vertex_floats, uint32_t num_materials);
 typedef struct tb_wave_trips { uint64_t inner_trips, leaf_trips, idle_passes, inner_active, leaf_active; double cost; } tb_wave_trips;
 typedef struct tb_wave_stage_info { uint32_t ran, rays, seed, park_min, depth_limit, moves, evaluations, inner_insts, leaf_insts, reserved;
-    tb_wave_trips before, after; double milliseconds; } tb_wave_stage_info;
+    tb_wave_trips before, after; double milliseconds;
+    uint64_t places_priced, abandoned, rays_checked, rays_rewalked, places_screened;
+    uint32_t threads, passes, places, validation_rejects, cuts_skipped, screen_waves, screen_keep, reserved2;
+    double validation_before, validation_after;
+    } tb_wave_stage_info;
 int tb_wave_replay(const char* const* steps, uint32_t lanes, uint32_t park_min, tb_wave_trips* out);
 int tb_host_scene_wave_walk(tb_host_scene* s, uint32_t n, const float* origins, const float* dirs, const float* t_max, uint32_t* inner_steps,
     uint32_t* leaf_steps, char* steps, uint64_t steps_capacity);
 int tb_host_scene_wave_rays(tb_host_scene* s, uint32_t seed, uint32_t waves, int feeler_percent, float* origins, float* dirs, float* t_max, uint32_t capacity);
 int tb_host_scene_wave_cost(tb_host_scene* s, uint32_t seed, uint32_t waves, int feeler_percent, uint32_t park_min, tb_wave_trips* out);
 int tb_host_scene_wave_stage(tb_host_scene* s, tb_wave_stage_info* out);
+int tb_host_scene_wave_search(tb_host_scene* s, uint32_t seed, uint32_t waves, int feeler_percent, uint32_t places, uint32_t keep, int threads,
+    tb_wave_stage_info* out);
 int tb_host_pbrt_dump(const char* pbrt_path, const char* out_path, char* err, uint32_t err_len);
 int tb_host_scene_triangles(tb_host_scene* s, const float** positions, uint32_t* num_vertices, const uint32_t** tri_vertex_index,
                             const uint32_t** tri_geometry, const uint32_t** tri_primitive, const uint32_t** tri_flags, uint32_t* num_triangles);
diff --git a/tracerboy_amd/_ctypes_abi.py b/tracerboy_amd/_ctypes_abi.py
--- a/tracerboy_amd/_ctypes_abi.py
+++ b/tracerboy_amd/_ctypes_abi.py
@@ -300,7 +300,10 @@
 
 class tb_wave_stage_info(C.Structure):
     _fields_ = [(n, C.c_uint32) for n in ("ran", "rays", "seed", "park_min", "depth_limit", "moves", "evaluations", "inner_insts", "leaf_insts",
-                                          "reserved")] + [("before", tb_wave_trips), ("after", tb_wave_trips), ("milliseconds", C.c_double)]
+                                          "reserved")] + [("before", tb_wave_trips), ("after", tb_wave_trips), ("milliseconds", C.c_double)] + \
+               [(n, C.c_uint64) for n in ("places_priced", "abandoned", "rays_checked", "rays_rewalked", "places_screened")] + \
+               [(n, C.c_uint32) for n in ("threads", "passes", "places", "validation_rejects", "cuts_skipped", "screen_waves", "screen_keep", "reserved2")] + \
+               [("validation_before", C.c_double), ("validation_after", C.c_double)]
 
 
 class tb_state_info(C.Structure):
diff --git a/tracerboy_amd/api.py b/tracerboy_amd/api.py
--- a/tracerboy_amd/api.py
+++ b/tracerboy_amd/api.py
@@ -194,6 +194,7 @@
         "tb_host_scene_wave_rays": (C.c_int, [vp, C.c_uint32, C.c_uint32, C.c_int, P(C.c_float), P(C.c_float), P(C.c_float), C.c_uint32]),
         "tb_host_scene_wave_cost": (C.c_int, [vp, C.c_uint32, C.c_uint32, C.c_int, C.c_uint32, P(abi.tb_wave_trips)]),
         "tb_host_scene_wave_stage": (C.c_int, [vp, P(abi.tb_wave_stage_info)]),
+        "tb_host_scene_wave_search": (C.c_int, [vp, C.c_uint32, C.c_uint32, C.c_int, C.c_uint32, C.c_uint32, C.c_int, P(abi.tb_wave_stage_info)]),
     }
     for name, (res, args) in sig.items():
         fn = getattr(L, name)
@@ -1018,6 +1019,13 @@
             raise TracerBoyError(rc, "tb_host_scene_wave_stage")
         return info
 
+    def wave_search(self, seed=0, waves=0, feeler_percent=-1, places=0, keep=0, threads=0):
+        info = abi.tb_wave_stage_info()
+        rc = lib().tb_host_scene_wave_search(self._h, seed, waves, feeler_percent, places, keep, threads, C.byref(info))
+        if rc != 0:
+            raise TracerBoyError(rc, "tb_host_scene_wave_search")
+        return info
+
     def wave_rays(self, seed=0, waves=0, feeler_percent=-1):
         fp = C.POINTER(C.c_float)
         n = lib().tb_host_scene_wave_rays(self._h, seed, waves, feeler_percent, None, None, None, 0)
diff --git a/tracerboy_amd/csrc/host/bvh_build.cpp b/tracerboy_amd/csrc/host/bvh_build.cpp
--- a/tracerboy_amd/csrc/host/bvh_build.cpp
+++ b/tracerboy_amd/csrc/host/bvh_build.cpp
@@ -11,9 +11,14 @@
 #include <cstring>
 #include <cstdlib>
 #include <exception>
+#include <functional>
+#include <limits>
 #include <stdexcept>
 #include <thread>
 #include <mutex>
+#ifdef __linux__
+#include <sched.h>
+#endif
 
 namespace tbhost {
 
@@ -388,13 +393,149 @@
 }
 
 constexpr bool kWaveTreeByDefault = true;
-constexpr uint32_t kWaveStageWaves = 24, kWaveStageFeelerPercent = 42, kWaveStageSeed = 0x7b01u, kWaveStagePasses = 4, kWaveStagePlaces = 3;
+constexpr uint32_t kWaveStageWaves = 24, kWaveStageFeelerPercent = 42, kWaveStageSeed = 0x7b01u, kWaveStageValidationSeed = 0x2c9au;
+constexpr uint32_t kWaveStagePlaces = 0;
+constexpr uint32_t kWaveStagePasses = 12;
+constexpr uint32_t kWaveStagePassesByArea = 4;
+constexpr uint32_t kWaveStageMaxThreads = 16;
+constexpr uint32_t kWaveStageScreenWaves = 8, kWaveStageScreenKeep = 4;
 
 bool willBeLdsResident(const HostScene& s, uint32_t N, uint32_t depthNodes)
 {
     if (!s.instances.empty() || !s.ldsSceneBudget) return false;
     return LdsSceneBytes(N > 1 ? N - 1 : 1, N, s.hitGroups.size(), s.indexBuffer.size(), s.vertexBuffer.size(), s.materials.size(), s.lights.size(),
         WalkStackDepth(depthNodes)) <= s.ldsSceneBudget;
+}
+
+struct WaveBase {
+    WaveTree wt; uint32_t depth = 0;
+    std::vector<char> steps; std::vector<uint32_t> off , nI, nL; std::vector<uint64_t> visited;
+    WaveRecord rec; std::vector<uint32_t> visitOff;
+    std::vector<WaveTrips> wave; WaveTrips total;
+    std::vector<float> enter, leave;
+};
+
+struct WaveBoxKept {
+    const float* enter; const float* leave; const uint8_t* same;
+    bool operator()(float& resultT, float closest, const WaveTree& t, const WaveRay& r, uint32_t n) const
+    {
+        if (!same[n]) return WaveBoxTest(resultT, closest, r, t.center[n], t.half[n]);
+        resultT = enter[n];
+        return resultT < tb_min(leave[n], closest);
+    }
+};
+
+void waveBaseOf(WaveBase& b, uint32_t N, const uint32_t* left, const uint32_t* right, const tb3* lmn, const tb3* lmx, const std::vector<WaveRay>& rays,
+    uint32_t parkMin)
+{
+    b.depth = WaveTreeFit(b.wt, N, left, right, lmn, lmx);
+    const size_t R = rays.size(), W = (R + kWaveLanes - 1) / kWaveLanes;
+    b.steps.clear(); b.off.assign(R + 1, 0); b.nI.assign(R, 0); b.nL.assign(R, 0); b.visited.assign(2 * R, 0); b.wave.assign(W, WaveTrips{}); b.total = WaveTrips{};
+    b.rec.visits.clear(); b.rec.stacks.clear(); b.visitOff.assign(R + 1, 0);
+    for (size_t r = 0; r < R; r++) { b.off[r] = (uint32_t)b.steps.size(); b.visitOff[r] = (uint32_t)b.rec.visits.size();
+        WaveWalk(b.wt, rays[r], b.steps, &b.visited[2 * r], &b.rec); }
+    b.off[R] = (uint32_t)b.steps.size(); b.visitOff[R] = (uint32_t)b.rec.visits.size();
+    const size_t M = 2 * (size_t)N - 1;
+    b.enter.resize(R * M); b.leave.resize(R * M);
+    for (size_t r = 0; r < R; r++) for (size_t n = 0; n < M; n++) WaveBoxSlabs(b.enter[r * M + n], b.leave[r * M + n], rays[r], b.wt.center[n], b.wt.half[n]);
+    for (size_t r = 0; r < R; r++) { b.nI[r] = b.visitOff[r + 1] - b.visitOff[r]; b.nL[r] = b.off[r + 1] - b.off[r] - b.nI[r]; }
+    const char* base = b.steps.empty() ? "" : b.steps.data();
+    const char* ptr[kWaveLanes]; uint32_t len[kWaveLanes];
+    for (size_t w = 0; w < W; w++) {
+        const uint32_t lanes = (uint32_t)std::min<size_t>(kWaveLanes, R - w * kWaveLanes);
+        for (uint32_t l = 0; l < lanes; l++) { const size_t r = w * kWaveLanes + l; ptr[l] = base + b.off[r]; len[l] = b.off[r + 1] - b.off[r]; }
+        b.wave[w] = WaveReplay(ptr, len, lanes, parkMin); b.total.add(b.wave[w]);
+    }
+}
+
+struct WaveCandidate { WaveTrips trips; uint32_t depth = 0; bool priced = false, complete = false; uint64_t suspects = 0, rewalked = 0; };
+struct WaveScratch { WaveTree wt; std::vector<uint32_t> left, right, from; std::vector<char> arena; std::vector<uint8_t> differs, todo, sameBox; std::vector<double> floor; };
+
+inline bool sameBits(const tb3& a, const tb3& b) { return memcmp(&a, &b, sizeof(tb3)) == 0; }
+
+void waveCandidate(const WaveBase& b, WaveScratch& sc, uint32_t N, const tb3* lmn, const tb3* lmx, const std::vector<WaveRay>& rays, uint32_t parkMin,
+    uint32_t depthLimit, size_t waveLimit, const std::atomic<double>& bound, WaveCandidate& out)
+{
+    out = WaveCandidate{};
+    out.depth = WaveTreeFit(sc.wt, N, sc.left.data(), sc.right.data(), lmn, lmx);
+    if (out.depth > depthLimit) return;
+    out.priced = true;
+    const WaveTree& c = sc.wt; const WaveTree& o = b.wt;
+    const bool all = !sameBits(c.center[0], o.center[0]) || !sameBits(c.half[0], o.half[0]);
+    uint64_t changed[2] = {0, 0};
+    const size_t M = 2 * (size_t)N - 1;
+    sc.sameBox.resize(M);
+    for (size_t n = 0; n < M; n++) sc.sameBox[n] = sameBits(c.center[n], o.center[n]) && sameBits(c.half[n], o.half[n]) ? 1 : 0;
+    auto kept = [&](size_t r) { return WaveBoxKept{&b.enter[r * M], &b.leave[r * M], sc.sameBox.data()}; };
+    sc.differs.assign(N - 1, 0);
+    for (uint32_t i = 0; i + 1 < N; i++) { const uint32_t l = c.left[i], r = c.right[i];
+        if (l != o.left[i] || r != o.right[i] || !sameBits(c.center[l], o.center[l]) || !sameBits(c.half[l], o.half[l]) || !sameBits(c.center[r], o.center[r]) ||
+            !sameBits(c.half[r], o.half[r])) { sc.differs[i] = 1; WaveMaskSet(changed, i); } }
+    const size_t W = std::min(b.wave.size(), waveLimit), R = std::min(rays.size(), W * kWaveLanes);
+    constexpr uint32_t FROM_START = 0xffffffffu;
+    sc.todo.assign(R, 0); sc.from.resize(R); sc.floor.assign(W, -1.0);
+    double partial = 0;
+    for (size_t w = 0; w < W; w++) {
+        const size_t first = w * kWaveLanes, end = std::min(R, first + kWaveLanes);
+        bool any = false; uint32_t maxI = 0, maxL = 0;
+        for (size_t r = first; r < end; r++) {
+            if (all) { sc.todo[r] = 1; sc.from[r] = FROM_START; any = true; continue; }
+            if ((b.visited[2 * r] & changed[0]) || (b.visited[2 * r + 1] & changed[1])) {
+                out.suspects++;
+                for (uint32_t k = b.visitOff[r]; k < b.visitOff[r + 1]; k++) { const WaveVisit& v = b.rec.visits[k];
+                    if (!sc.differs[v.node]) continue;
+                    uint32_t walked, parked; WavePushesWith(kept(r), c, rays[r], v.node, v.closest, walked, parked);
+                    if (walked == v.first && parked == v.parked) continue;
+                    sc.todo[r] = 1; sc.from[r] = k; any = true; break; }
+                if (sc.todo[r]) continue;
+            }
+            maxI = std::max(maxI, b.nI[r]); maxL = std::max(maxL, b.nL[r]);
+        }
+        if (!any) { out.trips.add(b.wave[w]); partial += b.wave[w].cost(); }
+        else { sc.floor[w] = (double)maxI * kWaveInnerInsts + (double)maxL * kWaveLeafInsts; partial += sc.floor[w]; }
+    }
+    if (partial > bound.load(std::memory_order_relaxed)) return;
+    const char* keep = b.steps.empty() ? "" : b.steps.data();
+    const char* ptr[kWaveLanes]; uint32_t len[kWaveLanes]; size_t at[kWaveLanes + 1]; uint32_t stack[kWaveWalkStack];
+    for (size_t w = 0; w < W; w++) {
+        if (sc.floor[w] < 0.0) continue;
+        const size_t first = w * kWaveLanes; const uint32_t lanes = (uint32_t)(std::min(R, first + kWaveLanes) - first);
+        sc.arena.clear();
+        for (uint32_t l = 0; l < lanes; l++) { const size_t r = first + l; at[l] = sc.arena.size();
+            if (!sc.todo[r]) continue;
+            out.rewalked++;
+            if (sc.from[r] == FROM_START) { WaveWalk(c, rays[r], sc.arena); continue; }
+            const WaveVisit& v = b.rec.visits[sc.from[r]];
+            sc.arena.insert(sc.arena.end(), keep + b.off[r], keep + b.off[r] + v.step);
+            if (v.top) memcpy(stack, &b.rec.stacks[v.rest], v.top * sizeof(uint32_t));
+            stack[v.top] = v.node;
+            WaveWalkOnWith(kept(r), c, rays[r], stack, (int)v.top + 1, v.closest, sc.arena, at[l], nullptr, nullptr); }
+        at[lanes] = sc.arena.size();
+        const char* fresh = sc.arena.empty() ? "" : sc.arena.data();
+        bool same = true;
+        for (uint32_t l = 0; l < lanes; l++) { const size_t r = first + l;
+            if (!sc.todo[r]) { ptr[l] = keep + b.off[r]; len[l] = b.off[r + 1] - b.off[r]; continue; }
+            ptr[l] = fresh + at[l]; len[l] = (uint32_t)(at[l + 1] - at[l]);
+            if (same && (len[l] != b.off[r + 1] - b.off[r] || memcmp(ptr[l], keep + b.off[r], len[l]) != 0)) same = false; }
+        const WaveTrips tr = same ? b.wave[w] : WaveReplay(ptr, len, lanes, parkMin);
+        out.trips.add(tr); partial += tr.cost() - sc.floor[w];
+        if (partial > bound.load(std::memory_order_relaxed)) return;
+    }
+    out.complete = true;
+}
+
+
+uint32_t waveStageWorkers(int asked)
+{
+    unsigned n = 1;
+    if (asked >= 1) n = (unsigned)asked;
+    else {
+#ifdef __linux__
+        cpu_set_t set; CPU_ZERO(&set);
+        if (sched_getaffinity(0, sizeof set, &set) == 0) n = (unsigned)std::max(CPU_COUNT(&set), 1);
+#endif
+    }
+    return std::min<unsigned>(n, kWaveStageMaxThreads);
 }
 
 void optimizeForWaves(const HostScene& s, Tree& t, HostScene::WaveStageReport& rep)
@@ -403,26 +544,41 @@
     const auto started = std::chrono::steady_clock::now();
     const uint32_t M = 2 * N - 1, NONE = 0xffffffffu;
     auto isLeaf = [&](uint32_t x) { return x >= N - 1; };
+    const uint32_t placesLimit = s.waveSearchPlaces ? s.waveSearchPlaces : kWaveStagePlaces;
+    const bool byArea = placesLimit != 0;
+    const uint32_t maxPasses = byArea ? kWaveStagePassesByArea : kWaveStagePasses;
+    const uint32_t seed = s.waveSearchSeed ? s.waveSearchSeed : kWaveStageSeed, waves = s.waveSearchWaves ? s.waveSearchWaves : kWaveStageWaves;
+    const uint32_t feelers = s.waveSearchFeelerPercent < 0 ? kWaveStageFeelerPercent : (uint32_t)std::min(s.waveSearchFeelerPercent, 100);
     std::vector<tb3> lmn(N), lmx(N);
-    WaveTree wt; wt.v0.resize(N); wt.v1.resize(N); wt.v2.resize(N);
+    WaveTree tris; tris.v0.resize(N); tris.v1.resize(N); tris.v2.resize(N);
     for (uint32_t k = 0; k < N; k++) { const Bounds b = boundsOfRef(s, t, t.order[k]); lmn[k] = b.mn; lmx[k] = b.mx;
-        const uint32_t tri = triOfRef(t, t.order[k]); wt.v0[k] = P(s, tri, 0); wt.v1[k] = P(s, tri, 1); wt.v2[k] = P(s, tri, 2); }
+        const uint32_t tri = triOfRef(t, t.order[k]); tris.v0[k] = P(s, tri, 0); tris.v1[k] = P(s, tri, 1); tris.v2[k] = P(s, tri, 2); }
     WaveSurfaces surf; WaveSurfacesOf(s, surf);
-    std::vector<WaveRay> rays;
-    WaveModelRays(surf, kWaveStageSeed, kWaveStageWaves, kWaveStageFeelerPercent, rays);
+    std::vector<WaveRay> rays, check;
+    WaveModelRays(surf, seed, waves, feelers, rays);
     if (rays.empty()) return;
-    std::vector<char> arena;
-    uint32_t depthNow = 0;
-    auto price = [&]() { depthNow = WaveTreeFit(wt, N, t.left.data(), t.right.data(), lmn.data(), lmx.data()); rep.evaluations++;
-        return WaveCostOfTree(wt, rays, kLdsSceneParkMin, arena); };
-    WaveTrips cur = price();
-    const uint32_t d0 = depthNow, image = (uint32_t)LdsImageBytes(N - 1, N);
+    WaveModelRays(surf, kWaveStageValidationSeed, waves, feelers, check);
+    WaveBase base; base.wt = tris;
+    WaveTree checked = tris; std::vector<char> arena;
+    auto rebase = [&]() { waveBaseOf(base, N, t.left.data(), t.right.data(), lmn.data(), lmx.data(), rays, kLdsSceneParkMin); };
+    rep.evaluations++;
+    auto priceCheck = [&]() { WaveTreeFit(checked, N, t.left.data(), t.right.data(), lmn.data(), lmx.data());
+        return WaveCostOfTree(checked, check, kLdsSceneParkMin, arena).cost(); };
+    rebase();
+    WaveTrips cur = base.total;
+    double curCheck = priceCheck();
+    const uint32_t d0 = base.depth, image = (uint32_t)LdsImageBytes(N - 1, N);
     const bool sixFit = LdsCopyFits(6, WalkStackDepth(d0), image);
     auto depthOk = [&](uint32_t d) { return d <= (d0 <= 31u ? 31u : (d0 <= 39u ? 39u : d0)) && willBeLdsResident(s, N, d) &&
         (!sixFit || LdsCopyFits(6, WalkStackDepth(d), image)); };
     uint32_t depthLimit = d0; while (depthOk(depthLimit + 1)) depthLimit++;
-    rep.ran = 1; rep.rays = (uint32_t)rays.size(); rep.seed = kWaveStageSeed; rep.parkMin = kLdsSceneParkMin; rep.depthLimit = depthLimit;
+    rep.ran = 1; rep.rays = (uint32_t)rays.size(); rep.seed = seed; rep.parkMin = kLdsSceneParkMin; rep.depthLimit = depthLimit;
     rep.innerBefore = cur.inner; rep.leafBefore = cur.leaf; rep.costBefore = cur.cost();
+    rep.places = placesLimit; rep.validationBefore = curCheck;
+    const uint32_t workers = waveStageWorkers(s.waveTreeThreads);
+    rep.threads = workers;
+    std::vector<WaveScratch> scratch(workers);
+    for (WaveScratch& sc : scratch) sc.wt = tris;
 
     std::vector<uint32_t> parent(M, NONE);
     for (uint32_t i = 0; i + 1 < N; i++) { parent[t.left[i]] = i; parent[t.right[i]] = i; }
@@ -438,13 +594,32 @@
     auto replaceChild = [&](uint32_t p, uint32_t from, uint32_t to) { if (t.left[p] == from) t.left[p] = to; else t.right[p] = to; parent[to] = p; };
     struct Place { float induced; uint32_t node; };
     std::vector<Place> places; std::vector<uint32_t> cand(M - 1), inTree;
-    for (uint32_t pass = 0; pass < kWaveStagePasses; pass++) {
+    std::vector<WaveCandidate> priced, screened; std::vector<size_t> finalists;
+    const size_t screenWaves = !byArea && base.wave.size() > kWaveStageScreenWaves ? kWaveStageScreenWaves : 0;
+    const std::vector<WaveRay> screenRays(rays.begin(), rays.begin() + (s.waveSearchVerify ? std::min(rays.size(), screenWaves * kWaveLanes) : 0));
+    const uint32_t screenKeep = s.waveSearchKeep ? s.waveSearchKeep : kWaveStageScreenKeep;
+    rep.screenWaves = (uint32_t)screenWaves; rep.screenKeep = screenWaves ? screenKeep : 0;
+    auto forEach = [&](size_t count, const std::function<void(size_t, WaveScratch&)>& fn) {
+        std::atomic<size_t> next{0}; std::exception_ptr failed; std::mutex fm;
+        auto work = [&](WaveScratch& sc) {
+            try { for (size_t k = next++; k < count; k = next++) fn(k, sc); }
+            catch (...) { std::lock_guard<std::mutex> lock(fm); if (!failed) failed = std::current_exception(); next = count; } };
+        const size_t helpers = std::min<size_t>(workers, count);
+        if (helpers <= 1) work(scratch[0]);
+        else { std::vector<std::thread> th; for (size_t i = 1; i < helpers; i++) th.emplace_back(work, std::ref(scratch[i]));
+            work(scratch[0]); for (auto& one : th) one.join(); }
+        if (failed) std::rethrow_exception(failed); };
+    std::vector<uint32_t> triedAt(M, 0);
+    for (uint32_t pass = 0; pass < maxPasses; pass++) {
         bool moved = false;
+        rep.passes = pass + 1;
         refitBelow(0);
         for (uint32_t x = 1; x < M; x++) cand[x - 1] = x;
         std::stable_sort(cand.begin(), cand.end(), [&](uint32_t a, uint32_t b) { return sa[a] > sa[b]; });
         for (uint32_t x : cand) {
             const uint32_t p = parent[x]; if (p == NONE || p == 0) continue;
+            if (!byArea && triedAt[x] == rep.moves + 1u) { rep.cutsSkipped++; continue; }
+            triedAt[x] = rep.moves + 1u;
             const uint32_t g = parent[p], oldLeft = t.left[p], oldRight = t.right[p], sib = oldLeft == x ? oldRight : oldLeft;
             const bool pWasLeft = t.left[g] == p;
             replaceChild(g, p, sib); parent[p] = NONE;
@@ -456,19 +631,65 @@
                 for (uint32_t a = parent[y]; a != NONE; a = parent[a]) { Bounds w = box[a]; grow(w, bx); induced += area(w) - sa[a]; }
                 places.push_back(Place{induced, y}); }
             std::stable_sort(places.begin(), places.end(), [](const Place& a, const Place& b) { return a.induced < b.induced; });
-            uint32_t best = NONE; WaveTrips bestTrips = cur;
-            for (size_t k = 0; k < places.size() && k < kWaveStagePlaces; k++) {
-                const uint32_t y = places[k].node, q = parent[y];
+            if (byArea && places.size() > placesLimit) places.resize(placesLimit);
+            auto hang = [&](WaveScratch& sc, uint32_t y) { const uint32_t q = parent[y];
+                sc.left = t.left; sc.right = t.right;
+                if (sc.left[q] == y) sc.left[q] = p; else sc.right[q] = p;
+                sc.left[p] = y; sc.right[p] = x; };
+            auto verify = [&](WaveScratch& sc, const WaveCandidate& got, const std::vector<WaveRay>& over, double boundNow) {
+                if (!s.waveSearchVerify || !got.priced) return;
+                const WaveTrips plain = WaveCostOfTree(sc.wt, over, kLdsSceneParkMin, sc.arena);
+                if (got.complete ? plain.inner != got.trips.inner || plain.leaf != got.trips.leaf || plain.idle != got.trips.idle : !(plain.cost() > boundNow))
+                    throw std::logic_error("wave stage: a shortcut changed a price"); };
+            finalists.clear();
+            const bool screen = screenWaves && places.size() > screenKeep;
+            if (screen) {
+                screened.assign(places.size(), WaveCandidate{});
+                std::atomic<double> bound{std::numeric_limits<double>::infinity()}; std::mutex bm; std::vector<double> cheapest;
+                forEach(places.size(), [&](size_t k, WaveScratch& sc) {
+                    hang(sc, places[k].node);
+                    waveCandidate(base, sc, N, lmn.data(), lmx.data(), rays, kLdsSceneParkMin, depthLimit, screenWaves, bound, screened[k]);
+                    verify(sc, screened[k], screenRays, bound.load(std::memory_order_relaxed));
+                    if (!screened[k].complete) return;
+                    std::lock_guard<std::mutex> lock(bm);
+                    cheapest.insert(std::upper_bound(cheapest.begin(), cheapest.end(), screened[k].trips.cost()), screened[k].trips.cost());
+                    if (cheapest.size() > screenKeep) cheapest.pop_back();
+                    if (cheapest.size() == screenKeep) bound.store(cheapest.back(), std::memory_order_relaxed); });
+                for (size_t k = 0; k < places.size(); k++) { rep.evaluations++; if (!screened[k].priced) continue;
+                    rep.placesScreened++; rep.raysChecked += screened[k].suspects; rep.raysRewalked += screened[k].rewalked;
+                    if (!screened[k].complete) rep.abandoned++; else finalists.push_back(k); }
+                std::stable_sort(finalists.begin(), finalists.end(), [&](size_t a, size_t b) { return screened[a].trips.cost() < screened[b].trips.cost(); });
+                if (finalists.size() > screenKeep) finalists.resize(screenKeep);
+                std::sort(finalists.begin(), finalists.end());
+            } else for (size_t k = 0; k < places.size(); k++) finalists.push_back(k);
+            priced.assign(places.size(), WaveCandidate{});
+            {
+                std::atomic<double> bound{cur.cost()};
+                forEach(finalists.size(), [&](size_t f, WaveScratch& sc) { const size_t k = finalists[f];
+                    hang(sc, places[k].node);
+                    waveCandidate(base, sc, N, lmn.data(), lmx.data(), rays, kLdsSceneParkMin, depthLimit, base.wave.size(), bound, priced[k]);
+                    verify(sc, priced[k], rays, bound.load(std::memory_order_relaxed));
+                    if (priced[k].complete) { const double c = priced[k].trips.cost(); double seen = bound.load(std::memory_order_relaxed);
+                        while (c < seen && !bound.compare_exchange_weak(seen, c, std::memory_order_relaxed)) {} } });
+            }
+            size_t best = places.size(); double bestCost = cur.cost();
+            for (size_t k : finalists) { if (!screen) rep.evaluations++;  if (!priced[k].priced) continue;
+                rep.placesPriced++; rep.raysChecked += priced[k].suspects; rep.raysRewalked += priced[k].rewalked; if (!priced[k].complete) { rep.abandoned++; continue; }
+                if (priced[k].trips.cost() < bestCost) { best = k; bestCost = priced[k].trips.cost(); } }
+            bool keep = best != places.size();
+            if (keep) {
+                const uint32_t y = places[best].node, q = parent[y];
                 replaceChild(q, y, p); t.left[p] = y; t.right[p] = x; parent[y] = p; parent[x] = p;
-                const WaveTrips tr = price();
-                if (depthNow <= depthLimit && tr.cost() < bestTrips.cost()) { best = y; bestTrips = tr; }
-                replaceChild(q, p, y); parent[p] = NONE;
+                if (!byArea) { const double c = priceCheck();
+                    if (c > curCheck) { keep = false; rep.validationRejects++; replaceChild(q, p, y); parent[p] = NONE; } else curCheck = c; }
             }
-            if (best != NONE) {
-                const uint32_t q = parent[best];
-                replaceChild(q, best, p); t.left[p] = best; t.right[p] = x; parent[best] = p; parent[x] = p;
-                cur = bestTrips; moved = true; rep.moves++;
-            } else {
+            if (keep) {
+                rebase();
+                if (base.total.inner != priced[best].trips.inner || base.total.leaf != priced[best].trips.leaf || base.depth != priced[best].depth)
+                    throw std::logic_error("wave stage: a place was priced wrongly");
+                cur = base.total; moved = true; rep.moves++;
+            }
+            else {
                 if (pWasLeft) t.left[g] = p; else t.right[g] = p;
                 parent[p] = g; t.left[p] = oldLeft; t.right[p] = oldRight; parent[sib] = p; parent[x] = p;
             }
@@ -476,6 +697,7 @@
         if (!moved) break;
     }
     rep.innerAfter = cur.inner; rep.leafAfter = cur.leaf; rep.costAfter = cur.cost();
+    rep.validationAfter = byArea ? priceCheck() : curCheck;
     rep.milliseconds = std::chrono::duration<double, std::milli>(std::chrono::steady_clock::now() - started).count();
 }
 
diff --git a/tracerboy_amd/csrc/host/context_scene.cpp b/tracerboy_amd/csrc/host/context_scene.cpp
--- a/tracerboy_amd/csrc/host/context_scene.cpp
+++ b/tracerboy_amd/csrc/host/context_scene.cpp
@@ -246,7 +246,7 @@
     const bool twoLevel = !s.instances.empty();
     s.reinsertionPasses = (int)opt<OPT_reinsertion_passes>(c); s.reinsertionShare = (int)opt<OPT_reinsertion_share>(c);
     s.presplitPercent = (int)std::max<int64_t>(0, std::min<int64_t>(400, opt<OPT_presplit>(c)));
-    s.waveTree = (int)opt<OPT_wave_tree>(c);
+    s.waveTree = (int)opt<OPT_wave_tree>(c); s.waveTreeThreads = (int)std::min<int64_t>(opt<OPT_wave_tree_threads>(c), 1024);
     s.ldsSceneBudget = opt<OPT_scene_in_lds>(c) != 0 ? (uint32_t)std::max<int64_t>(0, std::min<int64_t>(0x7fffffff, opt<OPT_lds_scene_budget>(c))) : 0u;
     if (build) {
     if (twoLevel && (builder == 2 || builder == 4))
diff --git a/tracerboy_amd/csrc/host/host_api.cpp b/tracerboy_amd/csrc/host/host_api.cpp
--- a/tracerboy_amd/csrc/host/host_api.cpp
+++ b/tracerboy_amd/csrc/host/host_api.cpp
@@ -465,7 +465,20 @@
     o->before.inner_trips = r.innerBefore; o->before.leaf_trips = r.leafBefore; o->before.cost = r.costBefore;
     o->after.inner_trips = r.innerAfter; o->after.leaf_trips = r.leafAfter; o->after.cost = r.costAfter;
     o->milliseconds = r.milliseconds;
-    return TB_OK;
+    o->places_priced = r.placesPriced; o->abandoned = r.abandoned; o->rays_checked = r.raysChecked; o->rays_rewalked = r.raysRewalked; o->cuts_skipped = r.cutsSkipped;
+    o->places_screened = r.placesScreened; o->screen_waves = r.screenWaves; o->screen_keep = r.screenKeep; o->threads = r.threads; o->passes = r.passes;
+    o->places = r.places; o->validation_rejects = r.validationRejects; o->validation_before = r.validationBefore; o->validation_after = r.validationAfter;
+    return TB_OK;
+}
+int tb_host_scene_wave_search(tb_host_scene* h, uint32_t seed, uint32_t waves, int feelerPercent, uint32_t places, uint32_t keep, int threads, tb_wave_stage_info* out)
+{
+    if (!h || waves > (1u << 16) || threads < 0) return TB_E_INVALID;
+    HostScene& s = h->scene;
+    if (!s.instances.empty() || s.triGeometry.empty()) return TB_E_UNSUPPORTED;
+    s.waveTree = 1; s.waveSearchSeed = seed; s.waveSearchWaves = waves; s.waveSearchFeelerPercent = feelerPercent; s.waveSearchPlaces = places; s.waveSearchKeep = keep;
+    s.waveTreeThreads = threads;
+    try { BuildBvh(s, 1); } catch (const std::exception&) { return TB_E_INVALID; }
+    return out ? tb_host_scene_wave_stage(h, out) : TB_OK;
 }
 
 static const char* nearestRefusal(uint32_t flags, uint64_t n, const void* points, const void* out, const tb_probe_grid* grid, bool isGrid)
diff --git a/tracerboy_amd/csrc/host/host_scene.h b/tracerboy_amd/csrc/host/host_scene.h
--- a/tracerboy_amd/csrc/host/host_scene.h
+++ b/tracerboy_amd/csrc/host/host_scene.h
@@ -42,9 +42,15 @@
     int reinsertionShare = 100;
     int presplitPercent = 0;
     int waveTree = -1;
+    int waveTreeThreads = 0;
+    uint32_t waveSearchSeed = 0, waveSearchWaves = 0, waveSearchPlaces = 0, waveSearchKeep = 0 ; int waveSearchFeelerPercent = -1;
+    bool waveSearchVerify = false;
     uint32_t ldsSceneBudget = 40u * 1024u;
     struct WaveStageReport { uint32_t ran = 0, rays = 0, seed = 0, parkMin = 0, depthLimit = 0, moves = 0, evaluations = 0;
-        uint64_t innerBefore = 0, leafBefore = 0, innerAfter = 0, leafAfter = 0; double costBefore = 0, costAfter = 0, milliseconds = 0; } waveStage;
+        uint64_t innerBefore = 0, leafBefore = 0, innerAfter = 0, leafAfter = 0; double costBefore = 0, costAfter = 0, milliseconds = 0;
+        uint64_t placesPriced = 0, abandoned = 0, raysChecked = 0, raysRewalked = 0; uint32_t threads = 0, passes = 0, places = 0, validationRejects = 0, cutsSkipped = 0;
+        uint64_t placesScreened = 0; uint32_t screenWaves = 0, screenKeep = 0;
+        double validationBefore = 0, validationAfter = 0; } waveStage;
 };
 
 struct ConvertOptions {
diff --git a/tracerboy_amd/csrc/host/options.h b/tracerboy_amd/csrc/host/options.h
--- a/tracerboy_amd/csrc/host/options.h
+++ b/tracerboy_amd/csrc/host/options.h
@@ -25,7 +25,7 @@
     X(split_trav, 4, 0) X(split_shade, 0, 0) X(split_ready, 32, 0) X(split_refill, 16, 0) X(split_wi, 85, 0) X(split_wl, 160, 0) \
     X(split_frame_group, 8, 0) X(split_stack_cap, 0, 0) X(split_spin_limit, 1 << 21, 0) X(split_profile, 0, 0) X(split_trav_last, 0, 0) \
     X(split_shade_prio, 0, 0) \
-    X(bvh_builder, 0, 0) X(reinsertion_passes, -1, 0) X(reinsertion_share, 100, 0) X(presplit, 0, 0) X(wave_tree, -1, 0) X(node_order, 2, 0) \
+    X(bvh_builder, 0, 0) X(reinsertion_passes, -1, 0) X(reinsertion_share, 100, 0) X(presplit, 0, 0) X(wave_tree, -1, 0) X(wave_tree_threads, 0, OPT_NOT_NEGATIVE) X(node_order, 2, 0) \
     X(node_order_top_levels, 10, 0) X(scene_in_lds, 1, 0) X(lds_scene_budget, 40 * 1024, 0) \
     X(park_min, 0, OPT_NO_DEFAULT) X(flatten_instances, 0, OPT_NO_DEFAULT) X(flip_texture_uvs, 0, OPT_NO_DEFAULT) X(texture_use_hint, 0, OPT_NO_DEFAULT)
 
diff --git a/tracerboy_amd/csrc/host/wave_cost.h b/tracerboy_amd/csrc/host/wave_cost.h
--- a/tracerboy_amd/csrc/host/wave_cost.h
+++ b/tracerboy_amd/csrc/host/wave_cost.h
@@ -66,15 +66,24 @@
     r.shear = tb3_make(tb3_get(d, r.kx) / tb3_get(d, r.kz), tb3_get(d, r.ky) / tb3_get(d, r.kz), 1.0f / tb3_get(d, r.kz));
 }
 
-inline bool WaveBoxTest(float& resultT, float closest, const WaveRay& r, tb3 c, tb3 h)
+inline void WaveBoxSlabs(float& enterT, float& leaveT, const WaveRay& r, tb3 c, tb3 h)
 {
     const tb3 mid = tb3_make(tb_fma(c.x, r.inv.x, -r.oinv.x), tb_fma(c.y, r.inv.y, -r.oinv.y), tb_fma(c.z, r.inv.z, -r.oinv.z));
     const tb3 maxL = tb3_make(tb_fma(h.x, r.ainv.x, mid.x), tb_fma(h.y, r.ainv.y, mid.y), tb_fma(h.z, r.ainv.z, mid.z));
     const tb3 minL = tb3_make(tb_fma(-h.x, r.ainv.x, mid.x), tb_fma(-h.y, r.ainv.y, mid.y), tb_fma(-h.z, r.ainv.z, mid.z));
-    const float minT = tb_max(tb_max(minL.x, minL.y), minL.z), maxT = tb_min(tb_min(maxL.x, maxL.y), maxL.z);
-    resultT = tb_max(minT, 0.0f);
-    return resultT < tb_min(maxT, closest);
-}
+    const float minT = tb_max(tb_max(minL.x, minL.y), minL.z);
+    leaveT = tb_min(tb_min(maxL.x, maxL.y), maxL.z);
+    enterT = tb_max(minT, 0.0f);
+}
+inline bool WaveBoxTest(float& resultT, float closest, const WaveRay& r, tb3 c, tb3 h)
+{
+    float leaveT;
+    WaveBoxSlabs(resultT, leaveT, r, c, h);
+    return resultT < tb_min(leaveT, closest);
+}
+struct WaveBoxDirect {
+    bool operator()(float& resultT, float closest, const WaveTree& t, const WaveRay& r, uint32_t n) const { return WaveBoxTest(resultT, closest, r, t.center[n], t.half[n]); }
+};
 
 inline void WaveTriTest(float& hitT, const WaveRay& r, tb3 v0, tb3 v1, tb3 v2)
 {
@@ -99,13 +108,26 @@
 
 constexpr int kWaveWalkStack = 256;
 
-inline float WaveWalk(const WaveTree& t, const WaveRay& r, std::vector<char>& steps)
-{
-    float closest = r.tMax;
-    if (!t.N || r.cannotHit) return closest;
-    float unusedT;
-    if (!WaveBoxTest(unusedT, closest, r, t.center[0], t.half[0])) return closest;
-    uint32_t stack[kWaveWalkStack]; int top = 0; stack[top++] = 0;
+inline void WaveMaskSet(uint64_t mask[2], uint32_t node) { if (node < 128u) mask[node >> 6] |= 1ull << (node & 63u); else mask[0] = mask[1] = ~0ull; }
+
+constexpr uint32_t kWaveNoNode = 0xffffffffu;
+struct WaveVisit { uint32_t node, rest, top, step; float closest; uint32_t first, parked; };
+struct WaveRecord { std::vector<WaveVisit> visits; std::vector<uint32_t> stacks; };
+
+template <class Box>
+inline void WavePushesWith(const Box& box, const WaveTree& t, const WaveRay& r, uint32_t node, float closest, uint32_t& first, uint32_t& parked)
+{
+    const uint32_t l = t.left[node], rr = t.right[node];
+    float lt, rt;
+    const bool lh = box(lt, closest, t, r, l), rh = box(rt, closest, t, r, rr);
+    if (lh && rh) { const bool rightFirst = rt < lt; first = rightFirst ? rr : l; parked = rightFirst ? l : rr; }
+    else { first = lh ? l : (rh ? rr : kWaveNoNode); parked = kWaveNoNode; }
+}
+
+template <class Box>
+inline float WaveWalkOnWith(const Box& box, const WaveTree& t, const WaveRay& r, uint32_t* stack, int top, float closest, std::vector<char>& steps,
+    size_t stepBase, uint64_t* visited, WaveRecord* rec)
+{
     while (top) {
         const uint32_t node = stack[--top];
         if (node >= t.N - 1) {
@@ -115,17 +137,36 @@
             WaveTriTest(t0, r, t.v0[k], t.v1[k], t.v2[k]);
             if (t0 < closest && t0 > kWaveMinT) closest = t0;
         } else {
-            const uint32_t l = t.left[node], rr = t.right[node];
-            float lt, rt;
-            const bool lh = WaveBoxTest(lt, closest, r, t.center[l], t.half[l]), rh = WaveBoxTest(rt, closest, r, t.center[rr], t.half[rr]);
+            uint32_t first, parked;
+            WavePushesWith(box, t, r, node, closest, first, parked);
+            if (rec) { rec->visits.push_back(WaveVisit{node, (uint32_t)rec->stacks.size(), (uint32_t)top, (uint32_t)(steps.size() - stepBase), closest, first, parked});
+                rec->stacks.insert(rec->stacks.end(), stack, stack + top); }
             steps.push_back('I');
+            if (visited) WaveMaskSet(visited, node);
             if (top + 2 > kWaveWalkStack) return closest;
-            if (lh && rh) { const bool rightFirst = rt < lt; stack[top++] = rightFirst ? l : rr; stack[top++] = rightFirst ? rr : l; }
-            else if (lh || rh) stack[top++] = rh ? rr : l;
+            if (parked != kWaveNoNode) stack[top++] = parked;
+            if (first != kWaveNoNode) stack[top++] = first;
         }
     }
     return closest;
 }
+inline float WaveWalkOn(const WaveTree& t, const WaveRay& r, uint32_t* stack, int top, float closest, std::vector<char>& steps, size_t stepBase,
+    uint64_t* visited, WaveRecord* rec)
+{
+    return WaveWalkOnWith(WaveBoxDirect{}, t, r, stack, top, closest, steps, stepBase, visited, rec);
+}
+
+
+inline float WaveWalk(const WaveTree& t, const WaveRay& r, std::vector<char>& steps, uint64_t* visited = nullptr, WaveRecord* rec = nullptr)
+{
+    const float closest = r.tMax;
+    if (!t.N || r.cannotHit) return closest;
+    float unusedT;
+    if (!WaveBoxTest(unusedT, closest, r, t.center[0], t.half[0])) return closest;
+    uint32_t stack[kWaveWalkStack]; stack[0] = 0;
+    return WaveWalkOn(t, r, stack, 1, closest, steps, steps.size(), visited, rec);
+}
+
 
 struct WaveTrips {
     uint64_t inner = 0, leaf = 0, idle = 0;
@@ -140,21 +181,19 @@
     if (lanes > kWaveLanes) lanes = kWaveLanes;
     if (parkMin < 1) parkMin = 1;
     uint32_t p[kWaveLanes] = {};
-    auto at = [&](uint32_t l, char c) { return p[l] < len[l] && steps[l][p[l]] == c; };
-    auto count = [&](char c) { uint32_t n = 0; for (uint32_t l = 0; l < lanes; l++) n += at(l, c) ? 1u : 0u; return n; };
-    uint32_t inner = count('I');
+    uint64_t inner = 0, leaf = 0;
+    auto arrive = [&](uint32_t l) { if (p[l] < len[l]) { const char c = steps[l][p[l]]; if (c == 'I') inner |= 1ull << l; else if (c == 'L') leaf |= 1ull << l; } };
+    auto step = [&](uint64_t& set) { uint64_t m = set; set = 0; while (m) { const uint32_t l = (uint32_t)__builtin_ctzll(m); m &= m - 1; p[l]++; arrive(l); } };
+    for (uint32_t l = 0; l < lanes; l++) arrive(l);
     bool busy;
     do {
         if (inner) do {
-            w.inner++; w.innerActive += inner;
-            for (uint32_t l = 0; l < lanes; l++) if (at(l, 'I')) p[l]++;
-            inner = count('I');
-        } while (inner >= parkMin);
-        const uint32_t leaf = count('L');
+            w.inner++; w.innerActive += (uint64_t)__builtin_popcountll(inner);
+            step(inner);
+        } while ((uint32_t)__builtin_popcountll(inner) >= parkMin);
         busy = inner != 0 || leaf != 0;
-        if (leaf) { w.leaf++; w.leafActive += leaf; for (uint32_t l = 0; l < lanes; l++) if (at(l, 'L')) p[l]++; }
+        if (leaf) { w.leaf++; w.leafActive += (uint64_t)__builtin_popcountll(leaf); step(leaf); }
         else w.idle++;
-        inner = count('I');
     } while (busy);
     return w;
 }
```

Result: faster. 8790 Msamples/s, median of 6 (+1.7%).
